# HengWeiBin/CenterFusionDetect3D

Hardware: AMD Instinct MI355X
Metric: frames/sec/GPU CenterFusion forward, 3x448x800 bs=16; 1/2/4/8-GPU scaling (higher is better)
Workload: dtype f32 storage + f32 accumulate; products as split-operand MFMA passes: f16x3 backbone/neck (3 passes), heads' first 3x3 layers fp16 main term + block-scaled FP6 e2m3 cross terms (1.5 passes), heads' 1x1 layers bf16x3; 1 GPU; Centerfusion_Middle (DLA-34 + DCNv2 neck + pc_dep frustum fusion, 7+4 heads) forward + NMS/top-100 decode + 2D->3D postProcess, bs=16/GPU, 3x448x800, 50-200 radar pts/frame, random-init weights; global_batch=16, parallelism=dp1 (batch shard, async all-gather of the final boxes)

## Files before the change

### centerfusiondetect3d_amd/_lib.py

```python
import ctypes as C
import os

_PKG = os.path.dirname(os.path.abspath(__file__))
LIB_PATH = os.path.join(_PKG, "libcfhip.so")

ABI_VERSION = 7
CF_MAX_SRC = 4
CF_MAX_GROUPS = 4
ACT_NONE, ACT_RELU, ACT_SIGMOID_CLAMP, ACT_RAW_AND_SIGDEPTH = 0, 1, 2, 3
LAYOUT_NHWC, LAYOUT_NCHW = 0, 1

_f = C.c_void_p


class ConvArgs(C.Structure):
    _fields_ = [("src", _f * CF_MAX_SRC), ("src_c", C.c_int32 * CF_MAX_SRC), ("n_src", C.c_int32),
                ("B", C.c_int32), ("H", C.c_int32), ("W", C.c_int32), ("Ho", C.c_int32),
                ("Wo", C.c_int32), ("stride", C.c_int32), ("weight", _f), ("slots", _f),
                ("bias", _f), ("K_pad", C.c_int32), ("N", C.c_int32), ("N_pad", C.c_int32),
                ("residual", _f), ("res_stride", C.c_int32), ("out", _f), ("out2", _f),
                ("out_stride", C.c_int32), ("out_layout", C.c_int32), ("act", C.c_int32),
                ("precise", C.c_int32), ("out_scale", C.c_float), ("in_scale", C.c_float)]


class DcnArgs(C.Structure):
    _fields_ = [("x", _f), ("offmask", _f), ("om_stride", C.c_int32), ("B", C.c_int32),
                ("H", C.c_int32), ("W", C.c_int32), ("C", C.c_int32), ("weight", _f), ("bias", _f),
                ("N", C.c_int32), ("N_pad", C.c_int32), ("out", _f), ("out_stride", C.c_int32),
                ("act", C.c_int32), ("precise", C.c_int32), ("out_scale", C.c_float),
                ("out_split_bf16", _f), ("split_stride", C.c_int32), ("workspace", _f),
                ("workspace_bytes", C.c_size_t), ("mask_activated", C.c_int32), ("out_mx", _f), ("in_scale", C.c_float),
                ("mx_scale", C.c_float)]


class DcnBwdArgs(C.Structure):
    _fields_ = [("gout", _f), ("weight", _f), ("x", _f), ("offmask", _f), ("B", C.c_int32), ("H", C.c_int32),
                ("W", C.c_int32), ("C", C.c_int32), ("N", C.c_int32), ("gx", _f), ("gom", _f), ("gw", _f), ("gbias", _f),
                ("workspace", _f), ("workspace_bytes", C.c_size_t)]


CF_MAX_HEADS = 12
CF_DEPTH_MAPS_MAX = 8


class HeadTailArgs(C.Structure):
    _fields_ = [("x", _f), ("x_stride", C.c_int32), ("B", C.c_int32), ("H", C.c_int32),
                ("W", C.c_int32), ("n_heads", C.c_int32), ("n_hidden", C.c_int32),
                ("w_hidden", (_f * 2) * CF_MAX_HEADS), ("b_hidden", (_f * 2) * CF_MAX_HEADS),
                ("w_out", _f * CF_MAX_HEADS), ("b_out", _f * CF_MAX_HEADS),
                ("out", _f * CF_MAX_HEADS), ("out2", _f * CF_MAX_HEADS),
                ("c_base", C.c_int32 * CF_MAX_HEADS), ("n_out", C.c_int32 * CF_MAX_HEADS),
                ("act", C.c_int32 * CF_MAX_HEADS)]


class HeadFusedArgs(C.Structure):
    _fields_ = [("tail", HeadTailArgs), ("src", _f * 2), ("src_c", C.c_int32 * 2), ("n_src", C.c_int32),
                ("slots", _f), ("K_pad", C.c_int32), ("w_first", _f * CF_MAX_HEADS),
                ("b_first", _f * CF_MAX_HEADS), ("layout3x3", C.c_int32), ("w_out_perm", _f * CF_MAX_HEADS),
                ("mfma16", C.c_int32), ("mx", C.c_int32), ("first_scale", C.c_float * CF_MAX_HEADS)]


class StemArgs(C.Structure):
    _fields_ = [("x", _f), ("B", C.c_int32), ("C", C.c_int32), ("H", C.c_int32), ("W", C.c_int32),
                ("w_base", _f), ("b_base", _f), ("scale_base", C.c_float),
                ("w_level0", _f), ("b_level0", _f), ("scale_level0", C.c_float),
                ("w_level1", _f), ("b_level1", _f), ("scale_level1", C.c_float),
                ("out", _f), ("out_pool", _f), ("in_scale", C.c_float * 3)]


class StemEarlyArgs(C.Structure):
    _fields_ = [("stem", StemArgs), ("pc", _f), ("pc_h", C.c_int32), ("pc_w", C.c_int32), ("w_base_radar", _f)]


class PackSrc(C.Structure):
    _fields_ = [("channels", C.c_int32), ("stride", C.c_int32), ("c_base", C.c_int32)]


class PackBn(C.Structure):
    _fields_ = [("gamma", _f), ("beta", _f), ("mean", _f), ("var", _f), ("eps", C.c_float)]


class PackConvDesc(C.Structure):
    _fields_ = [("weight", _f), ("bias", _f), ("bn", PackBn),
                ("cout", C.c_int32), ("kh", C.c_int32), ("kw", C.c_int32), ("stride", C.c_int32),
                ("pad", C.c_int32), ("dilation", C.c_int32),
                ("src", C.POINTER(PackSrc)), ("n_src", C.c_int32),
                ("proj_weight", _f), ("proj_bias", _f), ("proj_bn", PackBn), ("proj", PackSrc)]


class PackInfo(C.Structure):
    _fields_ = [("n_pad", C.c_int32), ("k_pad", C.c_int32), ("n_slots", C.c_int32), ("patch", C.c_int32),
                ("out_scale", C.c_float), ("weight_bytes", C.c_size_t)]


class DecodeArgs(C.Structure):
    _fields_ = [("scores", _f), ("inds", _f), ("classes", _f), ("reg", _f), ("wh", _f),
                ("depth", _f), ("rot", _f), ("dim", _f), ("amodal", _f), ("att", _f), ("vel", _f),
                ("B", C.c_int32), ("K", C.c_int32), ("H", C.c_int32), ("W", C.c_int32),
                ("out_h", C.c_int32), ("out_w", C.c_int32), ("norm2d", C.c_int32), ("det", _f)]


class SerializeArgs(C.Structure):
    _fields_ = [("post", _f), ("B", C.c_int32), ("K", C.c_int32), ("trans_matrix", _f),
                ("velocity_matrix", _f), ("cs_rot", _f), ("pose_rot", _f), ("rows", _f), ("rotation", _f),
                ("n_samples", C.c_int32), ("sample_ptr", _f), ("sample_frames", _f),
                ("max_per_sample", C.c_int32), ("order", _f), ("counts", _f)]


CF_LOSS_MAX_HEADS = 16
CF_LOSS_STATS = 4 + 4 * CF_LOSS_MAX_HEADS
LOSS_L1, LOSS_L1_UNC, LOSS_BINROT, LOSS_BCE = 0, 1, 2, 3


class LossHead(C.Structure):
    _fields_ = [("kind", C.c_int32), ("channels", C.c_int32), ("map", _f), ("target", _f), ("mask", _f), ("rotbin", _f),
                ("unc", _f), ("weight", C.c_float), ("gmap", _f), ("gunc", _f)]


class LossArgs(C.Structure):
    _fields_ = [("heat", _f), ("heat_gt", _f), ("centers", _f), ("wh", _f), ("mask", _f), ("cls", _f),
                ("B", C.c_int32), ("C", C.c_int32), ("h", C.c_int32), ("w", C.c_int32), ("M", C.c_int32),
                ("n_heads", C.c_int32), ("out_area", C.c_float), ("heat_weight", C.c_float),
                ("head", LossHead * CF_LOSS_MAX_HEADS), ("losses", _f), ("total", _f), ("layer_mask", _f), ("stats", _f),
                ("workspace", _f), ("workspace_bytes", C.c_size_t), ("grad_out", _f), ("gheat", _f)]


CF_HEAD_TRAIN_MAX_HIDDEN = 2
_HT_LAYERS = CF_HEAD_TRAIN_MAX_HIDDEN + 2


class HeadTrainArgs(C.Structure):
    _fields_ = [("x", _f), ("x2", _f), ("x_stride", C.c_int32), ("c_x", C.c_int32), ("x2_stride", C.c_int32),
                ("c_x2", C.c_int32), ("B", C.c_int32), ("h", C.c_int32), ("w", C.c_int32), ("n_hidden", C.c_int32),
                ("hidden", C.c_int32), ("n_out", C.c_int32), ("chunk_px", C.c_int32),
                ("weight", _f * _HT_LAYERS), ("bias", _f * _HT_LAYERS), ("y", _f), ("gy", _f),
                ("gw", _f * _HT_LAYERS), ("gb", _f * _HT_LAYERS), ("workspace", _f), ("workspace_bytes", C.c_size_t)]


CF_TARGETS_MAX_OBJS = 128
CF_TARGETS_F = 20
TGT_HAS_AMODAL, TGT_HAS_ATTRIBUTES, TGT_HAS_VELOCITY, TGT_HAS_ALPHA = 1, 2, 4, 8
TGT_HAS_DEPTH, TGT_HAS_DIMENSION, TGT_HAS_LOCATION, TGT_HAS_YAW = 16, 32, 64, 128
TGT_REP3D, TGT_NORM2D, TGT_WRITE_DEPTH, TGT_WRITE_ROT, TGT_FRUSTUM = 1, 2, 4, 8, 16


class TargetsArgs(C.Structure):
    _fields_ = [("ann", _f), ("iann", _f), ("counts", _f), ("trans", _f), ("calib", _f), ("scale", _f), ("pc_dep", _f),
                ("B", C.c_int32), ("M", C.c_int32), ("C", C.c_int32), ("h", C.c_int32), ("w", C.c_int32),
                ("flags", C.c_int32), ("max_pc_dist", C.c_float),
                ("heat", _f), ("cls", _f), ("mask", _f), ("trunc_mask", _f), ("wh", _f), ("reg", _f), ("amodal_offset", _f),
                ("dimension", _f), ("depth", _f), ("rotbin", _f), ("rotres", _f), ("att", _f), ("att_mask", _f),
                ("velocity", _f), ("pc_hm", _f), ("t_bboxes", _f), ("t_scores", _f), ("t_centers", _f),
                ("t_heat_centers", _f), ("t_bboxes3d", _f), ("t_rotation", _f), ("t_att", _f), ("t_velocity", _f),
                ("workspace", _f), ("workspace_bytes", C.c_size_t)]


_i, _d = C.c_int, C.c_double
SYMBOLS = {
    "cf_conv2d_fused": (_i, [C.POINTER(ConvArgs), _f]),
    "cf_conv2d_f16x3": (_i, [C.POINTER(ConvArgs), _f]),
    "cf_conv3x3_f16x3": (_i, [C.POINTER(ConvArgs), _f]),
    "cf_conv3x3_root_f16x3": (_i, [C.POINTER(ConvArgs), C.POINTER(ConvArgs), C.POINTER(C.c_int32), _f]),
    "cf_conv3x3_proj_f16x3": (_i, [C.POINTER(ConvArgs), C.POINTER(C.c_int32), _f]),
    "cf_conv3x3_f16x3_grouped": (_i, [C.POINTER(C.POINTER(ConvArgs)), C.c_int32, _f]),
    "cf_conv3x3_grouped_form": (_i, [C.POINTER(C.POINTER(ConvArgs)), C.c_int32, C.POINTER(C.c_int32)]),
    "cf_stem_fused": (_i, [C.POINTER(StemArgs), _f]),
    "cf_stem_fused_early": (_i, [C.POINTER(StemEarlyArgs), _f]),
    "cf_split_bf16": (_i, [_f, _f, C.c_long, _i, _i, _i, _f]),
    "cf_head_fused": (_i, [C.POINTER(HeadFusedArgs), _f]),
    "cf_head_fused_with": (_i, [C.POINTER(HeadFusedArgs), _i, _i, _f]),
    "cf_head_fused_at": (_i, [C.POINTER(HeadFusedArgs), _f, _i, _f]),
    "cf_head_slot_tables": (_i, [_f, _f, _i, _i, _i, _f, _f, _f]),
    "cf_pack_feat_mx": (_i, [_f, _i, _f, C.c_long, _f]),
    "cf_pack_feat_mx_scaled": (_i, [_f, _i, _f, C.c_long, C.c_float, _f]),
    "cf_absmax_f32": (_i, [_f, C.c_long, _i, _i, _f, _f]),
    "cf_dcn_v2_fused": (_i, [C.POINTER(DcnArgs), _f]),
    "cf_dcn_v2_f16x3": (_i, [C.POINTER(DcnArgs), _f]),
    "cf_dcn_v2_workspace_bytes": (C.c_size_t, [_i, _i, _i, _i, _i]),
    "cf_dcn_v2_f16x3_grouped": (_i, [C.POINTER(C.POINTER(DcnArgs)), C.c_int32, _f]),
    "cf_gemm_tile_form": (_i, [C.c_long, _i, _i, _i, _i, _i, _i, C.POINTER(C.c_int32), C.POINTER(C.c_int32), C.POINTER(C.c_int32)]),
    "cf_dcn_v2_bwd_data": (_i, [C.POINTER(DcnBwdArgs), _f]),
    "cf_dcn_v2_bwd_weight": (_i, [C.POINTER(DcnBwdArgs), _f]),
    "cf_dcn_v2_bwd_workspace_bytes": (C.c_size_t, [_i, _i, _i, _i, _i]),
    "cf_loss_forward": (_i, [C.POINTER(LossArgs), _f]),
    "cf_loss_backward": (_i, [C.POINTER(LossArgs), _f]),
    "cf_loss_workspace_bytes": (C.c_size_t, [_i, _i, _i, _i]),
    "cf_targets_build": (_i, [C.POINTER(TargetsArgs), _f]),
    "cf_targets_workspace_bytes": (C.c_size_t, [_i, _i]),
    "cf_head_train_forward": (_i, [C.POINTER(HeadTrainArgs), _f]),
    "cf_head_backward": (_i, [C.POINTER(HeadTrainArgs), _f]),
    "cf_head_train_workspace_bytes": (C.c_size_t, [_i, _i, _i, _i, _i, _i]),
    "cf_head_bwd_workspace_bytes": (C.c_size_t, [_i, _i, _i, _i, _i, _i]),
    "cf_head_bwd_chunk_px": (_i, [_i, _i, _i, _i]),
    "cf_head_backward_dx": (_i, [C.POINTER(HeadTrainArgs), _f, _i, _f, _i, _f]),
    "cf_head_bwd_dx_workspace_bytes": (C.c_size_t, [_i, _i, _i, _i, _i, _i]),
    "cf_upsample_dw": (_i, [_f, _f, _f, _f, _i, _i, _i, _i, _i, _f]),
    "cf_maxpool2x2": (_i, [_f, _f, _i, _i, _i, _i, _f]),
    "cf_nchw_to_nhwc4": (_i, [_f, _f, _i, _i, _i, _i, _f]),
    "cf_nhwc_to_nchw": (_i, [_f, _f, _i, _i, _i, _i, _i, _f]),
    "cf_nchw_to_nhwc": (_i, [_f, _f, _i, _i, _i, _i, _i, _i, _f]),
    "cf_radar_ingest": (_i, [_f, _f, _i, _i, _i, _f, _i, _i, _d, _d, _i, _f, _f, _f, _f]),
    "cf_preprocess_images": (_i, [_f, _i, _i, _i, C.POINTER(C.c_double), C.POINTER(C.c_float),
                                 C.POINTER(C.c_float), _i, _i, _f, _f]),
    "cf_augment_workspace_bytes": (C.c_size_t, [_i, _i, _i]),
    "cf_augment_images": (_i, [_f, _i, _i, _i, _f, _f, _f, _f, _f, C.POINTER(C.c_float), C.POINTER(C.c_float), _i, _i, _i, _f,
                              _f, C.c_size_t, _f]),
    "cf_topk_workspace_bytes": (C.c_size_t, [_i, _i]),
    "cf_topk_workspace_bytes_nms": (C.c_size_t, [_i, _i, _i, _i, _i]),
    "cf_topk_peaks": (_i, [_f, _i, _i, _i, _i, _i, _i, _f, _f, _f, _f, _f]),
    "cf_topk_peaks_if_changed": (_i, [_f, _i, _i, _i, _i, _i, _i, _f, _f, _f, _f, _f, _f]),
    "cf_checksum64": (_i, [_f, C.c_long, _f, _f]),
    "cf_frustum_assoc": (_i, [_f, _i, _f, _f, _f, _f, _f, _f, _i, _i, _i, C.c_float, _f, _f, _f, _f]),
    "cf_topk_frustum": (_i, [_f, _i, _i, _f, _f, _f, _f, _f, _f, _i, _i, _i, C.c_float, _f, _f, _f, _f, _f, _f, _f, _f]),
    "cf_pc_hm_direct": (_i, [_f, _i, _i, _i, C.c_float, _f, _f, _f]),
    "cf_radar_roi_expand": (_i, [_f, _f, _f, _i, _i, _i, _f, _f, _i, _i, _i, _f, _f, _f, _f]),
    "cf_pillar_expand": (_i, [_f, _f, _f, _i, _i, _i, _f, _f, _i, _i, _d, _d, _d, _f, _f, _f, _f]),
    "cf_decode_gather": (_i, [C.POINTER(DecodeArgs), _f]),
    "cf_post_process": (_i, [_f, _f, _f, _i, _i, _i, _i, _f, _f]),
    "cf_decode_post": (_i, [C.POINTER(DecodeArgs), _f, _f, _f, _f]),
    "cf_decode_gather_unc": (_i, [C.POINTER(DecodeArgs), _f, _f]),
    "cf_decode_post_unc": (_i, [C.POINTER(DecodeArgs), _f, _f, _f, _f, _f]),
    "cf_depth_maps": (_i, [C.POINTER(_f), C.POINTER(C.c_long), _i, _i, _i, _i, _f, _f]),
    "cf_serialize_nuscenes": (_i, [C.POINTER(SerializeArgs), _f]),
    "cf_serialize_max_candidates": (_i, []),
    "cf_spin_us": (_i, [_i, _f]),
    "cf_last_error": (C.c_char_p, []),
    "cf_pack_conv_f16x3_info": (_i, [C.POINTER(PackConvDesc), C.POINTER(PackInfo)]),
    "cf_pack_conv_f16x3": (_i, [C.POINTER(PackConvDesc), _f, _f, _f, C.POINTER(PackInfo)]),
    "cf_pack_dcn_f16_info": (_i, [_i, _i, C.POINTER(PackInfo)]),
    "cf_pack_dcn_f16": (_i, [_f, _f, C.POINTER(PackBn), _i, _i, _f, _f, C.POINTER(PackInfo)]),
    "cf_abi_version": (_i, []),
}

_lib = None


class CfHipError(RuntimeError):
    pass


def load():
    global _lib
    if _lib is None:
        if not os.path.exists(LIB_PATH):
            raise CfHipError(
                f"{LIB_PATH} is missing: build it with `python -m centerfusiondetect3d_amd.build` "
                "(hipcc, gfx950). The CenterFusion forward has no CPU fallback.")
        lib = C.CDLL(LIB_PATH)
        for name, (res, args) in SYMBOLS.items():
            fn = getattr(lib, name)
            fn.restype, fn.argtypes = res, args
        if lib.cf_abi_version() != ABI_VERSION:
            raise CfHipError(f"{LIB_PATH} has ABI version {lib.cf_abi_version()}, this package needs {ABI_VERSION}: "
                             "rebuild it with `python -m centerfusiondetect3d_amd.build`")
        _lib = lib
    return _lib


def check(status, what=""):
    if status != 0:
        msg = load().cf_last_error().decode()
        raise CfHipError(f"{what} failed with status {status}: {msg}")


def ptr(t):
    return None if t is None else t.data_ptr()


def stream_ptr():
    import torch
    return torch.cuda.current_stream().cuda_stream
```

### centerfusiondetect3d_amd/csrc/cf_heads.hip

```cpp
#include <string>
#include "cf_common.h"
#include "cf_mx.h"

namespace {

typedef __bf16 bf16x8 __attribute__((ext_vector_type(8)));
typedef unsigned int u32x4 __attribute__((ext_vector_type(4)));
typedef unsigned int u32x2 __attribute__((ext_vector_type(2)));
typedef _Float16 hf16x8 __attribute__((ext_vector_type(8)));
typedef int i32x8 __attribute__((ext_vector_type(8)));

constexpr int HT_PX = 64;
constexpr int HT_C = 256;
constexpr int HT_ROWB = HT_C * 2 + 16;
constexpr int HT_PLANE = HT_PX * HT_ROWB;
constexpr int HT_LDS = 2 * HT_PLANE;

struct HeadTailK {
  const unsigned char* x;
  int x_stride;
  int M, HW;
  int n_heads;
  int n_hidden;
  const unsigned char* w_hidden[CF_MAX_HEADS][2];
  const float* b_hidden[CF_MAX_HEADS][2];
  const unsigned char* w_out[CF_MAX_HEADS];
  const float* b_out[CF_MAX_HEADS];
  float* out[CF_MAX_HEADS];
  float* out2[CF_MAX_HEADS];
  int c_base[CF_MAX_HEADS];
  int n_out[CF_MAX_HEADS];
  int act[CF_MAX_HEADS];
};

__device__ __forceinline__ float bf16_rne(float a) { return (float)(__bf16)a; }
__device__ __forceinline__ unsigned pack2(float a, float b) {
  return ((unsigned)__builtin_bit_cast(unsigned short, (__bf16)b) << 16) |
         __builtin_bit_cast(unsigned short, (__bf16)a);
}

__device__ __forceinline__ const bf16x8* wfrag(const unsigned char* w, int rt, int ks, int plane, int n_ks, int lane) {
  const unsigned char* base = w + ((size_t)rt * n_ks + ks) * 2048 + plane * 1024;
  return reinterpret_cast<const bf16x8*>(base + (unsigned)lane * 16u);
}

template <bool SCALED = false>
__device__ __forceinline__ void store_hidden_tile16(unsigned char* xt, const f32x4 (&acc)[4][4], const float* bias,
                                                    int wave, int lane, float sc = 1.0f, int pxcol = -1) {
  const int g = lane >> 4, c16 = pxcol < 0 ? (lane & 15) : pxcol;
#pragma unroll
  for (int rt = 0; rt < 4; ++rt) {
    const int ch = wave * 64 + rt * 16 + 4 * g;
    const f32x4 bb = *reinterpret_cast<const f32x4*>(bias + ch);
#pragma unroll
    for (int ct = 0; ct < 4; ++ct) {
      float v[4], hi[4];
#pragma unroll
      for (int e = 0; e < 4; ++e) {
        v[e] = fmaxf(SCALED ? __builtin_fmaf(acc[rt][ct][e], sc, bb[e]) : acc[rt][ct][e] + bb[e], 0.0f);
        hi[e] = bf16_rne(v[e]);
      }
      unsigned char* o = xt + (ct * 16 + c16) * HT_ROWB + ch * 2;
      const u32x2 ph = {pack2(hi[0], hi[1]), pack2(hi[2], hi[3])};
      const u32x2 pl = {pack2(v[0] - hi[0], v[1] - hi[1]), pack2(v[2] - hi[2], v[3] - hi[3])};
      *reinterpret_cast<u32x2*>(o) = ph;
      *reinterpret_cast<u32x2*>(o + HT_PLANE) = pl;
    }
  }
}

struct TileMap {
  int b, y0, x0, H, W, sh = 4;
  __device__ __forceinline__ bool operator()(int px, int& bb, int& pix) const {
    const int y = y0 + (px >> sh), x = x0 + (px & ((1 << sh) - 1));
    if (y >= H || x >= W) return false;
    bb = b;
    pix = y * W + x;
    return true;
  }
};

constexpr int AT_SLOTS = 18;
__device__ __forceinline__ int at_slot_of(int ty, int tx) { return (ty % 3 == 0 && tx % 3 == 0) ? (ty / 3) * 6 + tx / 3 : -1; }
struct SlotMap {
  const int* slots;
  int M, HW, half;
  __device__ __forceinline__ bool operator()(int px, int& bb, int& pix) const {
    const int t = half * 64 + px, sl = at_slot_of(t >> 4, t & 15);
    if (sl < 0) return false;
    const int s = slots[sl];
    if ((unsigned)s >= (unsigned)M) return false;
    bb = s / HW;
    pix = s - bb * HW;
    return true;
  }
};

template <class PixMap>
__device__ __forceinline__ void head_tail_from_lds16(const HeadTailK& p, unsigned char* xt, int head, const PixMap& pm) {
  const int tid = threadIdx.x, lane = tid & 63, wave = tid >> 6;
  const int g = lane >> 4, c16 = lane & 15;
  for (int l = 0; l < p.n_hidden; ++l) {
    const unsigned char* w = p.w_hidden[head][l];
    const float* bias = p.b_hidden[head][l];
    f32x4 acc[4][4];
#pragma unroll
    for (int a = 0; a < 4; ++a)
#pragma unroll
      for (int b = 0; b < 4; ++b)
#pragma unroll
        for (int r = 0; r < 4; ++r) acc[a][b][r] = 0.0f;
    bf16x8 wh[2][4], wl[2][4];
#pragma unroll
    for (int rt = 0; rt < 4; ++rt) {
      wh[0][rt] = *wfrag(w, wave * 4 + rt, 0, 0, 8, lane);
      wl[0][rt] = *wfrag(w, wave * 4 + rt, 0, 1, 8, lane);
    }
#pragma unroll
    for (int ks = 0; ks < 8; ++ks) {
      if (ks + 1 < 8) {
#pragma unroll
        for (int rt = 0; rt < 4; ++rt) {
          wh[(ks + 1) & 1][rt] = *wfrag(w, wave * 4 + rt, ks + 1, 0, 8, lane);
          wl[(ks + 1) & 1][rt] = *wfrag(w, wave * 4 + rt, ks + 1, 1, 8, lane);
        }
      }
      bf16x8 xh[4], xl[4];
#pragma unroll
      for (int ct = 0; ct < 4; ++ct) {
        const unsigned char* row = xt + (ct * 16 + c16) * HT_ROWB + (ks * 32 + g * 8) * 2;
        xh[ct] = *reinterpret_cast<const bf16x8*>(row);
        xl[ct] = *reinterpret_cast<const bf16x8*>(row + HT_PLANE);
      }
#pragma unroll
      for (int rt = 0; rt < 4; ++rt)
#pragma unroll
        for (int ct = 0; ct < 4; ++ct)
          acc[rt][ct] = __builtin_amdgcn_mfma_f32_16x16x32_bf16(wl[ks & 1][rt], xh[ct], acc[rt][ct], 0, 0, 0);
#pragma unroll
      for (int rt = 0; rt < 4; ++rt)
#pragma unroll
        for (int ct = 0; ct < 4; ++ct)
          acc[rt][ct] = __builtin_amdgcn_mfma_f32_16x16x32_bf16(wh[ks & 1][rt], xl[ct], acc[rt][ct], 0, 0, 0);
#pragma unroll
      for (int rt = 0; rt < 4; ++rt)
#pragma unroll
        for (int ct = 0; ct < 4; ++ct)
          acc[rt][ct] = __builtin_amdgcn_mfma_f32_16x16x32_bf16(wh[ks & 1][rt], xh[ct], acc[rt][ct], 0, 0, 0);
      __builtin_amdgcn_sched_barrier(0);
    }
    __syncthreads();
    store_hidden_tile16(xt, acc, bias, wave, lane);
    __syncthreads();
  }

  f32x4 oacc[4];
#pragma unroll
  for (int b = 0; b < 4; ++b)
#pragma unroll
    for (int r = 0; r < 4; ++r) oacc[b][r] = 0.0f;
  {
    const unsigned char* w = p.w_out[head];
#pragma unroll
    for (int s2 = 0; s2 < 2; ++s2) {
      const int ks = wave * 2 + s2;
      const bf16x8 ah = *wfrag(w, 0, ks, 0, 8, lane), al = *wfrag(w, 0, ks, 1, 8, lane);
#pragma unroll
      for (int ct = 0; ct < 4; ++ct) {
        const unsigned char* row = xt + (ct * 16 + c16) * HT_ROWB + (ks * 32 + g * 8) * 2;
        const bf16x8 xh = *reinterpret_cast<const bf16x8*>(row);
        const bf16x8 xl = *reinterpret_cast<const bf16x8*>(row + HT_PLANE);
        oacc[ct] = __builtin_amdgcn_mfma_f32_16x16x32_bf16(al, xh, oacc[ct], 0, 0, 0);
        oacc[ct] = __builtin_amdgcn_mfma_f32_16x16x32_bf16(ah, xl, oacc[ct], 0, 0, 0);
        oacc[ct] = __builtin_amdgcn_mfma_f32_16x16x32_bf16(ah, xh, oacc[ct], 0, 0, 0);
      }
    }
  }
  __syncthreads();
  float* red = reinterpret_cast<float*>(xt);
  const int n_out = p.n_out[head], act = p.act[head];
#pragma unroll
  for (int ct = 0; ct < 4; ++ct)
#pragma unroll
    for (int r = 0; r < 4; ++r) {
      const int n = 4 * g + r;
      if (n < n_out) red[(wave * 16 + n) * HT_PX + ct * 16 + c16] = oacc[ct][r];
    }
  __syncthreads();
  const float* bo = p.b_out[head];
  float* out = p.out[head];
  float* out2 = p.out2[head];
  const int px = tid & 63;
  int b, pix;
  if (pm(px, b, pix)) {
    for (int n = tid >> 6; n < n_out; n += 4) {
      const float raw = red[n * HT_PX + px] + red[(16 + n) * HT_PX + px] + red[(32 + n) * HT_PX + px] +
                        red[(48 + n) * HT_PX + px] + bo[n];
      const size_t o = ((size_t)b * n_out + n) * p.HW + pix;
      float v = raw;
      if (act == CF_ACT_RELU) v = fmaxf(raw, 0.0f);
      else if (act == CF_ACT_SIGMOID_CLAMP) v = fminf(fmaxf(cf_sigmoid(raw), 1e-4f), 1.0f - 1e-4f);
      out[o] = v;
      if (act == CF_ACT_RAW_AND_SIGDEPTH) out2[o] = 1.0f / (cf_sigmoid(raw) + 1e-6f) - 1.0f;
    }
  }
}

constexpr int HP_ROWS = (8 + 2) * (16 + 2);
constexpr int HP_PX = 8 * 16;
constexpr int HP16_RED = 4 * 16 * HP_PX * 4;
constexpr int hp16_patch_bytes(bool pc) { return HP_ROWS * (4 * 64 + (pc ? 32 : 0) + 16); }
constexpr int HP_PCIMG_ROWB = 32 * 2 + 16;
constexpr int HP_PCIMG = HP_PX * 2 * HP_PCIMG_ROWB;
constexpr int hp16_pc_extra(bool pc) { return pc ? 16 + HP_PCIMG : 0; }
constexpr int hp16_lds(bool pc, bool hidden) {
  return hidden ? (HT_LDS > hp16_patch_bytes(pc) + hp16_pc_extra(pc) ? HT_LDS : hp16_patch_bytes(pc) + hp16_pc_extra(pc))
                : hp16_patch_bytes(pc) + hp16_pc_extra(pc) + HP16_RED;
}

struct HeadPatchK {
  HeadTailK t;
  const unsigned char* src[2];
  int src_c[2];
  int H, W, tiles_x, tiles_y, n_ks;
  int pc_skip;
  int hloop;
  const unsigned char* w_first[CF_MAX_HEADS];
  const float* b_first[CF_MAX_HEADS];
  const unsigned char* w_out_perm[CF_MAX_HEADS];
  float first_scale[CF_MAX_HEADS];
  const int* slot_pixels;
};

template <int NS, bool PC, bool TP, bool MX = false, int HID = -1, bool AT = false>
__global__ __launch_bounds__(256, 2) void head_patch16_kernel(HeadPatchK q) {
  static_assert(NS == 4, "64 feature channels");
  static_assert(!AT || !TP, "virtual tiles are laid out on the flat 8 x 16 tile");
  constexpr int MX_SLAB = 14592, PC_OFF = MX ? 272 : NS * 64;
  constexpr int TSH = TP ? 3 : 4, TMASK = (1 << TSH) - 1;
  constexpr int T_H = TP ? 16 : 8, T_W = TP ? 8 : 16, P_W = T_W + 2;
  static_assert((T_H + 2) * P_W == HP_ROWS, "both tile shapes have the same patch size");
  constexpr int ROWB = NS * 64 + (PC ? 32 : 0) + 16;
  constexpr int NKF = 9 * NS / 2;
  constexpr int NK = NKF + (PC ? 1 : 0);
  extern __shared__ __attribute__((aligned(16))) unsigned char xt[];
  const HeadTailK& p = q.t;
  const int tid = threadIdx.x, lane = tid & 63, wave = __builtin_amdgcn_readfirstlane(tid >> 6);
  const int g = lane >> 4;
  const int c16 = (MX && !TP) ? ((lane & 12) == 4 || (lane & 12) == 8 ? (((lane & 15) - 4) & 3) * 4 + (((lane & 15) - 4) >> 2)
                                                                      : (lane & 3) * 4 + 2 + ((lane & 15) >> 3))
                              : (lane & 15);
  const int per_img = q.tiles_x * q.tiles_y;
  const int per_head = AT ? per_img : per_img * (p.M / p.HW);
  const int hg = blockIdx.x / per_head;
  int rem = cf_xcd_remap(blockIdx.x - hg * per_head, per_head);
  const int head0 = hg * q.hloop, head1 = min(head0 + q.hloop, p.n_heads);
  const int b = rem / per_img;
  rem -= b * per_img;
  const int y0 = (rem / q.tiles_x) * T_H, x0 = (rem % q.tiles_x) * T_W;
  const int* const at_slots = AT ? q.slot_pixels + (size_t)rem * AT_SLOTS : nullptr;
  auto at_src = [&](int row) -> int {
    const int pr = row / P_W, pc = row % P_W;
    if (pr >= 9) return -1;
    const int s = at_slots[(pr / 3) * 6 + pc / 3];
    if ((unsigned)s >= (unsigned)p.M) return -1;
    const int bb = s / p.HW, pix = s - bb * p.HW;
    const int y = pix / q.W + pr % 3 - 1, x = pix % q.W + pc % 3 - 1;
    if ((unsigned)y >= (unsigned)q.H || (unsigned)x >= (unsigned)q.W) return -1;
    return bb * p.HW + y * q.W + x;
  };
  if constexpr (AT) {
    int any = 0;
    for (int i = 0; i < AT_SLOTS; ++i) any |= (unsigned)at_slots[i] < (unsigned)p.M ? 1 : 0;
    if (!any) return;
  }

  if constexpr (MX) {
    constexpr int UPR = 17;
    constexpr int NIT = (HP_ROWS * UPR + 255) / 256;
    u32x4 v[NIT];
#pragma unroll
    for (int it = 0; it < NIT; ++it) {
      const int idx = tid + it * 256;
      const int row = idx / UPR, u = idx % UPR;
      const int y = y0 - 1 + row / P_W, x = x0 - 1 + row % P_W;
      v[it] = u32x4{0u, 0u, 0u, 0u};
      if constexpr (AT) {
        const int s = row < HP_ROWS ? at_src(row) : -1;
        if (s >= 0) v[it] = *reinterpret_cast<const u32x4*>(q.src[0] + (size_t)s * 272 + u * 16);
      } else
      if (row < HP_ROWS && (unsigned)y < (unsigned)q.H && (unsigned)x < (unsigned)q.W)
        v[it] = *reinterpret_cast<const u32x4*>(q.src[0] + (size_t)(b * p.HW + y * q.W + x) * 272 + u * 16);
    }
#pragma unroll
    for (int it = 0; it < NIT; ++it) {
      const int idx = tid + it * 256;
      const int row = idx / UPR, u = idx % UPR;
      if (row < HP_ROWS) *reinterpret_cast<u32x4*>(xt + row * ROWB + u * 16) = v[it];
    }
  } else {
    constexpr int UPR = NS * 4;
    constexpr int NIT = (HP_ROWS * UPR + 255) / 256;
    u32x4 v[NIT];
#pragma unroll
    for (int it = 0; it < NIT; ++it) {
      const int idx = tid + it * 256;
      const int row = idx / UPR, u = idx % UPR;
      const int y = y0 - 1 + row / P_W, x = x0 - 1 + row % P_W;
      v[it] = u32x4{0u, 0u, 0u, 0u};
      if constexpr (AT) {
        const int s = row < HP_ROWS ? at_src(row) : -1;
        if (s >= 0) v[it] = *reinterpret_cast<const u32x4*>(q.src[0] + ((size_t)s * 2 * q.src_c[0]) * 2 +
                                                             (u / (NS * 2)) * q.src_c[0] * 2 + (u % (NS * 2)) * 16);
      } else
      if (row < HP_ROWS && (unsigned)y < (unsigned)q.H && (unsigned)x < (unsigned)q.W)
        v[it] = *reinterpret_cast<const u32x4*>(q.src[0] + ((size_t)(b * p.HW + y * q.W + x) * 2 * q.src_c[0]) * 2 +
                                                (u / (NS * 2)) * q.src_c[0] * 2 + (u % (NS * 2)) * 16);
    }
#pragma unroll
    for (int it = 0; it < NIT; ++it) {
      const int idx = tid + it * 256;
      const int row = idx / UPR, u = idx % UPR;
      const int plane = u / (NS * 2), uu = u % (NS * 2);
      if (row < HP_ROWS) *reinterpret_cast<u32x4*>(xt + row * ROWB + (uu >> 1) * 64 + plane * 32 + (uu & 1) * 16) = v[it];
    }
  }
  unsigned* const pc_flags = reinterpret_cast<unsigned*>(xt + hp16_patch_bytes(PC));
  if (PC) {
    unsigned nz = 0u;
    for (int idx = tid; idx < HP_ROWS * 2; idx += 256) {
      const int row = idx >> 1, plane = idx & 1;
      const int y = y0 - 1 + row / P_W, x = x0 - 1 + row % P_W;
      u32x4 w = {0u, 0u, 0u, 0u};
      if constexpr (AT) {
        const int s = at_src(row);
        if (s >= 0) w = *reinterpret_cast<const u32x4*>(q.src[1] + ((size_t)s * 2 + plane) * q.src_c[1] * 2);
      } else
      if ((unsigned)y < (unsigned)q.H && (unsigned)x < (unsigned)q.W)
        w = *reinterpret_cast<const u32x4*>(q.src[1] + ((size_t)(b * p.HW + y * q.W + x) * 2 + plane) * q.src_c[1] * 2);
      *reinterpret_cast<u32x4*>(xt + row * ROWB + PC_OFF + plane * 16) = w;
      nz |= (w[0] | w[1] | w[2] | w[3]) & 0x7fff7fffu;
    }
    const bool wave_nz = __builtin_amdgcn_ballot_w64(nz != 0u) != 0ull;
    if (lane == 0) pc_flags[wave] = (wave_nz || !q.pc_skip) ? 1u : 0u;
  }

  int rowb[8];
#pragma unroll
  for (int ct = 0; ct < 8; ++ct)
    rowb[ct] = ((c16 >> TSH) * P_W + (c16 & TMASK)) * ROWB + ct * ((16 >> TSH) * P_W * ROWB);
  const int koff = (g >> 1) * 64 + (g & 1) * 16;
  unsigned char* const pcimg = xt + hp16_patch_bytes(PC) + 16;
  const int imgb = c16 * (2 * HP_PCIMG_ROWB) + g * 16;
  __syncthreads();
  bool pc_live = false;
  if (PC) {
    const u32x4 f = *reinterpret_cast<const u32x4*>(pc_flags);
    pc_live = __builtin_amdgcn_readfirstlane((int)(f[0] | f[1] | f[2] | f[3])) != 0;
  }
  if (PC && pc_live) {
    const int ipx = tid & (HP_PX - 1), plane = tid >> 7;
    const unsigned char* sp = xt + ((ipx >> TSH) * P_W + (ipx & TMASK)) * ROWB + PC_OFF + plane * 16;
    unsigned e[32];
#pragma unroll
    for (int t = 0; t < 9; ++t) {
      const u32x2 w = *reinterpret_cast<const u32x2*>(sp + ((t / 3) * P_W + t % 3) * ROWB);
      e[3 * t] = w[0] & 0xffffu;
      e[3 * t + 1] = w[0] >> 16;
      e[3 * t + 2] = w[1] & 0xffffu;
    }
#pragma unroll
    for (int k = 27; k < 32; ++k) e[k] = 0u;
    unsigned char* dp = pcimg + (ipx * 2 + plane) * HP_PCIMG_ROWB;
#pragma unroll
    for (int j = 0; j < 4; ++j)
      *reinterpret_cast<u32x4*>(dp + j * 16) = u32x4{e[8 * j] | (e[8 * j + 1] << 16), e[8 * j + 2] | (e[8 * j + 3] << 16),
                                                     e[8 * j + 4] | (e[8 * j + 5] << 16), e[8 * j + 6] | (e[8 * j + 7] << 16)};
    __syncthreads();
  }
  auto pc_kstep = [&](const bf16x8 (&ah)[4], const bf16x8 (&al)[4], f32x4 (&acc)[4][8]) __attribute__((always_inline)) {
#pragma unroll
    for (int hf = 0; hf < 2; ++hf) {
      bf16x8 xh[4], xl[4];
#pragma unroll
      for (int ct = 0; ct < 4; ++ct) {
        const unsigned char* r = pcimg + imgb + (4 * hf + ct) * (16 * 2 * HP_PCIMG_ROWB);
        xh[ct] = *reinterpret_cast<const bf16x8*>(r);
        xl[ct] = *reinterpret_cast<const bf16x8*>(r + HP_PCIMG_ROWB);
      }
#pragma unroll
      for (int rt = 0; rt < 4; ++rt)
#pragma unroll
        for (int ct = 0; ct < 4; ++ct)
          acc[rt][4 * hf + ct] = __builtin_amdgcn_mfma_f32_16x16x32_bf16(al[rt], xh[ct], acc[rt][4 * hf + ct], 0, 0, 0);
#pragma unroll
      for (int rt = 0; rt < 4; ++rt)
#pragma unroll
        for (int ct = 0; ct < 4; ++ct)
          acc[rt][4 * hf + ct] = __builtin_amdgcn_mfma_f32_16x16x32_bf16(ah[rt], xl[ct], acc[rt][4 * hf + ct], 0, 0, 0);
#pragma unroll
      for (int rt = 0; rt < 4; ++rt)
#pragma unroll
        for (int ct = 0; ct < 4; ++ct)
          acc[rt][4 * hf + ct] = __builtin_amdgcn_mfma_f32_16x16x32_bf16(ah[rt], xh[ct], acc[rt][4 * hf + ct], 0, 0, 0);
    }
  };
  auto first_layer = [&](int head, f32x4 (&acc)[4][8]) __attribute__((always_inline)) {
  if constexpr (MX) {
    const unsigned char* wb = q.w_first[head] + (size_t)wave * (9 * MX_SLAB);
#pragma unroll
    for (int a = 0; a < 4; ++a)
#pragma unroll
      for (int c = 0; c < 8; ++c)
#pragma unroll
        for (int r = 0; r < 4; ++r) acc[a][c][r] = 0.0f;
    hf16x8 am[2][4];
    u32x4 ax0[4];
    u32x2 ax1[4];
    int sa;
    auto slab = [&](int tap) {
      return __builtin_amdgcn_make_buffer_rsrc(const_cast<unsigned char*>(wb + tap * MX_SLAB), 0, MX_SLAB, 0x00020000);
    };
    const int l16 = lane * 16, l8 = lane * 8, l4 = lane * 4;
    bf16x8 ph[4], pl[4];
    auto ldp = [&](bf16x8 (&d)[4], int plane) {
      const __amdgpu_buffer_rsrc_t rs = __builtin_amdgcn_make_buffer_rsrc(
          const_cast<unsigned char*>(q.w_first[head] + (size_t)4 * 9 * MX_SLAB), 0, 4 * 3 * 4 * 2048, 0x00020000);
      const int lo = l16 + (g ? 2 * 4 * 2048 : 0);
#pragma unroll
      for (int rt = 0; rt < 4; ++rt)
        d[rt] = __builtin_bit_cast(bf16x8, __builtin_amdgcn_raw_buffer_load_b128(rs, lo, wave * (3 * 4 * 2048) + rt * 2048 + plane * 1024, 0));
    };
    auto ldm = [&](hf16x8 (&d)[4], int tap, int ks2) {
      const __amdgpu_buffer_rsrc_t rs = slab(tap);
#pragma unroll
      for (int rt = 0; rt < 4; ++rt)
        d[rt] = __builtin_bit_cast(hf16x8, __builtin_amdgcn_raw_buffer_load_b128(rs, l16, (rt * 2 + ks2) * 1024, 0));
    };
    auto ldx = [&](int tap) {
      const __amdgpu_buffer_rsrc_t rs = slab(tap);
#pragma unroll
      for (int rt = 0; rt < 4; ++rt) {
        ax0[rt] = __builtin_bit_cast(u32x4, __builtin_amdgcn_raw_buffer_load_b128(rs, l16, 8192 + rt * 1536, 0));
        ax1[rt] = __builtin_bit_cast(u32x2, __builtin_amdgcn_raw_buffer_load_b64(rs, l8, 8192 + rt * 1536 + 1024, 0));
      }
      sa = (int)__builtin_amdgcn_raw_buffer_load_b32(rs, l4, 14336, 0);
    };
    auto main_half = [&](const hf16x8 (&A)[4], int off, int hf) {
      hf16x8 xb[4];
#pragma unroll
      for (int ct = 0; ct < 4; ++ct) xb[ct] = *reinterpret_cast<const hf16x8*>(xt + rowb[4 * hf + ct] + off);
#pragma unroll
      for (int rt = 0; rt < 4; ++rt)
#pragma unroll
        for (int ct = 0; ct < 4; ++ct)
          acc[rt][4 * hf + ct] = __builtin_amdgcn_mfma_f32_16x16x32_f16(A[rt], xb[ct], acc[rt][4 * hf + ct], 0, 0, 0);
    };
    auto cross_pair = [&](int toff, int pr) {
      i32x8 xb[2];
      int sb[2];
#pragma unroll
      for (int c2 = 0; c2 < 2; ++c2) {
        const unsigned char* r = xt + rowb[2 * pr + c2] + toff;
        const u32x4 b0 = *reinterpret_cast<const u32x4*>(r + 64 * g + 32);
        const u32x2 b1 = *reinterpret_cast<const u32x2*>(r + 64 * g + 48);
        xb[c2] = i32x8{(int)b0[0], (int)b0[1], (int)b0[2], (int)b0[3], (int)b1[0], (int)b1[1], 0, 0};
        sb[c2] = (int)(*reinterpret_cast<const unsigned*>(r + 256) >> (8 * g));
      }
#define CF_MX_ROW(RT)                                                                                                   \
      {                                                                                                                 \
        const i32x8 a6 = {(int)ax0[RT][0], (int)ax0[RT][1], (int)ax0[RT][2], (int)ax0[RT][3], (int)ax1[RT][0],          \
                          (int)ax1[RT][1], 0, 0};                                                                       \
        _Pragma("unroll") for (int c2 = 0; c2 < 2; ++c2)                                                                \
          acc[RT][2 * pr + c2] = __builtin_amdgcn_mfma_scale_f32_16x16x128_f8f6f4(a6, xb[c2], acc[RT][2 * pr + c2],    \
                                                                                  2, 2, RT, sa, 0, sb[c2]);             \
      }
      CF_MX_ROW(0) CF_MX_ROW(1) CF_MX_ROW(2) CF_MX_ROW(3)
#undef CF_MX_ROW
    };
    ldm(am[0], 0, 0);
    ldm(am[1], 0, 1);
    ldx(0);
#pragma unroll
    for (int tap = 0; tap < 9; ++tap) {
      const int toff = ((tap / 3) * P_W + tap % 3) * ROWB;
      const int o0 = toff + g * 64, o1 = toff + g * 64 + 16;
      main_half(am[0], o0, 0);
      if (tap > 0) ldx(tap);
      __builtin_amdgcn_sched_barrier(0);
      main_half(am[0], o0, 1);
      main_half(am[1], o1, 0);
      if (tap + 1 < 9) ldm(am[0], tap + 1, 0);
      else if (PC && HID == 1) ldp(ph, 0);
      __builtin_amdgcn_sched_barrier(0);
      main_half(am[1], o1, 1);
      cross_pair(toff, 0);
      cross_pair(toff, 1);
      if (tap + 1 < 9) ldm(am[1], tap + 1, 1);
      else if (PC && HID == 1) ldp(pl, 1);
      __builtin_amdgcn_sched_barrier(0);
      cross_pair(toff, 2);
      cross_pair(toff, 3);
    }
    __builtin_amdgcn_sched_barrier(0);
    if (PC) {
      if (pc_live) {
        if constexpr (HID != 1) { ldp(ph, 0); ldp(pl, 1); }
        pc_kstep(ph, pl, acc);
      }
    }
    return;
  }
  const unsigned char* w1 = q.w_first[head];
#pragma unroll
  for (int a = 0; a < 4; ++a)
#pragma unroll
    for (int c = 0; c < 8; ++c)
#pragma unroll
      for (int r = 0; r < 4; ++r) acc[a][c][r] = 0.0f;

  bf16x8 wh[2][4], wl[2][4];
  auto load_w = [&](bf16x8 (&dh)[4], bf16x8 (&dl)[4], int ks) {
#pragma unroll
    for (int rt = 0; rt < 4; ++rt) {
      dh[rt] = *wfrag(w1, wave * 4 + rt, ks, 0, q.n_ks, lane);
      dl[rt] = *wfrag(w1, wave * 4 + rt, ks, 1, q.n_ks, lane);
    }
  };
  load_w(wh[0], wl[0], 0);

#pragma unroll
  for (int ks = 0; ks < NKF; ++ks) {
    if (ks + 1 < NK) load_w(wh[(ks + 1) & 1], wl[(ks + 1) & 1], ks + 1);
    const int tap = ks / (NS / 2), half = ks % (NS / 2);
    const int off = ((tap / 3) * P_W + tap % 3) * ROWB + half * 128 + koff, lo = 32;
#pragma unroll
    for (int hf = 0; hf < 2; ++hf) {
      bf16x8 xh[4], xl[4];
#pragma unroll
      for (int ct = 0; ct < 4; ++ct) {
        xh[ct] = *reinterpret_cast<const bf16x8*>(xt + rowb[4 * hf + ct] + off);
        xl[ct] = *reinterpret_cast<const bf16x8*>(xt + rowb[4 * hf + ct] + off + lo);
      }
#pragma unroll
      for (int rt = 0; rt < 4; ++rt)
#pragma unroll
        for (int ct = 0; ct < 4; ++ct)
          acc[rt][4 * hf + ct] = __builtin_amdgcn_mfma_f32_16x16x32_bf16(wl[ks & 1][rt], xh[ct], acc[rt][4 * hf + ct], 0, 0, 0);
#pragma unroll
      for (int rt = 0; rt < 4; ++rt)
#pragma unroll
        for (int ct = 0; ct < 4; ++ct)
          acc[rt][4 * hf + ct] = __builtin_amdgcn_mfma_f32_16x16x32_bf16(wh[ks & 1][rt], xl[ct], acc[rt][4 * hf + ct], 0, 0, 0);
#pragma unroll
      for (int rt = 0; rt < 4; ++rt)
#pragma unroll
        for (int ct = 0; ct < 4; ++ct)
          acc[rt][4 * hf + ct] = __builtin_amdgcn_mfma_f32_16x16x32_bf16(wh[ks & 1][rt], xh[ct], acc[rt][4 * hf + ct], 0, 0, 0);
    }
    __builtin_amdgcn_sched_barrier(0);
  }
  if (PC) {
    if (pc_live) pc_kstep(wh[NKF & 1], wl[NKF & 1], acc);
  }
  };

  if (HID < 0 ? p.n_hidden > 0 : HID == 1) {
    const int head = head0;
    f32x4 acc[4][8];
    first_layer(head, acc);
    __syncthreads();
#pragma unroll
    for (int half = 0; half < 2; ++half) {
      f32x4 a2[4][4];
#pragma unroll
      for (int rt = 0; rt < 4; ++rt)
#pragma unroll
        for (int ct = 0; ct < 4; ++ct) a2[rt][ct] = acc[rt][4 * half + ct];
      store_hidden_tile16<MX>(xt, a2, q.b_first[head], wave, lane, MX ? q.first_scale[head] : 1.0f, c16);
      if constexpr (MX) __builtin_amdgcn_sched_barrier(0);
      __syncthreads();
      if constexpr (AT) head_tail_from_lds16(p, xt, head, SlotMap{at_slots, p.M, p.HW, half});
      else head_tail_from_lds16(p, xt, head, TileMap{b, y0 + (64 >> TSH) * half, x0, q.H, q.W, TSH});
      __syncthreads();
    }
    return;
  }
  if constexpr (HID == 1) return;

  for (int head = head0; head < head1; ++head) {
  f32x4 acc[4][8];
  first_layer(head, acc);
  f32x4 oacc[8];
#pragma unroll
  for (int c = 0; c < 8; ++c)
#pragma unroll
    for (int r = 0; r < 4; ++r) oacc[c][r] = 0.0f;
  {
    const float* b1 = q.b_first[head] + wave * 64 + 4 * g;
    const unsigned char* wo = q.w_out_perm[head];
    const float fsc = MX ? q.first_scale[head] : 1.0f;
    (void)fsc;
#pragma unroll
    for (int s2 = 0; s2 < 2; ++s2) {
      const int ks2 = wave * 2 + s2;
      const bf16x8 ah = *wfrag(wo, 0, ks2, 0, 8, lane), al = *wfrag(wo, 0, ks2, 1, 8, lane);
      const f32x4 ba = *reinterpret_cast<const f32x4*>(b1 + 32 * s2);
      const f32x4 bb = *reinterpret_cast<const f32x4*>(b1 + 32 * s2 + 16);
#pragma unroll
      for (int ct = 0; ct < 8; ++ct) {
        float v[8], hi[8];
#pragma unroll
        for (int j = 0; j < 8; ++j) {
          const float bj = j < 4 ? ba[j] : bb[j - 4];
          v[j] = fmaxf(MX ? __builtin_fmaf(acc[2 * s2 + (j >> 2)][ct][j & 3], fsc, bj) : acc[2 * s2 + (j >> 2)][ct][j & 3] + bj, 0.0f);
          hi[j] = bf16_rne(v[j]);
        }
        const u32x4 ph = {pack2(hi[0], hi[1]), pack2(hi[2], hi[3]), pack2(hi[4], hi[5]), pack2(hi[6], hi[7])};
        const u32x4 pl = {pack2(v[0] - hi[0], v[1] - hi[1]), pack2(v[2] - hi[2], v[3] - hi[3]),
                          pack2(v[4] - hi[4], v[5] - hi[5]), pack2(v[6] - hi[6], v[7] - hi[7])};
        const bf16x8 xh = __builtin_bit_cast(bf16x8, ph), xl = __builtin_bit_cast(bf16x8, pl);
        oacc[ct] = __builtin_amdgcn_mfma_f32_16x16x32_bf16(al, xh, oacc[ct], 0, 0, 0);
        oacc[ct] = __builtin_amdgcn_mfma_f32_16x16x32_bf16(ah, xl, oacc[ct], 0, 0, 0);
        oacc[ct] = __builtin_amdgcn_mfma_f32_16x16x32_bf16(ah, xh, oacc[ct], 0, 0, 0);
      }
    }
  }
  const int n_out = p.n_out[head], act = p.act[head];
  float* red = reinterpret_cast<float*>(xt + hp16_patch_bytes(PC) + hp16_pc_extra(PC));
#pragma unroll
  for (int ct = 0; ct < 8; ++ct)
#pragma unroll
    for (int r = 0; r < 4; ++r) {
      const int n = 4 * g + r;
      if (n < n_out) red[(wave * 16 + n) * HP_PX + ct * 16 + c16] = oacc[ct][r];
    }
  __syncthreads();
  {
    const int px = tid & (HP_PX - 1);
    const int y = y0 + (px >> TSH), x = x0 + (px & TMASK);
    bool valid = y < q.H && x < q.W;
    int ob = b;
    size_t opix = (size_t)y * q.W + x;
    if constexpr (AT) {
      const int sl = at_slot_of(px >> 4, px & 15);
      const int s = sl >= 0 ? at_slots[sl] : -1;
      valid = (unsigned)s < (unsigned)p.M;
      ob = s / p.HW;
      opix = (size_t)(s - ob * p.HW);
    }
    if (valid) {
      const float* bo = p.b_out[head];
      float* out = p.out[head];
      float* out2 = p.out2[head];
      for (int n = tid >> 7; n < n_out; n += 2) {
        const float raw = red[n * HP_PX + px] + red[(16 + n) * HP_PX + px] + red[(32 + n) * HP_PX + px] +
                          red[(48 + n) * HP_PX + px] + bo[n];
        const size_t o = ((size_t)ob * n_out + n) * p.HW + opix;
        float v = raw;
        if (act == CF_ACT_RELU) v = fmaxf(raw, 0.0f);
        else if (act == CF_ACT_SIGMOID_CLAMP) v = fminf(fmaxf(cf_sigmoid(raw), 1e-4f), 1.0f - 1e-4f);
        out[o] = v;
        if (act == CF_ACT_RAW_AND_SIGDEPTH) out2[o] = 1.0f / (cf_sigmoid(raw) + 1e-6f) - 1.0f;
      }
    }
  }
  __syncthreads();
  }
}

__global__ __launch_bounds__(256) void pack_feat_mx_kernel(const float* __restrict__ x, int in_stride,
                                                           unsigned char* __restrict__ rows, long M, float scale) {
  const long t = (long)blockIdx.x * 256 + threadIdx.x;
  const long m = t >> 1;
  const int blk = (int)(t & 1);
  if (m >= M) return;
  const f32x4* src = reinterpret_cast<const f32x4*>(x + m * in_stride + 32 * blk);
  float v[32];
#pragma unroll
  for (int i = 0; i < 8; ++i) {
    const f32x4 q = src[i];
#pragma unroll
    for (int e = 0; e < 4; ++e) v[4 * i + e] = q[e];
  }
  mx_pack_block(v, rows + m * 272, blk, scale);
}

}

extern "C" int cf_pack_feat_mx_scaled(const float* x, int in_stride, void* rows, long M, float scale, void* stream) {
  CF_REQUIRE(x && rows && M > 0, "cf_pack_feat_mx: null tensor or M=%ld", M);
  const float sc = cf_resolve_in_scale(scale);
  CF_REQUIRE(sc > 0.0f, "cf_pack_feat_mx_scaled: scale must be 0 (= 16) or a power of two");
  CF_REQUIRE(in_stride >= 64 && in_stride % 4 == 0, "cf_pack_feat_mx: in_stride=%d (64 channels, 16-byte aligned rows)", in_stride);
  CF_REQUIRE(M < (1L << 30), "cf_pack_feat_mx: M=%ld too large", M);
  const long threads = 2 * M;
  hipLaunchKernelGGL(pack_feat_mx_kernel, dim3((unsigned)((threads + 255) / 256)), dim3(256), 0, (hipStream_t)stream, x,
                     in_stride, static_cast<unsigned char*>(rows), M, sc);
  return cf_check_launch("cf_pack_feat_mx");
}

extern "C" int cf_pack_feat_mx(const float* x, int in_stride, void* rows, long M, void* stream) {
  return cf_pack_feat_mx_scaled(x, in_stride, rows, M, 16.0f, stream);
}

static int fill_tail(const cf_head_tail_args* a, HeadTailK& k) {
  CF_REQUIRE(a->B > 0 && a->H > 0 && a->W > 0, "cf_head_fused: bad geometry");
  CF_REQUIRE(a->n_heads >= 1 && a->n_heads <= CF_MAX_HEADS, "cf_head_fused: n_heads=%d", a->n_heads);
  CF_REQUIRE(a->n_hidden >= 0 && a->n_hidden <= 2, "cf_head_fused: n_hidden=%d", a->n_hidden);
  const long M = (long)a->B * a->H * a->W;
  CF_REQUIRE(M < (1L << 31), "cf_head_fused: tensor too large");
  k.x = reinterpret_cast<const unsigned char*>(a->x);
  k.x_stride = a->x_stride;
  k.M = (int)M;
  k.HW = a->H * a->W;
  k.n_heads = a->n_heads;
  k.n_hidden = a->n_hidden;
  for (int i = 0; i < a->n_heads; ++i) {
    for (int l = 0; l < a->n_hidden; ++l) {
      CF_REQUIRE(a->w_hidden[i][l] && a->b_hidden[i][l], "cf_head_fused: head %d layer %d weights missing", i, l);
      k.w_hidden[i][l] = reinterpret_cast<const unsigned char*>(a->w_hidden[i][l]);
      k.b_hidden[i][l] = a->b_hidden[i][l];
    }
    CF_REQUIRE(a->w_out[i] && a->b_out[i] && a->out[i], "cf_head_fused: head %d output layer missing", i);
    CF_REQUIRE(a->n_out[i] >= 1 && a->n_out[i] <= 32, "cf_head_fused: head %d n_out=%d", i, a->n_out[i]);
    CF_REQUIRE(a->act[i] != CF_ACT_RAW_AND_SIGDEPTH || a->out2[i], "cf_head_fused: head %d needs out2", i);
    k.w_out[i] = reinterpret_cast<const unsigned char*>(a->w_out[i]);
    k.b_out[i] = a->b_out[i];
    k.out[i] = a->out[i];
    k.out2[i] = a->out2[i];
    k.c_base[i] = a->c_base[i];
    k.n_out[i] = a->n_out[i];
    k.act[i] = a->act[i];
  }
  return CF_OK;
}

constexpr int HEAD_MAX_K_PAD = 2048;
#define CF_HEAD_FORMS "cf_head_fused runs layout3x3 = 1 (64-channel first source [, 8-channel second]) with mfma16 = 1 " \
                      "(16x16x32 fragments, n_out <= 16) only"

static int head_fused_launch(const cf_head_fused_args* a, const int* slot_pixels, int n_tiles, int tile, int pc_skip, void* stream) {
  const bool at = slot_pixels != nullptr;
  HeadPatchK hp{};
  hp.slot_pixels = slot_pixels;
  const int rc = fill_tail(&a->tail, hp.t);
  if (rc != CF_OK) return rc;
  CF_REQUIRE(a->n_src >= 1 && a->n_src <= 2, "cf_head_fused: n_src=%d", a->n_src);
  for (int i = 0; i < a->n_src; ++i) {
    CF_REQUIRE(a->src[i] && a->src_c[i] > 0 && a->src_c[i] % 8 == 0, "cf_head_fused: source %d invalid", i);
    hp.src[i] = reinterpret_cast<const unsigned char*>(a->src[i]);
    hp.src_c[i] = a->src_c[i];
  }
  const bool mx = a->mx != 0;
  if (mx) {
    CF_REQUIRE(a->layout3x3 && a->mfma16 && a->src_c[0] == 64 && (a->n_src == 1 || a->src_c[1] == 8),
               "cf_head_fused: mx = 1 needs layout3x3 = 1, mfma16 = 1, a 64-channel mx source [and an 8-channel pc_hm source]");
  } else {
    CF_REQUIRE(a->slots && a->K_pad > 0 && a->K_pad % 64 == 0, "cf_head_fused: K_pad=%d must be a multiple of 64", a->K_pad);
    CF_REQUIRE(a->K_pad <= HEAD_MAX_K_PAD, "cf_head_fused: K_pad=%d exceeds %d", a->K_pad, HEAD_MAX_K_PAD);
  }
  const int n_heads = a->tail.n_heads, H = a->tail.H, W = a->tail.W;
  for (int i = 0; i < n_heads; ++i) {
    CF_REQUIRE(a->w_first[i] && a->b_first[i], "cf_head_fused: head %d first layer missing", i);
    hp.w_first[i] = reinterpret_cast<const unsigned char*>(a->w_first[i]);
    hp.b_first[i] = a->b_first[i];
  }
  if (!(a->layout3x3 && a->src_c[0] == 64 && (a->n_src == 1 || a->src_c[1] == 8))) {
    CF_REQUIRE(a->mfma16 == 0, "cf_head_fused: mfma16 fragments need the 3x3 patch layout (layout3x3 = 1, 64-channel first "
                               "source [, 8-channel second]); this launch would run on the 32x32x16 slot-table kernel");
    cf_set_error(CF_HEAD_FORMS ": there is no slot-table kernel (layout3x3 = 0)");
    return CF_EINVAL;
  }
  const bool m16 = a->mfma16 != 0;
  hp.H = H; hp.W = W;
  hp.n_ks = a->K_pad / 32;
  CF_REQUIRE(mx || a->K_pad / 16 >= (a->n_src == 2 ? 38 : 36), "cf_head_fused: K_pad=%d too small for the 3x3 layout", a->K_pad);
  for (int i = 0; i < n_heads; ++i) {
    CF_REQUIRE(!mx || (a->first_scale[i] > 0.0f && a->first_scale[i] < 1e30f), "cf_head_fused: head %d: first_scale missing (mx)", i);
    hp.first_scale[i] = a->first_scale[i];
  }
  if (m16) {
    CF_REQUIRE(mx || (a->K_pad % 32 == 0 && a->K_pad / 32 >= (a->n_src == 2 ? 19 : 18)), "cf_head_fused: K_pad=%d (16x16x32 fragments)", a->K_pad);
    for (int i = 0; i < n_heads; ++i)
      CF_REQUIRE(a->tail.n_out[i] <= 16, "cf_head_fused: head %d: n_out=%d > 16 (the 16x16x32 kernels produce ONE 16-row output tile, with or without hidden layers)", i, a->tail.n_out[i]);
  }
  for (int i = 0; i < n_heads; ++i) {
    CF_REQUIRE(a->tail.n_hidden > 0 || a->w_out_perm[i], "cf_head_fused: head %d: w_out_perm missing", i);
    hp.w_out_perm[i] = reinterpret_cast<const unsigned char*>(a->w_out_perm[i]);
  }
  const long t_land = (long)((W + 15) / 16) * ((H + 7) / 8), t_port = (long)((W + 7) / 8) * ((H + 15) / 16);
  CF_REQUIRE(t_land * a->tail.B * n_heads < (1L << 31), "cf_head_fused: grid too large");
  CF_REQUIRE(m16, CF_HEAD_FORMS ": nothing reads 32x32x16 fragments (mfma16 = 0)");
  bool portrait = tile < 0 ? t_port < t_land : tile != 0;
  if (at) portrait = false;
  hp.pc_skip = pc_skip != 0;
  hp.tiles_x = portrait ? (W + 7) / 8 : (W + 15) / 16;
  hp.tiles_y = portrait ? (H + 15) / 16 : (H + 7) / 8;
  const int n_img = at ? 1 : a->tail.B;
  if (at) { hp.tiles_x = n_tiles; hp.tiles_y = 1; }
  int hloop = 1;
  if (a->tail.n_hidden == 0) {
    static const int slots = [] {
      int dev = 0, cus = 256;
      if (hipGetDevice(&dev) == hipSuccess) (void)hipDeviceGetAttribute(&cus, hipDeviceAttributeMultiprocessorCount, dev);
      return 2 * (cus > 0 ? cus : 256);
    }();
    const long tiles = (long)hp.tiles_x * hp.tiles_y * n_img;
    const int n = n_heads, cand[3] = {1, 2, (n + 1) / 2};
    double best = 0.0;
    for (int i = 0; i < 3; ++i) {
      const int h = cand[i] < 1 ? 1 : (cand[i] > n ? n : cand[i]);
      const double cost = (double)((tiles * ((n + h - 1) / h) + slots - 1) / slots) * (h + 0.25);
      if (i == 0 || cost < best - 1e-9) { best = cost; hloop = h; }
    }
  }
  hp.hloop = hloop;
  const long blocks = (long)hp.tiles_x * hp.tiles_y * n_img * ((n_heads + hloop - 1) / hloop);
  CF_REQUIRE(blocks < (1L << 31), "%s: grid too large", at ? "cf_head_fused_at" : "cf_head_fused");
  const bool hidden = a->tail.n_hidden > 0;
  const bool pc = a->n_src == 2;
  const int lds = hp16_lds(pc, hidden);
  auto launch = [&](auto kernel, CfLdsLimit& lim) {
    lim.ensure(kernel, lds, hp16_lds(pc, false));
    hipLaunchKernelGGL(kernel, dim3((unsigned)blocks), dim3(256), lds, (hipStream_t)stream, hp);
  };
  static CfLdsLimit lim16[4], limx[4], limxh[2], lim_at[4];
  if (at) {
    CF_REQUIRE(!mx || hidden == pc, "cf_head_fused_at: mx = 1 runs without hidden layers and pc_hm source, or with both (the forms "
                                    "the model's head groups take); pack other heads for bf16x3");
    if (mx && hidden) launch(head_patch16_kernel<4, true, false, true, 1, true>, lim_at[3]);
    else if (mx) launch(head_patch16_kernel<4, false, false, true, 0, true>, lim_at[2]);
    else if (pc) launch(head_patch16_kernel<4, true, false, false, -1, true>, lim_at[1]);
    else launch(head_patch16_kernel<4, false, false, false, -1, true>, lim_at[0]);
    return cf_check_launch("cf_head_fused_at");
  }
  if (mx && hidden) {
    CF_REQUIRE(pc, "cf_head_fused: mx = 1 with hidden layers needs the pc_hm source (n_src = 2); pack such heads for bf16x3");
    if (portrait) launch(head_patch16_kernel<4, true, true, true, 1>, limxh[1]);
    else launch(head_patch16_kernel<4, true, false, true, 1>, limxh[0]);
  } else if (mx) {
    if (pc && portrait) launch(head_patch16_kernel<4, true, true, true, 0>, limx[3]);
    else if (pc) launch(head_patch16_kernel<4, true, false, true, 0>, limx[2]);
    else if (portrait) launch(head_patch16_kernel<4, false, true, true, 0>, limx[1]);
    else launch(head_patch16_kernel<4, false, false, true, 0>, limx[0]);
  } else {
    if (pc && portrait) launch(head_patch16_kernel<4, true, true>, lim16[3]);
    else if (pc) launch(head_patch16_kernel<4, true, false>, lim16[2]);
    else if (portrait) launch(head_patch16_kernel<4, false, true>, lim16[1]);
    else launch(head_patch16_kernel<4, false, false>, lim16[0]);
  }
  return cf_check_launch("cf_head_fused");
}

extern "C" int cf_head_fused_with(const cf_head_fused_args* a, int tile, int pc_skip, void* stream) {
  CF_REQUIRE(a != nullptr, "cf_head_fused: null args (a)");
  CF_REQUIRE(tile >= -1 && tile <= 1, "cf_head_fused_with: tile=%d is not 0 (8 x 16), 1 (16 x 8) or -1 (the rule's own)", tile);
  CF_REQUIRE(pc_skip >= -1 && pc_skip <= 1, "cf_head_fused_with: pc_skip=%d is not 0, 1 or -1 (the rule's own)", pc_skip);
  return head_fused_launch(a, nullptr, 0, tile, pc_skip, stream);
}

extern "C" int cf_head_fused(const cf_head_fused_args* a, void* stream) { return cf_head_fused_with(a, -1, -1, stream); }

extern "C" int cf_head_fused_at(const cf_head_fused_args* a, const int32_t* slot_pixels, int n_tiles, void* stream) {
  CF_REQUIRE(a != nullptr, "cf_head_fused_at: null args");
  CF_REQUIRE(slot_pixels != nullptr && n_tiles > 0, "cf_head_fused_at: slot table missing or n_tiles=%d", n_tiles);
  const int rc = head_fused_launch(a, slot_pixels, n_tiles, -1, -1, stream);
  if (rc == CF_EINVAL) {
    const std::string why = cf_last_error();
    cf_set_error("cf_head_fused_at: %s", why.c_str());
  }
  return rc;
}

namespace {
__global__ __launch_bounds__(256) void head_slot_tables_kernel(const int* __restrict__ tk, const int* __restrict__ pk, int B, int K,
                                                               int HW, int* __restrict__ tp, int* __restrict__ ts) {
  const int i = blockIdx.x * 256 + threadIdx.x;
  const int per_p = (2 * K + AT_SLOTS - 1) / AT_SLOTS * AT_SLOTS, per_s = (K + AT_SLOTS - 1) / AT_SLOTS * AT_SLOTS;
  if (tp && i < B * per_p) {
    const int b = i / per_p, j = i - b * per_p;
    int v = -1;
    if (j < K) v = tk ? tk[b * K + j] : -1;
    else if (j < 2 * K) v = pk ? pk[b * K + j - K] : -1;
    tp[i] = (unsigned)v < (unsigned)HW ? b * HW + v : -1;
  }
  if (ts && i < B * per_s) {
    const int b = i / per_s, j = i - b * per_s;
    const int v = (j < K && pk) ? pk[b * K + j] : -1;
    ts[i] = (unsigned)v < (unsigned)HW ? b * HW + v : -1;
  }
}
}

extern "C" int cf_head_slot_tables(const int32_t* list_a, const int32_t* list_b, int B, int K, int HW, int32_t* table_ab,
                                   int32_t* table_b, void* stream) {
  CF_REQUIRE(B > 0 && K > 0 && HW > 0, "cf_head_slot_tables: B=%d K=%d HW=%d", B, K, HW);
  CF_REQUIRE((long)B * HW < (1L << 31), "cf_head_slot_tables: B * HW must stay below 2^31 (flat pixels are int32)");
  CF_REQUIRE((long)B * (2L * K + AT_SLOTS) < (1L << 31), "cf_head_slot_tables: B * K too large");
  CF_REQUIRE(list_a || list_b, "cf_head_slot_tables: no list");
  CF_REQUIRE(table_ab || table_b, "cf_head_slot_tables: no table");
  CF_REQUIRE(!table_b || list_b, "cf_head_slot_tables: table_b is built from list_b");
  const long n = (long)B * ((2 * K + AT_SLOTS - 1) / AT_SLOTS * AT_SLOTS);
  hipLaunchKernelGGL(head_slot_tables_kernel, dim3((unsigned)((n + 255) / 256)), dim3(256), 0, (hipStream_t)stream, list_a,
                     list_b, B, K, HW, table_ab, table_b);
  return cf_check_launch("cf_head_slot_tables");
}
```

### centerfusiondetect3d_amd/csrc/cf_topk.hip

```cpp
#include "cf_topk.h"

namespace {
template <bool NMS>
__device__ __forceinline__ float peak_value(const float* __restrict__ img, int i, int H, int W) {
  const float v = img[i];
  if (!NMS) return v;
  const int HW = H * W;
  const int c = i / HW, pix = i - c * HW;
  const int y = pix / W, x = pix - y * W;
  const float* pl = img + (size_t)c * HW;
  float m = v;
  const int y0 = y > 0 ? y - 1 : y, y1 = y < H - 1 ? y + 1 : y;
  const int x0 = x > 0 ? x - 1 : x, x1 = x < W - 1 ? x + 1 : x;
  for (int yy = y0; yy <= y1; ++yy)
    for (int xx = x0; xx <= x1; ++xx) m = fmaxf(m, pl[yy * W + xx]);
  return (m == v) ? v : v * 0.0f;
}

__global__ __launch_bounds__(256) void nms_kernel(const float* __restrict__ heat, float* __restrict__ out, int H,
                                                  int W, long total) {
  const long N = (long)H * W;
  for (long i = (long)blockIdx.x * 256 + threadIdx.x; i < total; i += (long)gridDim.x * 256) {
    const long plane = i / N;
    out[i] = peak_value<true>(heat + plane * N, (int)(i - plane * N), H, W);
  }
}

template <bool NMS>
__device__ __forceinline__ void topk_slice_body(const float* __restrict__ heat, int C, int H, int W, int K,
                                                uint64_t* __restrict__ out_keys, int img_i, int slice) {
  __shared__ __attribute__((aligned(16))) uint64_t keys[TOPK_CAP];
  __shared__ uint32_t hist[256];
  __shared__ uint32_t wave_cnt[TOPK_THREADS / 64];
  __shared__ uint32_t s_gt, s_sel[2];
  const int tid = threadIdx.x;
  const int HW = H * W, N = C * HW;
  const float* img = heat + (size_t)img_i * N;
  const int len = (N + TOPK_SLICES - 1) / TOPK_SLICES;
  const int lo = min(slice * len, N), hi = min(lo + len, N);
  uint64_t* out = out_keys + ((size_t)img_i * TOPK_SLICES + slice) * K;
  const int n = hi - lo;
  if (n <= K) {
    topk_tiny_slice<TOPK_THREADS>(keys, lo, n, K, out, [&](int i) { return f2u(peak_value<NMS>(img, i, H, W)); });
    return;
  }

  uint32_t lmax = 0;
  {
    int i = lo + tid;
    for (; i + 3 * TOPK_THREADS < hi; i += 4 * TOPK_THREADS) {
      float v[4];
#pragma unroll
      for (int u = 0; u < 4; ++u) v[u] = img[i + u * TOPK_THREADS];
#pragma unroll
      for (int u = 0; u < 4; ++u)
        if (!NMS || f2u(v[u]) > lmax || v[u] < 0.0f)
          lmax = max(lmax, NMS ? f2u(peak_value<NMS>(img, i + u * TOPK_THREADS, H, W)) : f2u(v[u]));
    }
    for (; i < hi; i += TOPK_THREADS) {
      const float v = img[i];
      if (!NMS || f2u(v) > lmax || v < 0.0f) lmax = max(lmax, f2u(peak_value<NMS>(img, i, H, W)));
    }
  }
  uint32_t* lm = reinterpret_cast<uint32_t*>(keys);
  lm[tid] = lmax;
  __syncthreads();
  {
    const u32x4p* l4 = reinterpret_cast<const u32x4p*>(lm);
    int rank = 0;
#pragma unroll 8
    for (int j4 = 0; j4 < TOPK_THREADS / 4; ++j4) {
      const u32x4p o = l4[j4];
#pragma unroll
      for (int e = 0; e < 4; ++e) rank += (o[e] > lmax || (o[e] == lmax && 4 * j4 + e < tid)) ? 1 : 0;
    }
    if (rank == K - 1) s_sel[0] = lmax;
  }
  __syncthreads();
  uint32_t L = s_sel[0];
  __syncthreads();

  for (int attempt = 0; attempt < 2; ++attempt) {
    if (tid == 0) s_gt = 0;
    __syncthreads();
    {
      auto take = [&](int i, float v) {
        uint32_t u = f2u(v);
        if (NMS && (u > L || v < 0.0f)) u = f2u(peak_value<NMS>(img, i, H, W));
        if (u > L) {
          const uint32_t pos = atomicAdd(&s_gt, 1u);
          if (pos < TOPK_CAP) keys[pos] = pack_key(u, i);
        }
      };
      int i = lo + tid;
      for (; i + 3 * TOPK_THREADS < hi; i += 4 * TOPK_THREADS) {
        float v[4];
#pragma unroll
        for (int u = 0; u < 4; ++u) v[u] = img[i + u * TOPK_THREADS];
#pragma unroll
        for (int u = 0; u < 4; ++u) take(i + u * TOPK_THREADS, v[u]);
      }
      for (; i < hi; i += TOPK_THREADS) take(i, img[i]);
    }
    __syncthreads();
    if (s_gt <= TOPK_CAP) break;
    L = topk_radix_select<TOPK_THREADS>(hist, s_sel, K, [&](auto count) {
      for (int i = lo + tid; i < hi; i += TOPK_THREADS) count(f2u(peak_value<NMS>(img, i, H, W)));
    });
  }
  const int g = (int)s_gt;
  int total = g;
  if (g < K) {
    const int r = K - g;
    int found = 0;
    for (int base = lo; base < hi && found < r; base += TOPK_THREADS) {
      const int i = base + tid;
      const bool eq = (i < hi) && (!NMS || f2u(img[i]) >= L || img[i] < 0.0f) && (f2u(peak_value<NMS>(img, i, H, W)) == L);
      int all;
      const int rank = found + topk_tie_round<TOPK_THREADS>(eq, wave_cnt, all);
      if (eq && rank < r) keys[g + rank] = pack_key(L, i);
      found += all;
      __syncthreads();
    }
    total = K;
  }
  if (total <= 4 * TOPK_THREADS) {
    __syncthreads();
    rank_select_desc(keys, total, K, out);
    return;
  }
  int P = 1;
  while (P < total) P <<= 1;
  for (int i = total + tid; i < P; i += TOPK_THREADS) keys[i] = 0;
  __syncthreads();
  bitonic_sort_desc(keys, P);
  for (int j = tid; j < K; j += TOPK_THREADS) out[j] = keys[j];
}

template <bool NMS>
__global__ __launch_bounds__(TOPK_THREADS) void topk_slice_kernel(const float* __restrict__ heat, int C, int H,
                                                                  int W, int K, uint64_t* __restrict__ out_keys) {
  topk_slice_body<NMS>(heat, C, H, W, K, out_keys, blockIdx.x / TOPK_SLICES, blockIdx.x % TOPK_SLICES);
}

__global__ __launch_bounds__(TOPK_RT) void topk_slice_reg_kernel(const float* __restrict__ heat, int C, int H, int W, int K,
                                                                 uint64_t* __restrict__ out_keys) {
  __shared__ uint64_t keys[TOPK_CAP];
  __shared__ __attribute__((aligned(16))) uint32_t gmax[256];
  __shared__ uint32_t hist[256];
  __shared__ uint32_t wave_cnt[TOPK_RT / 64];
  __shared__ uint32_t s_gt, s_sel[2];
  const int tid = threadIdx.x;
  const int N = C * H * W;
  const int img_i = blockIdx.x / TOPK_SLICES, slice = blockIdx.x % TOPK_SLICES;
  const float* img = heat + (size_t)img_i * N;
  const int len = (N + TOPK_SLICES - 1) / TOPK_SLICES;
  const int lo = min(slice * len, N), hi = min(lo + len, N);
  uint64_t* out = out_keys + (size_t)blockIdx.x * K;
  const int n = hi - lo;
  if (n <= K) {
    topk_tiny_slice<TOPK_RT>(keys, lo, n, K, out, [&](int i) { return f2u(img[i]); });
    return;
  }
  uint32_t u[TOPK_RE];
  uint32_t lmax = 0;
#pragma unroll
  for (int e = 0; e < TOPK_RE; ++e) {
    const int i = lo + tid + e * TOPK_RT;
    u[e] = i < hi ? f2u(img[i]) : 0u;
  }
#pragma unroll
  for (int e = 0; e < TOPK_RE; ++e) lmax = max(lmax, u[e]);
  const int P = K <= 128 ? 8 : 4, G = TOPK_RT / P;
  {
    uint32_t m = lmax;
    m = max(m, (uint32_t)__shfl_xor((int)m, 1));
    m = max(m, (uint32_t)__shfl_xor((int)m, 2));
    if (P == 8) m = max(m, (uint32_t)__shfl_xor((int)m, 4));
    if ((tid & (P - 1)) == 0) gmax[tid / P] = m;
  }
  if (tid == 0) s_sel[0] = 0u;
  __syncthreads();
  {
    const int c = tid / P, part = tid & (P - 1), per = G / P;
    const uint32_t mine = gmax[c];
    const u32x4p* g4 = reinterpret_cast<const u32x4p*>(gmax + part * per);
    int rank = 0;
#pragma unroll 4
    for (int j4 = 0; j4 < per / 4; ++j4) {
      const u32x4p o = g4[j4];
#pragma unroll
      for (int e = 0; e < 4; ++e) rank += (o[e] > mine || (o[e] == mine && part * per + 4 * j4 + e < c)) ? 1 : 0;
    }
    rank += __shfl_xor(rank, 1);
    rank += __shfl_xor(rank, 2);
    if (P == 8) rank += __shfl_xor(rank, 4);
    if (part == 0 && rank == K - 1) s_sel[0] = mine;
  }
  __syncthreads();
  uint32_t L = s_sel[0];
  __syncthreads();

  if (tid == 0) s_gt = 0;
  __syncthreads();
#pragma unroll
  for (int e = 0; e < TOPK_RE; ++e) {
    const int i = lo + tid + e * TOPK_RT;
    if (i < hi && u[e] >= L) {
      const uint32_t pos = atomicAdd(&s_gt, 1u);
      if (pos < TOPK_CAP) keys[pos] = pack_key(u[e], i);
    }
  }
  __syncthreads();
  if (s_gt <= TOPK_CAP) {
    rank_select_desc(keys, (int)s_gt, K, out);
    return;
  }
  __syncthreads();

  for (int attempt = 0; attempt < 2; ++attempt) {
    if (tid == 0) s_gt = 0;
    __syncthreads();
#pragma unroll
    for (int e = 0; e < TOPK_RE; ++e) {
      const int i = lo + tid + e * TOPK_RT;
      if (i < hi && u[e] > L) {
        const uint32_t pos = atomicAdd(&s_gt, 1u);
        if (pos < TOPK_CAP) keys[pos] = pack_key(u[e], i);
      }
    }
    __syncthreads();
    if (s_gt <= TOPK_CAP) break;
    L = topk_radix_select<TOPK_RT>(hist, s_sel, K, [&](auto count) {
#pragma unroll
      for (int e = 0; e < TOPK_RE; ++e)
        if (lo + tid + e * TOPK_RT < hi) count(u[e]);
    });
  }
  const int g = (int)s_gt;
  int total = g;
  if (g < K) {
    const int r = K - g;
    int found = 0;
#pragma unroll 1
    for (int e = 0; e < TOPK_RE && found < r; ++e) {
      const int i = lo + tid + e * TOPK_RT;
      uint32_t ue = 0;
#pragma unroll
      for (int q = 0; q < TOPK_RE; ++q) ue = q == e ? u[q] : ue;
      const bool eq = i < hi && ue == L;
      int all;
      const int rank = found + topk_tie_round<TOPK_RT>(eq, wave_cnt, all);
      if (eq && rank < r) keys[g + rank] = pack_key(L, i);
      found += all;
      __syncthreads();
    }
    total = K;
  }
  __syncthreads();
  rank_select_desc(keys, total, K, out);
}

template <int THREADS>
__device__ __forceinline__ void emit_peaks(const uint64_t* best, int K, int HW, int b, float* __restrict__ scores,
                                           int32_t* __restrict__ inds, int32_t* __restrict__ classes) {
  for (int j = threadIdx.x; j < K; j += THREADS) {
    float score;
    int pix, cls;
    unpack_key(best[j], HW, score, pix, cls);
    scores[(size_t)b * K + j] = score;
    inds[(size_t)b * K + j] = pix;
    classes[(size_t)b * K + j] = cls;
  }
}

__global__ __launch_bounds__(TOPK_MERGE_THREADS) void topk_merge_kernel(const uint64_t* __restrict__ in_keys,
                                                                        int K, int HW, float* __restrict__ scores,
                                                                        int32_t* __restrict__ inds,
                                                                        int32_t* __restrict__ classes) {
  extern __shared__ __attribute__((aligned(16))) uint64_t keys[];
  const int tid = threadIdx.x, total = TOPK_SLICES * K;
  const uint64_t* src = in_keys + (size_t)blockIdx.x * total;
  for (int i = tid; i < total; i += TOPK_MERGE_THREADS) keys[i] = src[i];
  __syncthreads();
  emit_peaks<TOPK_MERGE_THREADS>(merge_sorted_lists(keys, keys + total, K), K, HW, blockIdx.x, scores, inds, classes);
}
}

static int topk_check_geometry(const char* who, int B, int C, int H, int W, int K) {
  CF_REQUIRE(B > 0 && C > 0 && H > 0 && W > 0, "%s: bad geometry", who);
  CF_REQUIRE(K >= 1 && K <= TOPK_MAXK, "%s: K=%d outside [1,%d]", who, K, TOPK_MAXK);
  CF_REQUIRE((long)C * H * W >= K, "%s: fewer than K elements per image", who);
  CF_REQUIRE((long)C * H * W < (1L << 31), "%s: image too large", who);
  return CF_OK;
}

int topk_launch_slices(const char* who, const float* heat, int B, int C, int H, int W, int K, int nms, void* workspace,
                       hipStream_t st) {
  if (const int e = topk_check_geometry(who, B, C, H, W, K)) return e;
  CF_REQUIRE(nms >= 0 && nms <= 2, "%s: nms=%d", who, nms);
  uint64_t* keys = static_cast<uint64_t*>(workspace);
  if (nms == 2) {
    float* sup = reinterpret_cast<float*>(static_cast<unsigned char*>(workspace) + ((cf_topk_workspace_bytes(B, K) + 255) / 256) * 256);
    const long total = (long)B * C * H * W;
    const long blocks = (total + 255) / 256;
    hipLaunchKernelGGL(nms_kernel, dim3((unsigned)(blocks < 65536 ? blocks : 65536)), dim3(256), 0, st, heat, sup, H, W, total);
    heat = sup;
  }
  const long slice_len = ((long)C * H * W + TOPK_SLICES - 1) / TOPK_SLICES;
  const bool reg = nms == 0 && slice_len <= (long)TOPK_RT * TOPK_RE;
  const auto kernel = reg ? topk_slice_reg_kernel : nms == 1 ? topk_slice_kernel<true> : topk_slice_kernel<false>;
  hipLaunchKernelGGL(kernel, dim3(B * TOPK_SLICES), dim3(reg ? TOPK_RT : TOPK_THREADS), 0, st, heat, C, H, W, K, keys);
  return CF_OK;
}

extern "C" size_t cf_topk_workspace_bytes(int B, int K) {
  return (size_t)(B > 0 ? B : 0) * TOPK_SLICES * (size_t)(K > 0 ? K : 0) * sizeof(uint64_t);
}

extern "C" size_t cf_topk_workspace_bytes_nms(int B, int C, int H, int W, int K) {
  const size_t map = (size_t)(B > 0 ? B : 0) * (size_t)(C > 0 ? C : 0) * (size_t)(H > 0 ? H : 0) * (size_t)(W > 0 ? W : 0);
  return ((cf_topk_workspace_bytes(B, K) + 255) / 256) * 256 + map * sizeof(float);
}

extern "C" int cf_topk_peaks(const float* heat, int B, int C, int H, int W, int K, int nms, float* scores,
                             int32_t* inds, int32_t* classes, void* workspace, void* stream) {
  CF_REQUIRE(heat && scores && inds && classes && workspace, "cf_topk_peaks: null buffer");
  hipStream_t st = (hipStream_t)stream;
  if (const int e = topk_launch_slices("cf_topk_peaks", heat, B, C, H, W, K, nms, workspace, st)) return e;
  static CfLdsLimit merge_limit;
  merge_limit.ensure(topk_merge_kernel, topk_merge_lds_bytes(K), 65536);
  hipLaunchKernelGGL(topk_merge_kernel, dim3(B), dim3(TOPK_MERGE_THREADS), topk_merge_lds_bytes(K), st,
                     static_cast<const uint64_t*>(workspace), K, H * W, scores, inds, classes);
  return cf_check_launch("cf_topk_peaks");
}

namespace {
__global__ __launch_bounds__(TOPK_THREADS) void topk_fallback_kernel(const float* __restrict__ heat, int C, int H, int W, int K,
                                                                     uint64_t* __restrict__ keys_ws, float* __restrict__ scores,
                                                                     int32_t* __restrict__ inds, int32_t* __restrict__ classes,
                                                                     const unsigned long long* __restrict__ sums) {
  {
    int diff = 0;
    for (int i = threadIdx.x; i < CK_PARTS; i += TOPK_THREADS) diff |= sums[i] != sums[CK_PARTS + i] ? 1 : 0;
    if (!__syncthreads_or(diff)) return;
  }
  extern __shared__ __attribute__((aligned(16))) uint64_t mkeys[];
  const int b = blockIdx.x, tid = threadIdx.x, total = TOPK_SLICES * K;
  for (int sl = 0; sl < TOPK_SLICES; ++sl) {
    topk_slice_body<true>(heat, C, H, W, K, keys_ws, b, sl);
    __syncthreads();
  }
  __threadfence_block();
  __syncthreads();
  const uint64_t* src = keys_ws + (size_t)b * total;
  for (int i = tid; i < total; i += TOPK_THREADS) mkeys[i] = src[i];
  __syncthreads();
  emit_peaks<TOPK_THREADS>(merge_sorted_lists(mkeys, mkeys + total, K), K, H * W, b, scores, inds, classes);
}
}

extern "C" int cf_topk_peaks_if_changed(const float* heat, int B, int C, int H, int W, int K, int nms, float* scores,
                                        int32_t* inds, int32_t* classes, void* workspace,
                                        const unsigned long long* sums, void* stream) {
  CF_REQUIRE(heat && scores && inds && classes && workspace && sums, "cf_topk_peaks_if_changed: null buffer");
  if (const int e = topk_check_geometry("cf_topk_peaks_if_changed", B, C, H, W, K)) return e;
  CF_REQUIRE(nms == 1 || nms == 2, "cf_topk_peaks_if_changed: nms=%d (the guard of the decoder's NMS'd peaks: 1 or 2, same result)", nms);
  static CfLdsLimit limit;
  limit.ensure(topk_fallback_kernel, topk_merge_lds_bytes(K), 65536);
  hipLaunchKernelGGL(topk_fallback_kernel, dim3(B), dim3(TOPK_THREADS), topk_merge_lds_bytes(K), (hipStream_t)stream, heat, C,
                     H, W, K, static_cast<uint64_t*>(workspace), scores, inds, classes, sums);
  return cf_check_launch("cf_topk_peaks_if_changed");
}

namespace {
__global__ __launch_bounds__(1024) void checksum64_kernel(const uint32_t* __restrict__ x, long n, unsigned long long* __restrict__ parts) {
  unsigned long long acc = 0ull;
  const long step = (long)CK_PARTS * 1024;
  const long n4 = (reinterpret_cast<uintptr_t>(x) & 15) == 0 ? n / 4 : 0;
  const u32x4p* x4 = reinterpret_cast<const u32x4p*>(x);
  for (long i = (long)blockIdx.x * 1024 + threadIdx.x; i < n4; i += step) {
    const u32x4p v = x4[i];
#pragma unroll
    for (int e = 0; e < 4; ++e)
      acc += (unsigned long long)v[e] * (unsigned long long)(((uint32_t)(4 * i + e) * 2654435761u) | 1u);
  }
  for (long i = 4 * n4 + (long)blockIdx.x * 1024 + threadIdx.x; i < n; i += step)
    acc += (unsigned long long)x[i] * (unsigned long long)(((uint32_t)i * 2654435761u) | 1u);
#pragma unroll
  for (int o = 32; o > 0; o >>= 1) acc += (unsigned long long)__shfl_xor((long long)acc, o, 64);
  __shared__ unsigned long long part[16];
  if ((threadIdx.x & 63) == 0) part[threadIdx.x >> 6] = acc;
  __syncthreads();
  if (threadIdx.x == 0) {
    unsigned long long t = 0ull;
    for (int w = 0; w < 16; ++w) t += part[w];
    parts[blockIdx.x] = t;
  }
}
}

extern "C" int cf_checksum64(const void* x, long n_words, unsigned long long* parts, void* stream) {
  CF_REQUIRE(x && parts && n_words >= 0, "cf_checksum64: null buffer or n_words=%ld", n_words);
  hipLaunchKernelGGL(checksum64_kernel, dim3(CK_PARTS), dim3(1024), 0, (hipStream_t)stream, static_cast<const uint32_t*>(x), n_words, parts);
  return cf_check_launch("cf_checksum64");
}
```

### centerfusiondetect3d_amd/ops.py

```python
import ctypes as C
from typing import Optional, Sequence

import torch

from . import _lib
from ._lib import (ACT_NONE, ACT_RELU, ACT_SIGMOID_CLAMP, ACT_RAW_AND_SIGDEPTH, LAYOUT_NHWC, LAYOUT_NCHW)
from .packing import PackedConv, PackedDcn, MX_ROW as packing_MX_ROW


def _need_cuda(*ts):
    for t in ts:
        if t is not None and not t.is_cuda:
            raise _lib.CfHipError("libcfhip operators need device tensors (no CPU path)")


DEFAULT_IN_SCALE = 16.0
F16_MAX = 65504.0


IN_SCALE_KEEP_MIN = 2.0 ** -6
IN_SCALE_MAX = 2.0 ** 32
F32_MIN_NORMAL = 2.0 ** -126


# ... 585 lines not shown
    return total, vec, lm, stats


class _GenericLossFn(torch.autograd.Function):

    @staticmethod
    def forward(ctx, spec, *tensors):
        total, vec, lm, stats = _loss_run_forward(spec, tensors)
        ctx.spec = spec
        ctx.save_for_backward(stats, *tensors)
        ctx.mark_non_differentiable(vec, lm)
        return total, vec, lm

    @staticmethod
    @torch.autograd.function.once_differentiable
    def backward(ctx, gtotal, _gvec, _glm):
        stats, *tensors = ctx.saved_tensors
        spec = ctx.spec
        n = len(spec["kinds"])
        need = ctx.needs_input_grad[1:2 + n + 1]
        a, keep = _loss_forward(spec, tensors)
        dev = stats.device
        go = gtotal.detach().to(torch.float32).contiguous()
        a.stats, a.grad_out = stats.data_ptr(), go.data_ptr()
        grads = [None] * len(tensors)
        if need[0]:
            grads[0] = torch.empty(tensors[0].shape, device=dev, dtype=torch.float32)
            a.gheat = grads[0].data_ptr()
        sparse = [i for i in range(1, n + 2) if need[i] and tensors[i] is not None]
        if sparse:
            sizes = [(tensors[i].numel() + 3) // 4 * 4 for i in sparse]
            flat = torch.zeros(sum(sizes), device=dev, dtype=torch.float32)
            at = 0
            for i, sz in zip(sparse, sizes):
                grads[i] = flat[at:at + tensors[i].numel()].view(tensors[i].shape)
                at += sz
            for i in range(n):
                if grads[1 + i] is not None:
                    a.head[i].gmap = grads[1 + i].data_ptr()
                if grads[1 + n] is not None and spec["kinds"][i] == LOSS_L1_UNC:
                    a.head[i].gunc = grads[1 + n].data_ptr()
        _lib.check(_lib.load().cf_loss_backward(C.byref(a), _lib.stream_ptr()), "cf_loss_backward")
        return (None, *grads)


def generic_loss(heat, heat_gt, centers, wh, mask, cls, heads, heat_weight=1.0, out_area=None, uncertainty=None):
    kinds, weights = [int(hd[0]) for hd in heads], [float(hd[4]) for hd in heads]
    maps = [hd[1] for hd in heads]
    spec = {"kinds": kinds, "weights": weights, "heat_weight": float(heat_weight),
            "out_area": float(out_area if out_area is not None else heat.shape[-2] * heat.shape[-1])}
    tensors = [heat, *maps, uncertainty, heat_gt, centers, wh, mask, cls]
    for hd in heads:
        tensors += [hd[2], hd[3]]
    for t in [heat, *maps, uncertainty]:
        if t is not None and (not torch.is_tensor(t) or t.dtype != torch.float32):
            raise NotImplementedError("generic_loss: float32 maps only (no autocast, no fp16 / bf16 / float64)")
    _need_cuda(*[t for t in tensors if torch.is_tensor(t)])
    if torch.is_grad_enabled() and any(t is not None and t.requires_grad for t in [heat, *maps, uncertainty]):
        return _GenericLossFn.apply(spec, *tensors)
    with torch.no_grad():
        return _loss_run_forward(spec, tensors)[:3]


HEAD_HIDDEN = 256
HEAD_MAX_OUT = 16
HEAD_MAX_HIDDEN = _lib.CF_HEAD_TRAIN_MAX_HIDDEN
HEAD_FINALS = (None, "heatmap", "depth")


def _head_check(x, x2, weights, biases, final):
    if final not in HEAD_FINALS:
        raise ValueError(f"head_stack: final must be one of {HEAD_FINALS}, got {final!r}")
    weights, biases = list(weights), list(biases)
    if len(weights) != len(biases) or not 2 <= len(weights) <= HEAD_MAX_HIDDEN + 2:
        raise NotImplementedError(f"head_stack: a 3x3 layer, 0..{HEAD_MAX_HIDDEN} hidden 1x1 layers and an output layer "
                                  f"(2..{HEAD_MAX_HIDDEN + 2} weights with their biases), got {len(weights)} / {len(biases)}")
    for t in (x, x2, *weights, *biases):
        if t is not None and (not torch.is_tensor(t) or t.dtype != torch.float32):
            raise NotImplementedError("head_stack: float32 tensors only (no autocast, no fp16 / bf16 / float64)")
    if x.dim() != 4 or (x2 is not None and (x2.dim() != 4 or x2.shape[0] != x.shape[0] or x2.shape[2:] != x.shape[2:])):
        raise ValueError("head_stack: x must be (B,Cin,h,w) and the second source (B,C2,h,w) on the same map")
    c_x, c_x2 = x.shape[1], (0 if x2 is None else x2.shape[1])
    cin = c_x + c_x2
    if cin > 512:
        raise NotImplementedError(f"head_stack: Cin={cin} above the limit of 512")
    if tuple(weights[0].shape) != (HEAD_HIDDEN, cin, 3, 3):
        raise NotImplementedError(f"head_stack: the first layer must be a 3x3 convolution ({HEAD_HIDDEN},{cin},3,3) - hidden width "
                                  f"{HEAD_HIDDEN} only - got {tuple(weights[0].shape)}")
    for w in weights[1:-1]:
        if tuple(w.shape) != (HEAD_HIDDEN, HEAD_HIDDEN, 1, 1):
            raise NotImplementedError(f"head_stack: hidden layers must be 1x1 convolutions ({HEAD_HIDDEN},{HEAD_HIDDEN},1,1), "
                                      f"got {tuple(w.shape)}")
    n_out = weights[-1].shape[0]
    if weights[-1].dim() != 4 or tuple(weights[-1].shape[1:]) != (HEAD_HIDDEN, 1, 1) or not 1 <= n_out <= HEAD_MAX_OUT:
        raise NotImplementedError(f"head_stack: the output layer must be a 1x1 convolution (Cout,{HEAD_HIDDEN},1,1) with "
                                  f"1 <= Cout <= {HEAD_MAX_OUT}, got {tuple(weights[-1].shape)}")
    for w, b in zip(weights, biases):
        if tuple(b.shape) != (w.shape[0],):
            raise ValueError(f"head_stack: bias {tuple(b.shape)} does not fit weight {tuple(w.shape)}")
    return c_x, c_x2, len(weights) - 2, n_out


def head_train_args(xn, c_x, x2n, c_x2, weights, biases, chunk_px=0) -> _lib.HeadTrainArgs:
    a = _lib.HeadTrainArgs()
    a.B, a.h, a.w = xn.shape[:3]
    a.x, a.x_stride, a.c_x = xn.data_ptr(), xn.shape[-1], c_x
    if x2n is not None:
        a.x2, a.x2_stride, a.c_x2 = x2n.data_ptr(), x2n.shape[-1], c_x2
    a.n_hidden, a.hidden, a.n_out, a.chunk_px = len(weights) - 2, HEAD_HIDDEN, weights[-1].shape[0], int(chunk_px)
    for l, (w, b) in enumerate(zip(weights, biases)):
        a.weight[l], a.bias[l] = w.data_ptr(), b.data_ptr()
    return a


def _workspace(a, nbytes):
    ws = torch.empty(nbytes, device=torch.device("cuda", torch.cuda.current_device()), dtype=torch.uint8)
    a.workspace, a.workspace_bytes = ws.data_ptr(), nbytes
    return ws


class _HeadStackFn(torch.autograd.Function):

    @staticmethod
    def forward(ctx, xn, x2n, c_x, c_x2, chunk_px, n_layers, input_grad, *params):
        weights = [p.detach().contiguous() for p in params[:n_layers]]
        biases = [p.detach().contiguous() for p in params[n_layers:]]
        B, h, w = xn.shape[:3]
        with torch.cuda.device(xn.device):
            a = head_train_args(xn, c_x, x2n, c_x2, weights, biases, chunk_px)
            y = torch.empty((B, a.n_out, h, w), device=xn.device, dtype=torch.float32)
            a.y = y.data_ptr()
            ws = _workspace(a, _lib.load().cf_head_train_workspace_bytes(B, h, w, c_x + c_x2, a.n_hidden, int(chunk_px)))
            _lib.check(_lib.load().cf_head_train_forward(C.byref(a), _lib.stream_ptr()), "cf_head_train_forward")
        ctx.meta = (c_x, c_x2, int(chunk_px), n_layers, x2n is not None, bool(input_grad))
        ctx.save_for_backward(xn, *([x2n] if x2n is not None else []), *weights, *biases)
        return y

    @staticmethod
    @torch.autograd.function.once_differentiable
    def backward(ctx, gy):
        c_x, c_x2, chunk_px, n, has2, input_grad = ctx.meta
        saved = list(ctx.saved_tensors)
        xn = saved.pop(0)
        x2n = saved.pop(0) if has2 else None
        weights, biases = saved[:n], saved[n:]
        B, h, w = xn.shape[:3]
        gy = gy.detach().to(torch.float32).contiguous()
        with torch.cuda.device(xn.device):
            a = head_train_args(xn, c_x, x2n, c_x2, weights, biases, chunk_px)
            gws = [torch.empty_like(t) for t in weights]
            gbs = [torch.empty_like(t) for t in biases]
            for l in range(n):
                a.gw[l], a.gb[l] = gws[l].data_ptr(), gbs[l].data_ptr()
            a.gy = gy.data_ptr()
            want = input_grad and ctx.needs_input_grad[0], input_grad and has2 and ctx.needs_input_grad[1]
            gx = torch.empty_like(xn) if want[0] else None
            gx2 = torch.empty_like(x2n) if want[1] else None
            if gx is None and gx2 is None:
                ws = _workspace(a, _lib.load().cf_head_bwd_workspace_bytes(B, h, w, c_x + c_x2, a.n_hidden, chunk_px))
                _lib.check(_lib.load().cf_head_backward(C.byref(a), _lib.stream_ptr()), "cf_head_backward")
            else:
                ws = _workspace(a, _lib.load().cf_head_bwd_dx_workspace_bytes(B, h, w, c_x + c_x2, a.n_hidden, chunk_px))
                _lib.check(_lib.load().cf_head_backward_dx(C.byref(a), _lib.ptr(gx), xn.shape[-1], _lib.ptr(gx2),
                                                           0 if x2n is None else x2n.shape[-1], _lib.stream_ptr()),
                           "cf_head_backward_dx")
        need = ctx.needs_input_grad[7:]
        grads = [g if nd else None for g, nd in zip(gws + gbs, need)]
        return (gx, gx2, None, None, None, None, None, *grads)


class _NchwToNhwcFn(torch.autograd.Function):

    @staticmethod
    def forward(ctx, x):
        with torch.cuda.device(x.device):
            return nchw_to_nhwc(x.detach().contiguous())

    @staticmethod
    @torch.autograd.function.once_differentiable
    def backward(ctx, g):
        with torch.cuda.device(g.device):
            return nhwc_to_nchw(g.detach().contiguous())


def head_final(y, final):
    if final == "heatmap":
        return torch.clamp(torch.sigmoid(y), min=1e-4, max=1 - 1e-4)
    if final == "depth":
        return 1.0 / (torch.sigmoid(y) + 1e-6) - 1.0
    return y


def head_stack_nhwc(xn, c_x, x2n, c_x2, weights, biases, final=None, chunk_px=0, input_grad=False):
    weights, biases = list(weights), list(biases)
    y = _HeadStackFn.apply(xn, x2n, int(c_x), int(c_x2), int(chunk_px), len(weights), bool(input_grad), *weights, *biases)
    return y if final is None else (head_final(y, final), y)


def head_stack(x, weights, biases, final=None, x2=None, chunk_px=0, input_grad=False):
    weights, biases = list(weights), list(biases)
    c_x, c_x2, _, _ = _head_check(x, x2, weights, biases, final)
    _need_cuda(x, x2, *weights, *biases)
    if not input_grad and torch.is_grad_enabled() and (x.requires_grad or (x2 is not None and x2.requires_grad)):
        raise NotImplementedError("head_stack: the gradient with respect to x is off by default (frozen trunk only): detach it, "
                                  "or pass input_grad=True")
    if int(chunk_px) < 0 or int(chunk_px) % 64:
        raise ValueError("head_stack: chunk_px must be a multiple of 64 (0: the default)")

    def to_nhwc(t):
        if input_grad and torch.is_grad_enabled() and t.requires_grad:
            return _NchwToNhwcFn.apply(t)
        with torch.no_grad(), torch.cuda.device(t.device):
            return nchw_to_nhwc(t.contiguous())

    xn = to_nhwc(x)
    x2n = None if x2 is None else to_nhwc(x2)
    return head_stack_nhwc(xn, c_x, x2n, c_x2, weights, biases, final, chunk_px, input_grad)


def upsample_dw(x, weight_kkc, f, skip=None, out=None):
    _need_cuda(x, weight_kkc, skip)
    B, H, W, Cc = x.shape
    if out is None:
        out = torch.empty((B, H * f, W * f, Cc), device=x.device, dtype=torch.float32)
    _lib.check(_lib.load().cf_upsample_dw(x.data_ptr(), weight_kkc.data_ptr(), _lib.ptr(skip),
                                          out.data_ptr(), B, H, W, Cc, f, _lib.stream_ptr()),
               "cf_upsample_dw")
    return out


def maxpool2x2(x, out=None):
    _need_cuda(x)
    B, H, W, Cc = x.shape
    if out is None:
        out = torch.empty((B, H // 2, W // 2, Cc), device=x.device, dtype=torch.float32)
    _lib.check(_lib.load().cf_maxpool2x2(x.data_ptr(), out.data_ptr(), B, H, W, Cc,
                                         _lib.stream_ptr()), "cf_maxpool2x2")
    return out


def nchw_to_nhwc4(x, out=None):
    _need_cuda(x)
    B, Cc, H, W = x.shape
    if out is None:
        out = torch.empty((B, H, W, 4), device=x.device, dtype=torch.float32)
    _lib.check(_lib.load().cf_nchw_to_nhwc4(x.data_ptr(), out.data_ptr(), B, Cc, H, W,
                                            _lib.stream_ptr()), "cf_nchw_to_nhwc4")
    return out


def nhwc_to_nchw(x, channels=None, out=None):
    _need_cuda(x)
    B, H, W, S = x.shape
    Cc = channels or S
    if out is None:
        out = torch.empty((B, Cc, H, W), device=x.device, dtype=torch.float32)
    _lib.check(_lib.load().cf_nhwc_to_nchw(x.data_ptr(), out.data_ptr(), B, H, W, Cc, S,
                                           _lib.stream_ptr()), "cf_nhwc_to_nchw")
    return out


CHECKSUM_PARTS = 256


def checksum64(t, out=None):
    _need_cuda(t)
    nbytes = t.numel() * t.element_size()
    if not t.is_contiguous() or nbytes % 4:
        raise _lib.CfHipError("checksum64: contiguous tensor of a multiple of 4 bytes")
    if out is None:
        out = torch.empty(CHECKSUM_PARTS, device=t.device, dtype=torch.int64)
    assert out.numel() == CHECKSUM_PARTS and out.dtype == torch.int64 and out.is_contiguous()
    _lib.check(_lib.load().cf_checksum64(t.data_ptr(), nbytes // 4, out.data_ptr(), _lib.stream_ptr()), "cf_checksum64")
    return out


def topk_peaks(heat, K=100, nms=False, out=None, only_if_changed=None):
    _need_cuda(heat)
    if not heat.is_contiguous():
        heat = heat.contiguous()
    B, Cc, H, W = heat.shape
    dev = heat.device
    if out is not None:
        scores, inds, classes = out
    else:
        scores = torch.empty((B, K), device=dev, dtype=torch.float32)
        inds = torch.empty((B, K), device=dev, dtype=torch.int32)
        classes = torch.empty((B, K), device=dev, dtype=torch.int32)
    lib = _lib.load()
    mode = int(nms) if nms in (0, 1, 2) and not isinstance(nms, bool) else (2 if nms else 0)
    size = lib.cf_topk_workspace_bytes_nms(B, Cc, H, W, K) if mode == 2 else lib.cf_topk_workspace_bytes(B, K)
    ws = torch.empty(max(1, size), device=dev, dtype=torch.uint8)
    if only_if_changed is not None:
        _lib.check(lib.cf_topk_peaks_if_changed(heat.data_ptr(), B, Cc, H, W, K, mode, scores.data_ptr(), inds.data_ptr(),
                                                classes.data_ptr(), ws.data_ptr(), only_if_changed.data_ptr(),
                                                _lib.stream_ptr()), "cf_topk_peaks_if_changed")
        return scores, inds, classes
    _lib.check(lib.cf_topk_peaks(heat.data_ptr(), B, Cc, H, W, K, mode,
                                 scores.data_ptr(), inds.data_ptr(), classes.data_ptr(),
                                 ws.data_ptr(), _lib.stream_ptr()), "cf_topk_peaks")
    return scores, inds, classes


def frustum_assoc(inds, depth, wh, dim, rot, calib, pc_dep, max_pc_dist=60.0, want_nhwc4=False,
                  pc_hm=None, pc_hm_nhwc4=None, pc_hm_split8=None):
    _need_cuda(inds, depth, wh, dim, rot, calib, pc_dep)
    B, _, H, W = pc_dep.shape
    K = inds.shape[1]
    dev = pc_dep.device
    if pc_hm is None:
        pc_hm = torch.empty((B, 3, H, W), device=dev, dtype=torch.float32)
    if want_nhwc4 and pc_hm_nhwc4 is None:
        pc_hm_nhwc4 = torch.empty((B, H, W, 4), device=dev, dtype=torch.float32)
    ts = [t if t.is_contiguous() else t.contiguous() for t in (depth, wh, dim, rot, calib, pc_dep)]
    _lib.check(_lib.load().cf_frustum_assoc(inds.data_ptr(), K, *(t.data_ptr() for t in ts), B, H,
                                            W, float(max_pc_dist), pc_hm.data_ptr(),
                                            _lib.ptr(pc_hm_nhwc4), _lib.ptr(pc_hm_split8),
                                            _lib.stream_ptr()),
               "cf_frustum_assoc")
    return (pc_hm, pc_hm_nhwc4) if want_nhwc4 else pc_hm


def topk_frustum(heat, depth, wh, dim, rot, calib, pc_dep, K=100, max_pc_dist=60.0, want_nhwc4=False, want_split8=False,
                 want_peaks=False):
    _need_cuda(heat, depth, wh, dim, rot, calib, pc_dep)
    B, Cc, H, W = heat.shape
    dev = heat.device
    ts = [t if t.is_contiguous() else t.contiguous() for t in (heat, depth, wh, dim, rot, calib, pc_dep)]
    pc_hm = torch.empty((B, 3, H, W), device=dev, dtype=torch.float32)
    hm4 = torch.empty((B, H, W, 4), device=dev, dtype=torch.float32) if want_nhwc4 else None
    hm8 = torch.empty((B, H, W, 2, 8), device=dev, dtype=torch.bfloat16) if want_split8 else None
    peaks = (torch.empty((B, K), device=dev, dtype=torch.float32), torch.empty((B, K), device=dev, dtype=torch.int32),
             torch.empty((B, K), device=dev, dtype=torch.int32)) if want_peaks else (None, None, None)
    lib = _lib.load()
    ws = torch.empty(max(1, lib.cf_topk_workspace_bytes(B, K)), device=dev, dtype=torch.uint8)
    _lib.check(lib.cf_topk_frustum(ts[0].data_ptr(), Cc, K, *(t.data_ptr() for t in ts[1:]), B, H, W, float(max_pc_dist),
                                   pc_hm.data_ptr(), _lib.ptr(hm4), _lib.ptr(hm8), *(_lib.ptr(t) for t in peaks),
                                   ws.data_ptr(), _lib.stream_ptr()), "cf_topk_frustum")
    out = [pc_hm] + ([hm4] if want_nhwc4 else []) + ([hm8] if want_split8 else []) + ([peaks] if want_peaks else [])
    return out[0] if len(out) == 1 else tuple(out)


def _decode_args(scores, inds, classes, maps: dict, H, W, out_hw, norm2d, det):
    _need_cuda(scores, inds, classes)
    B, K = scores.shape
    a = _lib.DecodeArgs()
    a.scores, a.inds, a.classes = scores.data_ptr(), inds.data_ptr(), classes.data_ptr()
    keep = []
    for name in ("reg", "wh", "depth", "rot", "dim", "amodal", "att", "vel"):
        t = maps.get(name)
        if t is not None and not t.is_contiguous():
            t = t.contiguous()
        keep.append(t)
        setattr(a, name, _lib.ptr(t))
    a.B, a.K, a.H, a.W = B, K, H, W
    a.out_h, a.out_w, a.norm2d = int(out_hw[0]), int(out_hw[1]), int(bool(norm2d))
    a.det = _lib.ptr(det)
    return a, keep


def _uncertainty_map(uncertainty, B, H, W):
    if uncertainty is None:
        return None
    _need_cuda(uncertainty)
    if uncertainty.dtype != torch.float32 or tuple(uncertainty.shape) != (B, 1, H, W):
        raise _lib.CfHipError(f"uncertainty must be a float32 ({B},1,{H},{W}) map, got {uncertainty.dtype} "
                              f"{tuple(uncertainty.shape)}")
    return uncertainty if uncertainty.is_contiguous() else uncertainty.contiguous()


def decode_gather(scores, inds, classes, maps: dict, H, W, out_hw, norm2d=False, uncertainty=None):
    B, K = scores.shape
    det = torch.empty((B, K, 33), device=scores.device, dtype=torch.float32)
    a, _keep = _decode_args(scores, inds, classes, maps, H, W, out_hw, norm2d, det)
    unc = _uncertainty_map(uncertainty, B, H, W)
    if unc is None:
        _lib.check(_lib.load().cf_decode_gather(C.byref(a), _lib.stream_ptr()), "cf_decode_gather")
    else:
        _lib.check(_lib.load().cf_decode_gather_unc(C.byref(a), unc.data_ptr(), _lib.stream_ptr()), "cf_decode_gather_unc")
    return det


def decode_post(scores, inds, classes, maps: dict, H, W, out_hw, calib, trans_inv, norm2d=False, want_det=False,
                uncertainty=None):
    _need_cuda(calib, trans_inv)
    B, K = scores.shape
    dev = scores.device
    det = torch.empty((B, K, 33), device=dev, dtype=torch.float32) if want_det else None
    post = torch.empty((B, K, 54), device=dev, dtype=torch.float32)
    a, _keep = _decode_args(scores, inds, classes, maps, H, W, out_hw, norm2d, det)
    if calib.dtype != torch.float32 or not calib.is_contiguous() or calib.numel() != B * 12:
        raise _lib.CfHipError("cf_decode_post: calib must be contiguous float32 (B,3,4)")
    if trans_inv.dtype != torch.float32 or not trans_inv.is_contiguous() or trans_inv.numel() != 6:
        raise _lib.CfHipError("cf_decode_post: trans_inv must be contiguous float32 (2,3)")
    unc = _uncertainty_map(uncertainty, B, H, W)
    if unc is None:
        _lib.check(_lib.load().cf_decode_post(C.byref(a), calib.data_ptr(), trans_inv.data_ptr(), post.data_ptr(),
                                              _lib.stream_ptr()), "cf_decode_post")
    else:
        _lib.check(_lib.load().cf_decode_post_unc(C.byref(a), unc.data_ptr(), calib.data_ptr(), trans_inv.data_ptr(),
                                                  post.data_ptr(), _lib.stream_ptr()), "cf_decode_post_unc")
    return (post, det) if want_det else post


def depth_maps(maps, out=None):
    maps = list(maps)
    if not 1 <= len(maps) <= _lib.CF_DEPTH_MAPS_MAX:
        raise _lib.CfHipError(f"depth_maps: 1..{_lib.CF_DEPTH_MAPS_MAX} maps, got {len(maps)}")
    _need_cuda(*maps)
    B, one, H, W = maps[0].shape
    for t in maps:
        if t.dtype != torch.float32 or tuple(t.shape) != (B, 1, H, W):
            raise _lib.CfHipError(f"depth_maps: every map must be float32 ({B},1,{H},{W}), got {t.dtype} {tuple(t.shape)}")
    keep = [t if (B == 1 or t.stride(0) >= H * W) and t.stride(2) == W and t.stride(3) == 1 else t.contiguous() for t in maps]
    if out is None:
        out = torch.empty((len(keep), B, H, W), device=keep[0].device, dtype=torch.uint8)
    assert out.dtype == torch.uint8 and out.is_contiguous() and tuple(out.shape) == (len(keep), B, H, W)
    ptrs = (_lib._f * len(keep))(*(t.data_ptr() for t in keep))
    strides = (C.c_long * len(keep))(*(max(t.stride(0), H * W) for t in keep))
    _lib.check(_lib.load().cf_depth_maps(ptrs, strides, len(keep), B, H, W, out.data_ptr(), _lib.stream_ptr()), "cf_depth_maps")
    return out


def serialize_nuscenes(post, trans_matrix, velocity_matrix, cs_rot=None, pose_rot=None, sample_ptr=None,
                       sample_frames=None, max_per_sample=500):
    _need_cuda(post, trans_matrix, velocity_matrix)
    B, K, w = post.shape
    dev = post.device
    for t, dt, n in ((post, torch.float32, B * K * 54), (trans_matrix, torch.float32, B * 16),
                     (velocity_matrix, torch.float32, B * 16)):
        if t.dtype != dt or not t.is_contiguous() or t.numel() != n:
            raise _lib.CfHipError("cf_serialize_nuscenes: wrong dtype / shape / non-contiguous input")
    a = _lib.SerializeArgs()
    a.post, a.B, a.K = post.data_ptr(), B, K
    a.trans_matrix, a.velocity_matrix = trans_matrix.data_ptr(), velocity_matrix.data_ptr()
    if (cs_rot is None) != (pose_rot is None):
        raise _lib.CfHipError("cf_serialize_nuscenes: cs_rot and pose_rot go together")
    for q in (cs_rot, pose_rot):
        if q is not None and (q.dtype != torch.float64 or not q.is_contiguous() or q.numel() != B * 4 or not q.is_cuda):
            raise _lib.CfHipError("cf_serialize_nuscenes: quaternions must be contiguous float64 (B,4) on the device")
    a.cs_rot, a.pose_rot = _lib.ptr(cs_rot), _lib.ptr(pose_rot)
    rows = torch.empty((B * K, 12), device=dev, dtype=torch.float32)
    rotation = torch.empty((B * K, 4), device=dev, dtype=torch.float64)
    a.rows, a.rotation = rows.data_ptr(), rotation.data_ptr()
    order = counts = None
    if sample_ptr is not None:
        _need_cuda(sample_ptr, sample_frames)
        if sample_ptr.dtype != torch.int32 or sample_frames.dtype != torch.int32:
            raise _lib.CfHipError("cf_serialize_nuscenes: sample tables must be int32")
        S = sample_ptr.numel() - 1
        order = torch.empty((S, max_per_sample), device=dev, dtype=torch.int32)
        counts = torch.empty((S,), device=dev, dtype=torch.int32)
        a.n_samples, a.sample_ptr, a.sample_frames = S, sample_ptr.data_ptr(), sample_frames.data_ptr()
        a.max_per_sample, a.order, a.counts = int(max_per_sample), order.data_ptr(), counts.data_ptr()
    _lib.check(_lib.load().cf_serialize_nuscenes(C.byref(a), _lib.stream_ptr()), "cf_serialize_nuscenes")
    return rows, rotation, order, counts


def _radar_expand(entry, extra, pc_2d, pc_3d, counts, calib, trans, out_hw, want_aux):
    _need_cuda(pc_2d, pc_3d, counts, calib, trans)
    B, _, max_n = pc_2d.shape
    H, W = out_hw
    dev = pc_2d.device
    pc_dep = torch.empty((B, 3, H, W), device=dev, dtype=torch.float32)
    keep = torch.empty((B, max_n), device=dev, dtype=torch.uint8) if want_aux else None
    xy = torch.empty((B, 2, max_n), device=dev, dtype=torch.float64) if want_aux else None
    for t, dt in ((pc_2d, torch.float64), (pc_3d, torch.float64), (counts, torch.int32),
                  (calib, torch.float64), (trans, torch.float64)):
        if t.dtype != dt or not t.is_contiguous():
            raise _lib.CfHipError(f"{entry}: wrong dtype / non-contiguous input")
    _lib.check(getattr(_lib.load(), entry)(pc_2d.data_ptr(), pc_3d.data_ptr(), counts.data_ptr(), B, max_n, pc_3d.shape[1],
                                           calib.data_ptr(), trans.data_ptr(), H, W, *extra, pc_dep.data_ptr(),
                                           _lib.ptr(keep), _lib.ptr(xy), _lib.stream_ptr()), entry)
    return (pc_dep, keep, xy) if want_aux else pc_dep


def pillar_expand(pc_2d, pc_3d, counts, calib, trans, out_hw, pillar_dims=(1.5, 0.2, 0.2),
                  want_aux=False):
    return _radar_expand("cf_pillar_expand", [float(v) for v in pillar_dims], pc_2d, pc_3d, counts, calib, trans, out_hw,
                         want_aux)


ROI_METHODS = {"pillars": 0, "points": 1, "heatmap": 2}


def roi_method_id(roi_method):
    if roi_method not in ROI_METHODS:
        raise ValueError(f"Invalid PC_ROI_METHOD: {roi_method}")
    return ROI_METHODS[roi_method]


def radar_roi_expand(pc_2d, pc_3d, counts, calib, trans, out_hw, roi_method, want_aux=False):
    method = roi_method_id(roi_method)
    if method == 0:
        raise ValueError("radar_roi_expand: 'pillars' is pillar_expand (it needs the pillar dimensions)")
    return _radar_expand("cf_radar_roi_expand", [method], pc_2d, pc_3d, counts, calib, trans, out_hw, want_aux)


def stem_args(ps, x, out, shape=None, out_pool=None, in_scales=None, into=None) -> _lib.StemArgs:
    a = _lib.StemArgs() if into is None else into
    B, Cc, H, W = shape if x is None else x.shape
    a.x, a.B, a.C, a.H, a.W = (_lib.ptr(x), B, Cc, H, W)
    a.w_base, a.b_base, a.scale_base = ps.w_base.data_ptr(), ps.b_base.data_ptr(), ps.scale_base
    a.w_level0, a.b_level0, a.scale_level0 = ps.w_level0.data_ptr(), ps.b_level0.data_ptr(), ps.scale_level0
    a.w_level1, a.b_level1, a.scale_level1 = ps.w_level1.data_ptr(), ps.b_level1.data_ptr(), ps.scale_level1
    a.out = out.data_ptr()
    a.out_pool = _lib.ptr(out_pool)
    if in_scales is not None:
        for i, (s, name) in enumerate(zip(in_scales, ("scale_base", "scale_level0", "scale_level1"))):
            if s is not None and float(s) != DEFAULT_IN_SCALE:
                a.in_scale[i] = float(s)
                setattr(a, name, _scaled_out_scale(getattr(a, name), s, "stem_args"))
    return a


def stem_fused(ps, x, out=None, out_pool=None, in_scales=None):
    _need_cuda(x, out_pool)
    B, Cc, H, W = x.shape
    if out is None:
        out = torch.empty((B, H // 2, W // 2, 32), device=x.device, dtype=torch.float32)
    a = stem_args(ps, x.contiguous(), out, out_pool=out_pool, in_scales=in_scales)
    _lib.check(_lib.load().cf_stem_fused(C.byref(a), _lib.stream_ptr()), "cf_stem_fused")
    return out


def stem_early_args(ps, x, pc, out, shape=None, out_pool=None, in_scales=None) -> _lib.StemEarlyArgs:
    assert ps.w_base_radar is not None, "weights packed without the radar part (packing.pack_stem_early)"
    e = _lib.StemEarlyArgs()
    stem_args(ps, x, out, shape=shape, out_pool=out_pool, in_scales=in_scales, into=e.stem)
    e.pc = _lib.ptr(pc)
    e.pc_h, e.pc_w = (e.stem.H // 4, e.stem.W // 4) if pc is None else pc.shape[2:]
    e.w_base_radar = ps.w_base_radar.data_ptr()
    return e


def stem_fused_early(ps, x, pc, out=None, out_pool=None, in_scales=None):
    _need_cuda(x, pc, out_pool)
    B, Cc, H, W = x.shape
    if pc.dim() != 4 or pc.shape[0] != B or pc.shape[1] != 3 or pc.dtype != torch.float32:
        raise _lib.CfHipError(f"stem_fused_early: the radar map must be float32 (B, 3, H/4, W/4), got {tuple(pc.shape)}")
    if out is None:
        out = torch.empty((B, H // 2, W // 2, 32), device=x.device, dtype=torch.float32)
    a = stem_early_args(ps, x.contiguous(), pc.contiguous(), out, out_pool=out_pool, in_scales=in_scales)
    _lib.check(_lib.load().cf_stem_fused_early(C.byref(a), _lib.stream_ptr()), "cf_stem_fused_early")
    return out


def radar_ingest(pc, counts, intrinsics, img_wh, max_dist=60.0, z_offset=0.0, descending=False):
    _need_cuda(pc, counts, intrinsics)
    for t, dt in ((pc, torch.float64), (counts, torch.int32), (intrinsics, torch.float64)):
        if t.dtype != dt or not t.is_contiguous():
            raise _lib.CfHipError("cf_radar_ingest: wrong dtype / non-contiguous input")
    B, R, max_n = pc.shape
    pc_2d = torch.empty((B, 3, max_n), device=pc.device, dtype=torch.float64)
    pc_3d = torch.empty((B, R, max_n), device=pc.device, dtype=torch.float64)
    cnt = torch.empty((B,), device=pc.device, dtype=torch.int32)
    _lib.check(_lib.load().cf_radar_ingest(pc.data_ptr(), counts.data_ptr(), B, R, max_n, intrinsics.data_ptr(),
                                           int(img_wh[0]), int(img_wh[1]), float(max_dist), float(z_offset),
                                           int(bool(descending)), pc_2d.data_ptr(), pc_3d.data_ptr(), cnt.data_ptr(),
                                           _lib.stream_ptr()), "cf_radar_ingest")
    return pc_2d, pc_3d, cnt
```

### centerfusiondetect3d_amd/plan.py

```python
import ctypes as C
import weakref
from typing import Dict, List

import torch

from . import _lib, ops, packing
from .pending import PendingOutputs
from ._lib import (ACT_NONE, ACT_RELU, ACT_SIGMOID_CLAMP, ACT_RAW_AND_SIGDEPTH, LAYOUT_NHWC, LAYOUT_NCHW)
from .streams import _side_streams

SECONDARY_HEADS = ["velocity", "nuscenes_att", "depth2", "rotation2"]
AT_SLOTS = 18
AT_TIMED = ("at.topk", "at.peaks", "at.tables", "at.primary")


def feat_operand(model):
    if not model._heads_bf():
        return None
    return ((packing.MX_ROW,), torch.uint8) if model._mx_active else ((2, 64), torch.bfloat16)


def act_of(h):
    return ACT_SIGMOID_CLAMP if h == "heatmap" else (ACT_RAW_AND_SIGDEPTH if h in ("depth", "depth2") else ACT_NONE)

# ... 32 lines not shown
        self.tk_scores = self.tk_inds = self.tk_cls = self.tk_ws = None
        self.pk_ws = self.ev_peaks = None
        self.at, self.at_tails, self.group_flops, self.group_srcs, self._last = None, {}, {}, {}, None
        self.feat, self.feat_in = feat, feat_in
        self._m, self._pk = model, model._packed
        try:
            if part != "heads":
                self._build_trunk()
            if part != "trunk":
                self._build_heads()
        finally:
            self._m = self._pk = None

    def _buf(self, *shape, dtype=torch.float32):
        t = torch.empty(shape, device=self.device, dtype=dtype)
        self.bytes += t.numel() * t.element_size()
        self.keep.append(t)
        return t

    def _add(self, name, flops, step, *keep):
        self.keep += keep
        self.step_index[name] = len(self.steps)
        if flops is not None:
            self.step_flops[name] = flops
        self.add_step(step)
        return len(self.steps) - 1

    def _slot(self):
        self.add_step(None)
        return len(self.steps) - 1

    def _conv(self, name, srcs, h, w, act=ACT_RELU, residual=None, out=None, out_stride=None):
        m, B, pc = self._m, self.B, self._pk[name]
        ho = (h + 2 * pc.pad - pc.kh) // pc.stride + 1
        wo = (w + 2 * pc.pad - pc.kh) // pc.stride + 1
        if out is None:
            out = self._buf(B, ho, wo, pc.n)
        a = ops.conv_args(pc, srcs, [s.shape[-1] for s in srcs], B, h, w, out, out_stride or pc.n, act, residual,
                          residual.shape[-1] if residual is not None else 0, LAYOUT_NHWC, None, 0, m.precise,
                          in_scale=m._scale(name) if pc.out_scale > 0 else None)
        self.inputs[name] = list(srcs)
        fn = self.lib.cf_conv2d_fused
        if pc.out_scale > 0:
            fn = self.lib.cf_conv3x3_f16x3 if (pc.patch and m.conv_patch) else self.lib.cf_conv2d_f16x3
        self._add(name, 2.0 * B * ho * wo * pc.n * (pc.kh * pc.kh * sum(int(c) for c in pc.real_cin)), (fn, C.byref(a)), a)
        return out

    def _pool(self, x):
        if x.data_ptr() in self._pooled:
            return self._pooled[x.data_ptr()]
        _, h, w, c = x.shape
        o = self._buf(self.B, h // 2, w // 2, c)
        self.add_step((self.lib.cf_maxpool2x2, x.data_ptr(), o.data_ptr(), self.B, h, w, c))
        self._pooled[x.data_ptr()] = o
        return o

    def _block(self, p, x, residual, pooled=None):
        m, B = self._m, self.B
        _, h, w, _ = x.shape
        t = self._conv(p + ".conv1", [x], h, w)
        _, ho, wo, _ = t.shape
        if pooled is None:
            return self._conv(p + ".conv2", [t], ho, wo, residual=residual if residual is not None else x)
        pc = self._pk[p + ".conv2"]
        o = self._buf(B, ho, wo, pc.n)
        a = ops.conv_args(pc, [t, pooled], [t.shape[-1], pooled.shape[-1]], B, ho, wo, o, pc.n, ACT_RELU, None, 0,
                          LAYOUT_NHWC, None, 0, False, in_scale=m._scale(p + ".conv2"))
        self.inputs[p + ".conv2"], self.inputs[p[:-len(".tree1")] + ".project"] = [t], [pooled]
        ch = (C.c_int32 * 2)(*[int(c) for c in pc.real_cin])
        step = (self.lib.cf_conv3x3_proj_f16x3, C.byref(a), ch) if m.conv_patch else (self.lib.cf_conv2d_f16x3, C.byref(a))
        self._add(p + ".conv2+project", 2.0 * B * ho * wo * pc.n * (9 * pc.real_cin[0] + pc.real_cin[1]), step, a, ch)
        return o

    def _tree(self, p, levels, x, stride, level_root, children=None):
        m, B, pk = self._m, self.B, self._pk
        children = [] if children is None else children
        bottom = self._pool(x) if stride > 1 else x
        proj_fused = levels == 1 and getattr(pk[p + ".tree1.conv2"], "proj_k", 0) > 0
        if proj_fused:
            residual = None
        elif (p + ".project") in pk:
            _, h, w, _ = bottom.shape
            residual = self._conv(p + ".project", [bottom], h, w, act=ACT_NONE)
        else:
            residual = bottom
        if level_root:
            children.append(bottom)
        if levels > 1:
            x1 = self._tree(p + ".tree1", levels - 1, x, stride, False)
            children.append(x1)
            return self._tree(p + ".tree2", levels - 1, x1, 1, False, children)
        x1 = self._block(p + ".tree1", x, residual, pooled=bottom if proj_fused else None)
        _, h, w, _ = x1.shape
        pc2, pcr = pk[p + ".tree2.conv2"], pk[p + ".root"]
        if not (m.root_fuse and m.conv_patch and pc2.out_scale > 0 and pcr.out_scale > 0
                and getattr(pc2, "patch", False) and pc2.stride == 1 and (not children or m.root_fuse_children)):
            x2 = self._block(p + ".tree2", x1, None)
            return self._conv(p + ".root", [x2, x1, *children], h, w)
        t = self._conv(p + ".tree2.conv1", [x1], h, w)
        x2, o = self._buf(B, h, w, pc2.n), self._buf(B, h, w, pcr.n)
        a2 = ops.conv_args(pc2, [t], [t.shape[-1]], B, h, w, x2, pc2.n, ACT_RELU, x1, x1.shape[-1],
                           LAYOUT_NHWC, None, 0, False, in_scale=m._scale(p + ".tree2.conv2"))
        rsrcs = [x2, x1, *children]
        ar = ops.conv_args(pcr, rsrcs, [s_.shape[-1] for s_ in rsrcs], B, h, w, o, pcr.n, ACT_RELU, None, 0,
                           LAYOUT_NHWC, None, 0, False, in_scale=m._scale(p + ".root"))
        self.inputs[p + ".tree2.conv2"], self.inputs[p + ".root"] = [t], [x1, *children]
        self.hidden.add(p + ".root")
        rch = (C.c_int32 * len(rsrcs))(*[int(c) for c in pcr.real_cin])
        flops = 2.0 * B * h * w * (pc2.n * 9 * sum(int(c) for c in pc2.real_cin) + pcr.n * sum(int(c) for c in pcr.real_cin))
        self._add(p + ".tree2.conv2+root", flops, (self.lib.cf_conv3x3_root_f16x3, C.byref(a2), C.byref(ar), rch), a2, ar, rch)
        return o

    def _dcn_node(self, p, x, out=None, feat_producer=False):
        m, B = self._m, self.B
        _, h, w, c = x.shape
        om = self._buf(B, h, w, 32)
        self._conv(p + ".conv_offset_mask", [x], h, w, act=ACT_NONE, out=om, out_stride=32)
        pd = self._pk[p]
        o = self._buf(B, h, w, pd.n) if out is None else out
        ws = None
        if pd.out_scale > 0:
            nbytes = self.lib.cf_dcn_v2_workspace_bytes(B, h, w, pd.c, pd.n_pad)
            ws = self._buf(nbytes, dtype=torch.uint8) if nbytes else None
        a = ops.dcn_args(pd, x, om, 32, B, h, w, o, pd.n, ACT_RELU, precise=m.precise, workspace=ws,
                         in_scale=m._scale(p) if pd.out_scale > 0 else None)
        if feat_producer:
            self.feat_producer = a
        self.inputs[p] = [x]
        fn = self.lib.cf_dcn_v2_f16x3 if pd.out_scale > 0 else self.lib.cf_dcn_v2_fused
        self._add(p, 2.0 * B * h * w * pd.n * 9 * pd.c, (fn, C.byref(a)), a)
        return o

    def _dcn_group(self, members):
        m, B, G = self._m, self.B, len(members)
        _, h, w, c = members[0][1].shape
        pd0 = self._pk[members[0][0]]
        om = self._buf(G, B, h, w, 32)
        out = self._buf(G, B, h, w, pd0.n)
        nbytes = self.lib.cf_dcn_v2_workspace_bytes(B, h, w, pd0.c, pd0.n_pad)
        ws = self._buf(G * nbytes, dtype=torch.uint8) if nbytes else None
        ca, da, flops_c, flops_d = [], [], 0.0, 0.0
        for g, (name, x) in enumerate(members):
            pc, pd = self._pk[name + ".conv_offset_mask"], self._pk[name]
            ca.append(ops.conv_args(pc, [x], [c], B, h, w, om[g], 32, ACT_NONE, None, 0, LAYOUT_NHWC, None, 0, m.precise,
                                    in_scale=m._scale(name + ".conv_offset_mask")))
            da.append(ops.dcn_args(pd, x, om[g], 32, B, h, w, out[g], pd.n, ACT_RELU, precise=m.precise, workspace=ws,
                                   in_scale=m._scale(name)))
            self.inputs[name + ".conv_offset_mask"], self.inputs[name] = [x], [x]
            flops_c += 2.0 * B * h * w * pc.n * 9 * sum(int(v) for v in pc.real_cin)
            flops_d += 2.0 * B * h * w * pd.n * 9 * pd.c
        cp, dp = ops.group_ptrs(ca), ops.group_ptrs(da)
        for name, _ in members[1:]:
            self.step_index[name + ".conv_offset_mask"], self.step_index[name] = len(self.steps), len(self.steps) + 1
            self.step_flops[name + ".conv_offset_mask"] = self.step_flops[name] = 0.0
        first = members[0][0]
        self._add(first + ".conv_offset_mask", flops_c, (self.lib.cf_conv3x3_f16x3_grouped, cp, G), cp, ca)
        self._add(first, flops_d, (self.lib.cf_dcn_v2_f16x3_grouped, dp, G), dp, da)
        return [out[g] for g in range(G)]

    def _groupable(self, name, x):
        m, pc, pd = self._m, self._pk[name + ".conv_offset_mask"], self._pk[name]
        ok = pc.out_scale > 0 and getattr(pc, "patch", False) and m.conv_patch and pc.n_pad == 32 and \
            pd.out_scale > 0 and pd.n % 4 == 0 and pd.n_pad <= 128
        return (tuple(x.shape), pc.k_pad, pd.c, pd.n, pd.n_pad) if ok else None

    def _ida(self, p, layers, startp, endp, final_out=None, feat=False, also=()):
        projs = {}
        if self._m.neck_groups and not self.use_lanes:
            sets = {}
            for name, x in [(f"{p}.proj_{i - startp}", layers[i]) for i in range(startp + 1, endp)] + list(also):
                key = self._groupable(name, x) if name not in self._pre else None
                if key is not None:
                    sets.setdefault(key, []).append((name, x))
            for members in sets.values():
                for k in range(0, len(members), _lib.CF_MAX_GROUPS):
                    part = members[k:k + _lib.CF_MAX_GROUPS]
                    if len(part) > 1:
                        self._pre.update(zip([n for n, _ in part], self._dcn_group(part)))
        if self.use_lanes:
            self.ctl("rec", 0, ev0 := self.new_event())
            self.ctl("wait", 1, ev0)
            self.lane = 1
            for i in range(startp + 1, endp):
                projs[i] = self._dcn_node(f"{p}.proj_{i - startp}", layers[i])
                self.ctl("rec", 1, ev := self.new_event())
                projs[i] = (projs[i], ev)
            self.lane = 0
        for i in range(startp + 1, endp):
            j = i - startp
            if self.use_lanes:
                proj, ev = projs[i]
                self.ctl("wait", 0, ev)
            elif f"{p}.proj_{j}" in self._pre:
                proj = self._pre.pop(f"{p}.proj_{j}")
            else:
                proj = self._dcn_node(f"{p}.proj_{j}", layers[i])
            wk, f = self._pk[f"{p}.up_{j}"]
            _, h, w, c = proj.shape
            summed = self._buf(self.B, h * f, w * f, c)
            self.add_step((self.lib.cf_upsample_dw, proj.data_ptr(), wk.data_ptr(),
                           layers[i - 1].data_ptr(), summed.data_ptr(), self.B, h, w, c, f))
            layers[i] = self._dcn_node(f"{p}.node_{j}", summed, out=final_out if i == endp - 1 else None,
                                       feat_producer=feat and i == endp - 1)

    def _build_trunk(self):
        m, B, H, W, pk = self._m, self.B, self.H, self.W, self._pk
        if self.early and self.part == "all":
            self.direct_step = self._add("pc_hm_direct", 0.0, None)
        if "base.stem" in pk:
            y0, y1 = None, self._buf(B, H // 2, W // 2, 32)
            y1p = self._buf(B, H // 4, W // 4, 32) if m.stem_pool else None
            if y1p is not None:
                self._pooled[y1.data_ptr()] = y1p
            stem_layers = ("base.base_layer", "base.level0", "base.level1")
            kw = dict(shape=(B, 3, H, W), out_pool=y1p, in_scales=[m._scale(n) for n in stem_layers])
            self.stem = ops.stem_early_args(pk["base.stem"], None, None, y1, **kw) if self.early else \
                ops.stem_args(pk["base.stem"], None, y1, **kw)
            self.hidden.update(stem_layers)
            k_base = 16 * 49 * (6 if self.early else 3)
            self.in_step = self._add("base.stem", 2.0 * B * H * W * (k_base + 16 * 144 + 32 * 144 / 4), None, self.stem)
        else:
            self.in_step = self._slot()
            self.x4 = self._buf(B, H, W, 8 if self.early else 4)
            if self.early:
                self.x4.zero_()
            t = self._conv("base.base_layer", [self.x4], H, W)
            y0 = self._conv("base.level0", [t], H, W)
            y1 = self._conv("base.level1", [y0], H, W)
        layers = [y0, y1]
        for lvl, levels, root in ((2, 1, False), (3, 2, True), (4, 2, True), (5, 1, True)):
            layers.append(self._tree(f"base.level{lvl}", levels, layers[-1], 2, root))
        self.debug = {f"y{i}": t for i, t in enumerate(layers) if t is not None}
        out = [layers[-1]]
        n_ida = len(layers) - 2 - 1
        for i in range(n_ida):
            also = [("ida_up.proj_1", layers[-1])] if i == n_ida - 1 and i > 0 else []
            self._ida(f"dla_up.ida_{i}", layers, len(layers) - i - 2, len(layers), also=also)
            out.insert(0, layers[-1])
        for i, t in enumerate(out):
            self.debug[f"up{i}"] = t
        y = out[:3]
        self._ida("ida_up", y, 0, 3, final_out=self.feat, feat=True)
        feat = self.feat = y[-1]
        spec, pr, M4 = feat_operand(m), self.feat_producer, B * self.h4 * self.w4
        if spec is None:
            self.feat_in = feat
            return
        if self.feat_in is None:
            self.feat_in = self._buf(B, self.h4, self.w4, *spec[0], dtype=spec[1])
        if m._mx_active:
            if pr.out_scale > 0 and pr.N == 64 and pr.N_pad == 64 and bool(m.pack_mx_fused):
                pr.out_mx = self.feat_in.data_ptr()
                pr.mx_scale = m._feat_scale
                pr.workspace = None
            else:
                self._add("feat.pack_mx", None, (self.lib.cf_pack_feat_mx_scaled, feat.data_ptr(), 64, self.feat_in.data_ptr(),
                                                 C.c_long(M4), C.c_float(m._feat_scale)))
        elif pr.out_scale > 0 and pr.N == 64:
            pr.out_split_bf16, pr.split_stride = self.feat_in.data_ptr(), 64
            pr.workspace = None
        else:
            self.add_step((self.lib.cf_split_bf16, feat.data_ptr(), self.feat_in.data_ptr(), M4, 64, 64, 64))

    def _hconv(self, name, srcs, strides, out_c=None, out=None, out_offset=0):
        B, h4, w4, pc = self.B, self.h4, self.w4, self._pk[name]
        if out is None:
            out = self._buf(B, h4, w4, out_c)
        a = ops.conv_args(pc, srcs, strides, B, h4, w4, out, out.shape[-1], ACT_RELU, None, 0, LAYOUT_NHWC, None, out_offset, False, 4)
        flops = 2.0 * B * h4 * w4 * pc.n * (pc.kh * pc.kh * sum(int(c) for c in pc.real_cin))
        self._add(name, flops, (self.lib.cf_conv2d_fused, C.byref(a)), a)
        return out

    def _head_out(self, h, src, src_stride):
        B, h4, w4, act, pc = self.B, self.h4, self.w4, act_of(h), self._pk[f"heads.{h}.out"]
        a = ops.conv_args(pc, [src], [src_stride], B, h4, w4, src, 0, act, None, 0,
                          LAYOUT_NCHW, src if act == ACT_RAW_AND_SIGDEPTH else None, 0, False)
        self._add(f"heads.{h}.out", 2.0 * B * h4 * w4 * pc.n * 256, (self.lib.cf_conv2d_fused, C.byref(a)), a)
        self.outs[h] = a

    def _head_block(self, name, names, srcs, strides):
        B, h4, w4, heads = self.B, self.h4, self.w4, self._m.config.heads
        hd = [dict(self._pk[name][h], act=act_of(h)) for h in names]
        f = ops.head_fused_args(srcs, strides, hd[0].get("slots"), hd[0].get("k_pad", 0), B, h4, w4, hd)
        self.keep.append(f)
        return f, sum(2.0 * 256 * (9 * sum(d["real_cin"]) + 256 * len(d["w_hidden"]) + heads[h]) for h, d in zip(names, hd))

    def _fused_heads(self, name, names, srcs, strides):
        f, px_flops = self._head_block(name, names, srcs, strides)
        for n, h in enumerate(names):
            self.tails[h] = (f.tail, n)
        flops = self.B * self.h4 * self.w4 * px_flops
        self.group_flops[name] = (flops, px_flops, f)
        self.group_srcs[name] = list(srcs)
        self._add(name, flops, (self.lib.cf_head_fused, C.byref(f)), f)

    def _build_at(self, feat_in):
        B, K, primary = self.B, self.K, self.primary
        f_hm, px_hm = self._head_block("tails.primary", primary[:1], [feat_in], [64])
        f_rest, px_rest = self._head_block("tails.primary", primary[1:], [feat_in], [64])
        self.at_tails = {primary[0]: (f_hm.tail, 0), **{h: (f_rest.tail, n) for n, h in enumerate(primary[1:])}}
        tiles_b, tiles_ab = -(-K // AT_SLOTS), -(-2 * K // AT_SLOTS)
        self.at = dict(f_hm=f_hm, flops_hm=B * self.h4 * self.w4 * px_hm, f_rest=f_rest, px_rest=px_rest,
                       tab_b=self._buf(B * tiles_b * AT_SLOTS, dtype=torch.int32), n_b=B * tiles_b,
                       tab_ab=self._buf(B * tiles_ab * AT_SLOTS, dtype=torch.int32) if self.frustum else None, n_ab=B * tiles_ab)

    def _peaks_lane(self):
        ev_a = self.new_event()
        self.ctl("rec", 0, ev_a)
        self.lane = 1
        self.ctl("wait", 1, ev_a)
        n_cls = self._m.config.heads["heatmap"]
        self.pk_ws = self._buf(max(1, self.lib.cf_topk_workspace_bytes_nms(self.B, n_cls, self.h4, self.w4, self.K)), dtype=torch.uint8)
        self.peaks_step = self._slot()
        self.ev_peaks = self.new_event()
        self.ctl("rec", 1, self.ev_peaks)
        self.lane = 0

    def _chained_heads(self, bf, feat, feat_in):
        B, h4, w4, chained = self.B, self.h4, self.w4, self.chained
        if bf:
            src = feat_in
            if self._m._mx_active:
                src = self.feat_bf = self._buf(B, h4, w4, 2, 64, dtype=torch.bfloat16)
                self._add("feat.split_bf16", None, (self.lib.cf_split_bf16, feat.data_ptr(), src.data_ptr(), C.c_long(B * h4 * w4), 64, 64, 64))
            self._fused_heads("tails.chained", chained, [src], [64])
            return
        ss = 256 * len(chained)
        s1 = self._hconv("heads.secondary.0", [feat_in], [64], out_c=ss)
        s2 = self._buf(B, h4, w4, ss)
        for n, h in enumerate(chained):
            self._hconv(f"heads.{h}.2", [s1], [ss], out=s2, out_offset=256 * n)
            self._hconv(f"heads.{h}.4", [s2], [ss], out=s1, out_offset=256 * n)
            self._head_out(h, s1, ss)

    def _build_heads(self):
        m, B, h4, w4, K = self._m, self.B, self.h4, self.w4, self.K
        feat, feat_in = self.feat, self.feat_in
        radar = m.isRadarEnabled and m.fusionStrategy == "middle"
        frustum = radar and m.isFrustumEnabled
        bf = m._heads_bf()
        chained = [h for h in m.config.heads if len(m.config.head_conv[h]) == 3] if self.early else []
        primary = [h for h in m.config.heads if not (radar and h in SECONDARY_HEADS) and h not in chained]
        self.primary, self.radar, self.frustum, self.chained = primary, radar, frustum, chained
        if feat is not None:
            self.inputs["heads.primary.0"] = [feat]
            if radar:
                self.inputs["heads.secondary.0"] = [feat]
        split = bf and bool(m.heads_lanes) and primary[0] == "heatmap"
        if split:
            self.use_lanes = True
        if bf:
            self._fused_heads("tails.primary", primary, [feat_in], [64])
            if split and not (frustum and m.peaks_behind_frustum):
                self._peaks_lane()
        else:
            hs = 256 * len(primary)
            hid = self._hconv("heads.primary.0", [feat_in], [64], out_c=hs)
            for h in primary:
                self._head_out(h, hid, hs)
        if chained:
            self._chained_heads(bf, feat, feat_in)
        if radar:
            self.pc_hm4 = None if bf else self._buf(B, h4, w4, 4)
            self.pc_hm8 = self._buf(B, h4, w4, 2, 8, dtype=torch.bfloat16) if bf else None
            if frustum:
                self.tk_scores = self._buf(B, K)
                self.tk_inds = self._buf(B, K, dtype=torch.int32)
                self.tk_cls = self._buf(B, K, dtype=torch.int32)
                self.tk_ws = self._buf(max(1, self.lib.cf_topk_workspace_bytes(B, K)), dtype=torch.uint8)
                if not m.frustum_fused:
                    self.topk_step = self._slot()
                self.frustum_step = self._slot()
            else:
                self.frustum_step = self._add("pc_hm_direct", 0.0, None)
            if split and self.peaks_step is None:
                self._peaks_lane()
            if bf:
                self._fused_heads("tails.secondary", SECONDARY_HEADS, [feat_in, self.pc_hm8], [64, 8])
            else:
                ss = 256 * len(SECONDARY_HEADS)
                s1 = self._hconv("heads.secondary.0", [feat_in, self.pc_hm4], [64, 4], out_c=ss)
                s2 = self._buf(B, h4, w4, ss)
                for n, h in enumerate(SECONDARY_HEADS):
                    self._hconv(f"heads.{h}.2", [s1], [ss], out=s2, out_offset=256 * n)
                    self._hconv(f"heads.{h}.4", [s2], [ss], out=s1, out_offset=256 * n)
                    self._head_out(h, s1, ss)
        if split:
            self.ctl("wait", 0, self.ev_peaks)
        if split and len(primary) > 1:
            self._build_at(feat_in)

    def add_step(self, step):
        self.steps.append(step)
        self.lanes.append(self.lane)

    def ctl(self, op, lane, ev):
        self.steps.append((op, ev))
        self.lanes.append(lane)

    def new_event(self):
        self.n_events += 1
        return self.n_events - 1

    @staticmethod
    def _timed_call(ev, step, st, stream):
        e0, e1 = torch.cuda.Event(enable_timing=True), torch.cuda.Event(enable_timing=True)
        e0.record(stream)
        rc = step[0](*step[1:], st)
        e1.record(stream)
        ev.append((e0, e1))
        return rc

    def _launch(self, st, seq=None):
        lanes_on = self.use_lanes and not torch.cuda.is_current_stream_capturing()
        timed = self.timed
        if seq is None:
            seq = zip(range(len(self.steps)), self.steps, self.lanes)
        if not lanes_on:
            for i, step, _ in seq:
                if isinstance(step[0], str):
                    continue
                ev = timed.get(i) if timed else None
                rc = step[0](*step[1:], st) if ev is None else self._timed_call(ev, step, st, None)
                if rc != 0:
                    _lib.check(rc, step[0].__name__)
            return
        cur = torch.cuda.current_stream(self.device)
        if self._side is None:
            self._side = _side_streams(self.device, cur.cuda_stream, 1)[0]
            self._events = [torch.cuda.Event() for _ in range(self.n_events)]
        streams = (cur, self._side)
        ptrs = (st, self._side.cuda_stream)
        for i, step, lane in seq:
            op = step[0]
            if op == "rec":
                self._events[step[1]].record(streams[lane])
            elif op == "wait":
                streams[lane].wait_event(self._events[step[1]])
            else:
                ev = timed.get(i) if timed else None
                rc = op(*step[1:], ptrs[lane]) if ev is None else self._timed_call(ev, step, ptrs[lane], streams[lane])
                if rc != 0:
                    _lib.check(rc, op.__name__)

    def _patch_input(self, x, pc=None):
        if self.early and self.stem is not None:
            self.stem.stem.x, self.stem.pc = x.data_ptr(), pc.data_ptr()
            self.steps[self.in_step] = (self.lib.cf_stem_fused_early, C.byref(self.stem))
        elif self.early:
            self.steps[self.in_step] = (_early_input, x, pc, self.x4)
        elif self.stem is not None:
            self.stem.x = x.data_ptr()
            self.steps[self.in_step] = (self.lib.cf_stem_fused, C.byref(self.stem))
        else:
            self.steps[self.in_step] = (self.lib.cf_nchw_to_nhwc4, x.data_ptr(), self.x4.data_ptr(), self.B, 3, self.H, self.W)

    def run_trunk(self, x, pc=None):
        self._patch_input(x, pc)
        self._launch(_lib.stream_ptr())

    def _radar_outputs(self, y, out, heads, pc_dep, pc_hm):
        y["pc_hm_in"] = pc_dep[:, :1]
        y["pc_hm"] = pc_hm[:, 0, :, :].unsqueeze(1)
        for h in SECONDARY_HEADS:
            y[h] = out(h, heads[h])
        y["pc_hm_out"] = pc_hm[:, :1]
        y["depthMap"] = y["depth2"]
        y["depth2"] = out("depth2", 1, second=True)

    def run(self, model, x, pc_dep, calib, alloc=None):
        B, dev, lib, K = self.B, self.device, self.lib, self.K
        st = _lib.stream_ptr()
        h4, w4 = self.h4, self.w4
        heads = model.config.heads
        self.flush_pending()
        at = self.at if (self.at is not None and getattr(model, "heads_at_peaks", True)
                         and not torch.cuda.is_current_stream_capturing()) else None
        y, written = {}, []
        new = alloc or (lambda c: torch.empty((B, c, h4, w4), device=dev, dtype=torch.float32))

        def out(h, c, second=False):
            t = new(c)
            written.append(t)
            if h in self.tails:
                a, n = self.tails[h]
                (a.out2 if second else a.out)[n] = t.data_ptr()
                if h in self.at_tails:
                    a, n = self.at_tails[h]
                    (a.out2 if second else a.out)[n] = t.data_ptr()
            elif second:
                self.outs[h].out2 = t.data_ptr()
            else:
                self.outs[h].out = t.data_ptr()
            return t

        for h in self.primary + self.chained:
            y[h] = out(h, heads[h])
        depth_raw = y["depth"]
        y["depthMap"] = depth_raw
        y["depth"] = out("depth", 1, second=True)
        y["calib"] = calib
        hm = y["heatmap"]
        if self.peaks_step is not None:
            peaks_on = not torch.cuda.is_current_stream_capturing()
            if peaks_on:
                pk_s = torch.empty((B, K), device=dev, dtype=torch.float32)
                pk_i = torch.empty((B, K), device=dev, dtype=torch.int32)
                pk_c = torch.empty((B, K), device=dev, dtype=torch.int32)
                pk_sum = torch.empty(2 * ops.CHECKSUM_PARTS, device=dev, dtype=torch.int64)
                n_words = B * heads["heatmap"] * h4 * w4
                peaks = (_peaks_and_checksum, lib, (hm.data_ptr(), B, heads["heatmap"], h4, w4, K, 2,
                         pk_s.data_ptr(), pk_i.data_ptr(), pk_c.data_ptr(), self.pk_ws.data_ptr()),
                         (hm.data_ptr(), C.c_long(n_words), pk_sum.data_ptr()))
                self.steps[self.peaks_step] = peaks if at is None else (_no_launch,)
            else:
                self.steps[self.peaks_step] = (_no_launch,)
        if self.direct_step is not None:
            self.steps[self.direct_step] = (lib.cf_pc_hm_direct, pc_dep.data_ptr(), B, h4, w4,
                                            C.c_float(float(model.config.DATASET.MAX_PC_DIST)), None, None)
        if self.in_step is not None:
            self._patch_input(x, pc_dep)
        if self.radar:
            max_dist = C.c_float(float(model.config.DATASET.MAX_PC_DIST))
            maps = (_lib.ptr(self.pc_hm4), _lib.ptr(self.pc_hm8))
            if not self.frustum:
                pc_hm = pc_dep
                self.steps[self.frustum_step] = (lib.cf_pc_hm_direct, pc_dep.data_ptr(), B, h4, w4, max_dist, *maps)
            else:
                pc_hm = new(3)
                geom = (y["depth"].data_ptr(), y["widthHeight"].data_ptr(), y["dimension"].data_ptr(), y["rotation"].data_ptr(),
                        calib.data_ptr(), pc_dep.data_ptr(), B, h4, w4, max_dist, pc_hm.data_ptr(), *maps)
                tk = (self.tk_scores.data_ptr(), self.tk_inds.data_ptr(), self.tk_cls.data_ptr(), self.tk_ws.data_ptr())
                if at is not None:
                    if self.topk_step is not None:
                        self.steps[self.topk_step] = (_no_launch,)
                    self.steps[self.frustum_step] = (lib.cf_frustum_assoc, self.tk_inds.data_ptr(), K, *geom)
                elif self.topk_step is None:
                    self.steps[self.frustum_step] = (lib.cf_topk_frustum, hm.data_ptr(), heads["heatmap"], K, *geom, *tk)
                else:
                    self.steps[self.topk_step] = (lib.cf_topk_peaks, hm.data_ptr(), B, heads["heatmap"], h4, w4, K, 0, *tk)
                    self.steps[self.frustum_step] = (lib.cf_frustum_assoc, self.tk_inds.data_ptr(), K, *geom)
            self._radar_outputs(y, out, heads, pc_dep, pc_hm)
        for name, (flops, px_flops, _) in self.group_flops.items():
            self.step_flops[name] = flops
        if at is None:
            self._launch(st)
        else:
            topk = (lib.cf_topk_peaks, hm.data_ptr(), B, heads["heatmap"], h4, w4, K, 0, *tk) if self.frustum else None
            self._launch(st, self._at_seq(at, peaks, topk, pk_i))
            y = self._pending(y, model, written)
        if self.peaks_step is not None and peaks_on:
            hm._cf_peaks = (K, hm.data_ptr(), pk_s, pk_i, pk_c, pk_sum)
            if self._side is not None:
                for t in (hm, pk_s, pk_i, pk_c, pk_sum):
                    t.record_stream(self._side)
        return [y]

    def _at_seq(self, at, peaks, topk, pk_i):
        lib, idx = self.lib, self.step_index
        tab_b, n_b = at["tab_b"].data_ptr(), at["n_b"]
        tab_p, n_p = (at["tab_ab"].data_ptr(), at["n_ab"]) if self.frustum else (tab_b, n_b)
        HP_PX = 128
        extra = ([("at.topk", topk, 0)] if topk is not None else []) + [("at.peaks", peaks, 0)]
        extra += [
                  ("at.tables", (lib.cf_head_slot_tables, self.tk_inds.data_ptr() if self.frustum else None, pk_i.data_ptr(),
                                 self.B, self.K, self.h4 * self.w4, at["tab_ab"].data_ptr() if self.frustum else None, tab_b), 0),
                  ("at.primary", (lib.cf_head_fused_at, C.byref(at["f_rest"]), tab_p, n_p), 0)]
        repl = {idx["tails.primary"]: (lib.cf_head_fused, C.byref(at["f_hm"]))}
        self.step_flops["tails.primary"] = at["flops_hm"]
        self.step_flops["at.primary"] = n_p * HP_PX * at["px_rest"]
        for name in ("tails.chained", "tails.secondary"):
            if name in idx:
                _, px_flops, f = self.group_flops[name]
                repl[idx[name]] = (lib.cf_head_fused_at, C.byref(f), tab_b, n_b)
                self.step_flops[name] = n_b * HP_PX * px_flops
        seq = []
        for i, (step, lane) in enumerate(zip(self.steps, self.lanes)):
            seq.append((i, repl.get(i, step), lane))
            if i == idx["tails.primary"]:
                seq += extra
        return seq

    def _pending(self, y, model, written):
        fwd = torch.cuda.current_stream(self.device)
        lib, dev = self.lib, self.device
        names = [n for n in ("tails.primary", "tails.chained", "tails.secondary") if n in self.step_index]
        blocks = []
        for n in names:
            f = self.group_flops[n][2]
            c = _lib.HeadFusedArgs()
            C.memmove(C.byref(c), C.byref(f), C.sizeof(f))
            blocks.append(c)
        bufs = {t.data_ptr(): t for n in names for t in self.group_srcs[n]}
        keep = [written, list(y.values()), self, model._packed, bufs]

        def materialise():
            with torch.cuda.device(dev):
                for c in blocks:
                    rc = lib.cf_head_fused(C.byref(c), fwd.cuda_stream)
                    if rc != 0:
                        _lib.check(rc, "cf_head_fused")
                rd = torch.cuda.current_stream(dev)
                if rd != fwd:
                    rd.wait_stream(fwd)
            keep.clear()

        def release():
            with torch.cuda.device(dev), torch.cuda.stream(fwd):
                for ptr, t in list(bufs.items()):
                    snap = t.clone()
                    for c in blocks:
                        for i in range(c.n_src):
                            if c.src[i] == ptr:
                                c.src[i] = snap.data_ptr()
                    bufs[ptr] = snap
            keep[2] = None

        p = PendingOutputs(y, materialise, model._lock, release)
        self._last = weakref.ref(p)
        return p

    def flush_pending(self):
        last, self._last = (self._last() if self._last is not None else None), None
        if last is not None:
            last.release()


def _early_input(x, pc, x8, stream):
    x8[..., :3].copy_(x.permute(0, 2, 3, 1))
    x8[..., 3:6].copy_(pc.permute(0, 2, 3, 1).repeat_interleave(4, dim=1).repeat_interleave(4, dim=2))
    return 0


def _no_launch(stream):
    return 0


def _peaks_and_checksum(lib, topk_args, sum_args, stream):
    rc = lib.cf_topk_peaks(*topk_args, stream)
    return rc if rc != 0 else lib.cf_checksum64(*sum_args, stream)
```

### include/cf_hip.h

```cpp
#ifndef CF_HIP_H
#define CF_HIP_H

#include <stddef.h>
#include <stdint.h>

#ifdef __cplusplus
extern "C" {
#endif

#define CF_ABI_VERSION 7

#define CF_OK 0
#define CF_EINVAL (-22)
#define CF_ELAUNCH (-5)

#define CF_MAX_SRC 4
#define CF_MAX_GROUPS 4

#define CF_ACT_NONE 0
#define CF_ACT_RELU 1
#define CF_ACT_SIGMOID_CLAMP 2
#define CF_ACT_RAW_AND_SIGDEPTH 3

#define CF_LAYOUT_NHWC 0
#define CF_LAYOUT_NCHW 1

typedef struct cf_slot {
  int32_t src;
  int32_t dy;
  int32_t dx;
  int32_t c_off;
} cf_slot;

typedef struct cf_conv_args {
  const float* src[CF_MAX_SRC];
  int32_t src_c[CF_MAX_SRC];
  int32_t n_src;
  int32_t B, H, W;
  int32_t Ho, Wo;
  int32_t stride;
  const float* weight;
  const cf_slot* slots;
  const float* bias;
  int32_t K_pad;
  int32_t N;
  int32_t N_pad;
  const float* residual;
  int32_t res_stride;
  float* out;
  float* out2;
  int32_t out_stride;
  int32_t out_layout;
  int32_t act;
  int32_t precise;
  float out_scale;
  float in_scale;
} cf_conv_args;
int cf_conv2d_fused(const cf_conv_args* a, void* stream);

typedef struct cf_stem_args {
  const float* x;
  int32_t B, C, H, W;
  const void* w_base;   const float* b_base;   float scale_base;
  const void* w_level0; const float* b_level0; float scale_level0;
  const void* w_level1; const float* b_level1; float scale_level1;
  float* out;
  float* out_pool;
  float in_scale[3];
} cf_stem_args;
int cf_stem_fused(const cf_stem_args* a, void* stream);

typedef struct cf_stem_early_args {
  cf_stem_args stem;
  const float* pc;
  int32_t pc_h, pc_w;
  const void* w_base_radar;
} cf_stem_early_args;
int cf_stem_fused_early(const cf_stem_early_args* a, void* stream);

int cf_conv2d_f16x3(const cf_conv_args* a, void* stream);

int cf_conv3x3_f16x3(const cf_conv_args* a, void* stream);

int cf_conv3x3_root_f16x3(const cf_conv_args* conv, const cf_conv_args* root, const int32_t* root_channels, void* stream);

int cf_conv3x3_proj_f16x3(const cf_conv_args* a, const int32_t* src_channels, void* stream);

int cf_conv3x3_f16x3_grouped(const cf_conv_args* const* groups, int32_t n_groups, void* stream);
int cf_conv3x3_grouped_form(const cf_conv_args* const* groups, int32_t n_groups, int32_t* form);

typedef struct cf_pack_src {
  int32_t channels;
  int32_t stride;
  int32_t c_base;
} cf_pack_src;
typedef struct cf_pack_bn {
  const float* gamma; const float* beta; const float* mean; const float* var;
  float eps;
} cf_pack_bn;
typedef struct cf_pack_conv_desc {
  const float* weight;
  const float* bias;
  cf_pack_bn bn;
  int32_t cout, kh, kw, stride;
  int32_t pad;
  int32_t dilation;
  const cf_pack_src* src; int32_t n_src;
  const float* proj_weight;
  const float* proj_bias;
  cf_pack_bn proj_bn;
  cf_pack_src proj;
} cf_pack_conv_desc;
typedef struct cf_pack_info {
  int32_t n_pad, k_pad;
  int32_t n_slots;
  int32_t patch;
  float out_scale;
  size_t weight_bytes;
} cf_pack_info;
int cf_pack_conv_f16x3_info(const cf_pack_conv_desc* d, cf_pack_info* info);
int cf_pack_conv_f16x3(const cf_pack_conv_desc* d, void* weight_out, cf_slot* slots_out, float* bias_out, cf_pack_info* info);
int cf_pack_dcn_f16_info(int32_t cout, int32_t cin, cf_pack_info* info);
int cf_pack_dcn_f16(const float* weight, const float* bias, const cf_pack_bn* bn, int32_t cout, int32_t cin,
                    void* weight_out, float* bias_out, cf_pack_info* info);

int cf_split_bf16(const float* x, void* out, long M, int C, int in_stride, int Cs, void* stream);

#define CF_MAX_HEADS 12
typedef struct cf_head_tail_args {
  const void* x;
  int32_t x_stride;
  int32_t B, H, W;
  int32_t n_heads;
  int32_t n_hidden;
  const void* w_hidden[CF_MAX_HEADS][2];
  const float* b_hidden[CF_MAX_HEADS][2];
  const void* w_out[CF_MAX_HEADS];
  const float* b_out[CF_MAX_HEADS];
  float* out[CF_MAX_HEADS];
  float* out2[CF_MAX_HEADS];
  int32_t c_base[CF_MAX_HEADS];
  int32_t n_out[CF_MAX_HEADS];
  int32_t act[CF_MAX_HEADS];
} cf_head_tail_args;

typedef struct cf_head_fused_args {
  cf_head_tail_args tail;
  const void* src[2];
  int32_t src_c[2];
  int32_t n_src;
  const cf_slot* slots;
  int32_t K_pad;
  const void* w_first[CF_MAX_HEADS];
  const float* b_first[CF_MAX_HEADS];
  int32_t layout3x3;
  const void* w_out_perm[CF_MAX_HEADS];
  int32_t mfma16;
  int32_t mx;
  float first_scale[CF_MAX_HEADS];
} cf_head_fused_args;
int cf_head_fused(const cf_head_fused_args* a, void* stream);
int cf_head_fused_with(const cf_head_fused_args* a, int tile, int pc_skip, void* stream);

int cf_head_fused_at(const cf_head_fused_args* a, const int32_t* slot_pixels, int n_tiles, void* stream);
int cf_head_slot_tables(const int32_t* list_a, const int32_t* list_b, int B, int K, int HW, int32_t* table_ab,
                        int32_t* table_b, void* stream);

int cf_pack_feat_mx(const float* x, int in_stride, void* rows, long M, void* stream);
int cf_pack_feat_mx_scaled(const float* x, int in_stride, void* rows, long M, float scale, void* stream);

typedef struct cf_dcn_args {
  const float* x;
  const float* offmask;
  int32_t om_stride;
  int32_t B, H, W, C;
  const float* weight;
  const float* bias;
  int32_t N, N_pad;
  float* out;
  int32_t out_stride;
  int32_t act;
  int32_t precise;
  float out_scale;
  void* out_split_bf16;
  int32_t split_stride;
  void* workspace;
  size_t workspace_bytes;
  int32_t mask_activated;
  void* out_mx;
  float in_scale;
  float mx_scale;
} cf_dcn_args;
int cf_dcn_v2_fused(const cf_dcn_args* a, void* stream);

int cf_dcn_v2_f16x3(const cf_dcn_args* a, void* stream);
size_t cf_dcn_v2_workspace_bytes(int B, int H, int W, int C, int N_pad);

int cf_dcn_v2_f16x3_grouped(const cf_dcn_args* const* groups, int32_t n_groups, void* stream);

int cf_gemm_tile_form(long M, int N, int N_pad, int out_layout, int act, int precise, int dcn,
                      int32_t* kind, int32_t* bm, int32_t* bn);

typedef struct cf_dcn_bwd_args {
  const float* gout;
  const float* weight;
  const float* x;
  const float* offmask;
  int32_t B, H, W, C, N;
  float* gx;
  float* gom;
  float* gw;
  float* gbias;
  void* workspace;
  size_t workspace_bytes;
} cf_dcn_bwd_args;
int cf_dcn_v2_bwd_data(const cf_dcn_bwd_args* a, void* stream);
int cf_dcn_v2_bwd_weight(const cf_dcn_bwd_args* a, void* stream);
size_t cf_dcn_v2_bwd_workspace_bytes(int B, int H, int W, int C, int N);

int cf_upsample_dw(const float* x, const float* weight, const float* skip, float* out, int B,
                   int H, int W, int C, int f, void* stream);

int cf_maxpool2x2(const float* x, float* out, int B, int H, int W, int C, void* stream);

int cf_nchw_to_nhwc4(const float* x, float* out, int B, int C, int H, int W, void* stream);

int cf_nhwc_to_nchw(const float* x, float* out, int B, int H, int W, int C, int c_stride,
                    void* stream);

int cf_nchw_to_nhwc(const float* x, float* out, int B, int C, int H, int W, int out_stride, int out_offset,
                    void* stream);

int cf_radar_ingest(const double* pc, const int32_t* counts_in, int B, int n_rows, int max_n,
                    const double* intrinsics, int img_w, int img_h, double max_dist, double z_offset,
                    int descending, double* pc_2d, double* pc_3d, int32_t* counts_out, void* stream);

int cf_preprocess_images(const uint8_t* src, int B, int Hs, int Ws, const double* map_dst_to_src,
                         const float* mean, const float* stdv, int Hd, int Wd, float* out, void* stream);

size_t cf_augment_workspace_bytes(int B, int Hd, int Wd);
int cf_augment_images(const uint8_t* src, int B, int Hs, int Ws, const double* map_dst_to_src, const uint8_t* flip,
                      const int32_t* order, const float* factor, const float* lighting, const float* mean, const float* stdv,
                      int colour, int Hd, int Wd, float* out, void* workspace, size_t workspace_bytes, void* stream);

size_t cf_topk_workspace_bytes(int B, int K);
size_t cf_topk_workspace_bytes_nms(int B, int C, int H, int W, int K);
#define CF_CHECKSUM_PARTS 256
int cf_checksum64(const void* x, long n_words, unsigned long long* parts, void* stream);
int cf_topk_peaks_if_changed(const float* heat, int B, int C, int H, int W, int K, int nms, float* scores, int32_t* inds,
                             int32_t* classes, void* workspace, const unsigned long long* sums, void* stream);
int cf_topk_peaks(const float* heat, int B, int C, int H, int W, int K, int nms, float* scores,
                  int32_t* inds, int32_t* classes, void* workspace, void* stream);

int cf_frustum_assoc(const int32_t* inds, int K, const float* depth, const float* wh,
                     const float* dim, const float* rot, const float* calib, const float* pc_dep,
                     int B, int H, int W, float max_pc_dist, float* pc_hm, float* pc_hm_nhwc4,
                     void* pc_hm_split8, void* stream);

int cf_topk_frustum(const float* heat, int C, int K, const float* depth, const float* wh, const float* dim,
                    const float* rot, const float* calib, const float* pc_dep, int B, int H, int W, float max_pc_dist,
                    float* pc_hm, float* pc_hm_nhwc4, void* pc_hm_split8, float* scores, int32_t* inds, int32_t* classes,
                    void* workspace, void* stream);

int cf_pc_hm_direct(float* pc_dep, int B, int H, int W, float max_pc_dist, float* pc_hm_nhwc4, void* pc_hm_split8,
                    void* stream);

int cf_pillar_expand(const double* pc_2d, const double* pc_3d, const int32_t* counts, int B,
                     int max_n, int n_rows, const double* calib, const double* trans, int H, int W,
                     double pillar_h, double pillar_w, double pillar_l, float* pc_dep,
                     uint8_t* keep_mask, double* xy_out, void* stream);

int cf_radar_roi_expand(const double* pc_2d, const double* pc_3d, const int32_t* counts, int B, int max_n,
                        int n_rows, const double* calib, const double* trans, int H, int W, int method,
                        float* pc_dep, uint8_t* keep_mask, double* xy_out, void* stream);

typedef struct cf_decode_args {
  const float* scores;
  const int32_t* inds;
  const int32_t* classes;
  const float *reg, *wh, *depth, *rot, *dim, *amodal, *att, *vel;
  int32_t B, K, H, W;
  int32_t out_h, out_w;
  int32_t norm2d;
  float* det;
} cf_decode_args;
int cf_decode_gather(const cf_decode_args* a, void* stream);

int cf_post_process(const float* det, const float* calib, const float* trans_inv, int B, int K,
                    int out_h, int out_w, float* out, void* stream);

int cf_decode_post(const cf_decode_args* a, const float* calib, const float* trans_inv, float* post,
                   void* stream);

int cf_decode_gather_unc(const cf_decode_args* a, const float* uncertainty, void* stream);
int cf_decode_post_unc(const cf_decode_args* a, const float* uncertainty, const float* calib, const float* trans_inv,
                       float* post, void* stream);

#define CF_DEPTH_MAPS_MAX 8
int cf_depth_maps(const float* const* maps, const long* batch_strides, int n_maps, int B, int H, int W, uint8_t* out,
                  void* stream);

typedef struct cf_serialize_args {
  const float* post;
  int32_t B, K;
  const float* trans_matrix;
  const float* velocity_matrix;
  const double* cs_rot;
  const double* pose_rot;
  float* rows;
  double* rotation;
  int32_t n_samples;
  const int32_t* sample_ptr;
  const int32_t* sample_frames;
  int32_t max_per_sample;
  int32_t* order;
  int32_t* counts;
} cf_serialize_args;
int cf_serialize_nuscenes(const cf_serialize_args* a, void* stream);
int cf_serialize_max_candidates(void);

#define CF_LOSS_MAX_HEADS 16
#define CF_LOSS_L1 0
#define CF_LOSS_L1_UNC 1
#define CF_LOSS_BINROT 2
#define CF_LOSS_BCE 3
#define CF_LOSS_STATS (4 + 4 * CF_LOSS_MAX_HEADS)

typedef struct cf_loss_head {
  int32_t kind;
  int32_t channels;
  const float* map;
  const float* target;
  const float* mask;
  const int64_t* rotbin;
  const float* unc;
  float weight;
  float* gmap;
  float* gunc;
} cf_loss_head;

typedef struct cf_loss_args {
  const float* heat;
  const float* heat_gt;
  const float* centers;
  const float* wh;
  const float* mask;
  const int64_t* cls;
  int32_t B, C, h, w, M;
  int32_t n_heads;
  float out_area;
  float heat_weight;
  cf_loss_head head[CF_LOSS_MAX_HEADS];
  float* losses;
  float* total;
  uint8_t* layer_mask;
  float* stats;
  void* workspace;
  size_t workspace_bytes;
  const float* grad_out;
  float* gheat;
} cf_loss_args;
int cf_loss_forward(const cf_loss_args* a, void* stream);
int cf_loss_backward(const cf_loss_args* a, void* stream);
size_t cf_loss_workspace_bytes(int B, int C, int h, int w);

#define CF_HEAD_TRAIN_MAX_HIDDEN 2
typedef struct cf_head_train_args {
  const float* x;
  const float* x2;
  int32_t x_stride, c_x, x2_stride, c_x2;
  int32_t B, h, w;
  int32_t n_hidden;
  int32_t hidden;
  int32_t n_out;
  int32_t chunk_px;
  const float* weight[CF_HEAD_TRAIN_MAX_HIDDEN + 2];
  const float* bias[CF_HEAD_TRAIN_MAX_HIDDEN + 2];
  float* y;
  const float* gy;
  float* gw[CF_HEAD_TRAIN_MAX_HIDDEN + 2];
  float* gb[CF_HEAD_TRAIN_MAX_HIDDEN + 2];
  void* workspace;
  size_t workspace_bytes;
} cf_head_train_args;
int cf_head_train_forward(const cf_head_train_args* a, void* stream);
int cf_head_backward(const cf_head_train_args* a, void* stream);
size_t cf_head_train_workspace_bytes(int B, int h, int w, int Cin, int n_hidden, int chunk_px);
size_t cf_head_bwd_workspace_bytes(int B, int h, int w, int Cin, int n_hidden, int chunk_px);
int cf_head_bwd_chunk_px(int B, int h, int w, int chunk_px);
int cf_head_backward_dx(const cf_head_train_args* a, float* gx, int gx_stride, float* gx2, int gx2_stride, void* stream);
size_t cf_head_bwd_dx_workspace_bytes(int B, int h, int w, int Cin, int n_hidden, int chunk_px);

#define CF_TARGETS_MAX_OBJS 128
#define CF_TARGETS_F 20
#define CF_TARGETS_DESC_BYTES 112
#define CF_TARGETS_HAS_AMODAL 1
#define CF_TARGETS_HAS_ATTRIBUTES 2
#define CF_TARGETS_HAS_VELOCITY 4
#define CF_TARGETS_HAS_ALPHA 8
#define CF_TARGETS_HAS_DEPTH 16
#define CF_TARGETS_HAS_DIMENSION 32
#define CF_TARGETS_HAS_LOCATION 64
#define CF_TARGETS_HAS_YAW 128
#define CF_TARGETS_REP3D 1
#define CF_TARGETS_NORM2D 2
#define CF_TARGETS_WRITE_DEPTH 4
#define CF_TARGETS_WRITE_ROT 8
#define CF_TARGETS_FRUSTUM 16

typedef struct cf_targets_args {
  const double* ann;
  const int32_t* iann;
  const int32_t* counts;
  const double* trans;
  const float* calib;
  const double* scale;
  const float* pc_dep;
  int32_t B, M, C, h, w;
  int32_t flags;
  float max_pc_dist;
  float* heat;
  int64_t* cls;
  float* mask;
  float* trunc_mask;
  float* wh;
  float* reg;
  float* amodal_offset;
  float* dimension;
  float* depth;
  int64_t* rotbin;
  float* rotres;
  float* att;
  float* att_mask;
  float* velocity;
  float* pc_hm;
  float* t_bboxes;
  float* t_scores;
  float* t_centers;
  float* t_heat_centers;
  float* t_bboxes3d;
  float* t_rotation;
  float* t_att;
  float* t_velocity;
  void* workspace;
  size_t workspace_bytes;
} cf_targets_args;
int cf_targets_build(const cf_targets_args* a, void* stream);
size_t cf_targets_workspace_bytes(int B, int M);


int cf_absmax_f32(const float* x, long M, int C, int stride, float* out, void* stream);

int cf_spin_us(int microseconds, void* stream);

const char* cf_last_error(void);
int cf_abi_version(void);

#ifdef __cplusplus
}
#endif
#endif
```

Before: 3017 frames/s.

## Fuse raw/NMS top-k peaks with slot-table build; skip dead columns in AT heads

Adds a fused top-k kernel that computes the raw and NMS peak sets in one pass over the heatmap, holding values in registers. A merge kernel then writes the scores, indices and head slot tables directly. This replaces three separate launches (topk, peaks, slot tables). Separately, the slot-table head path now issues MFMAs, LDS loads and stores only for the column tiles that hold live slot pixels (every third tile), skipping work on dead columns. The HP_PX accounting constant also changes from 128 to 48.

```diff
diff --git a/centerfusiondetect3d_amd/_lib.py b/centerfusiondetect3d_amd/_lib.py
--- a/centerfusiondetect3d_amd/_lib.py
+++ b/centerfusiondetect3d_amd/_lib.py
@@ -208,6 +208,8 @@
     "cf_topk_workspace_bytes": (C.c_size_t, [_i, _i]),
     "cf_topk_workspace_bytes_nms": (C.c_size_t, [_i, _i, _i, _i, _i]),
     "cf_topk_peaks": (_i, [_f, _i, _i, _i, _i, _i, _i, _f, _f, _f, _f, _f]),
+    "cf_topk_peaks_fused_workspace_bytes": (C.c_size_t, [_i, _i, _i, _i, _i]),
+    "cf_topk_peaks_fused": (_i, [_f, _i, _i, _i, _i, _i, _f, _f, _f, _f, _f, _f, _f, _f, _f, _f]),
     "cf_topk_peaks_if_changed": (_i, [_f, _i, _i, _i, _i, _i, _i, _f, _f, _f, _f, _f, _f]),
     "cf_checksum64": (_i, [_f, C.c_long, _f, _f]),
     "cf_frustum_assoc": (_i, [_f, _i, _f, _f, _f, _f, _f, _f, _i, _i, _i, C.c_float, _f, _f, _f, _f]),
diff --git a/centerfusiondetect3d_amd/csrc/cf_heads.hip b/centerfusiondetect3d_amd/csrc/cf_heads.hip
--- a/centerfusiondetect3d_amd/csrc/cf_heads.hip
+++ b/centerfusiondetect3d_amd/csrc/cf_heads.hip
@@ -44,7 +44,7 @@
   return reinterpret_cast<const bf16x8*>(base + (unsigned)lane * 16u);
 }
 
-template <bool SCALED = false>
+template <bool SCALED = false, int CTS = 0xF>
 __device__ __forceinline__ void store_hidden_tile16(unsigned char* xt, const f32x4 (&acc)[4][4], const float* bias,
                                                     int wave, int lane, float sc = 1.0f, int pxcol = -1) {
   const int g = lane >> 4, c16 = pxcol < 0 ? (lane & 15) : pxcol;
@@ -54,6 +54,7 @@
     const f32x4 bb = *reinterpret_cast<const f32x4*>(bias + ch);
 #pragma unroll
     for (int ct = 0; ct < 4; ++ct) {
+      if (!((CTS >> ct) & 1)) continue;
       float v[4], hi[4];
 #pragma unroll
       for (int e = 0; e < 4; ++e) {
@@ -80,7 +81,7 @@
   }
 };
 
-constexpr int AT_SLOTS = 18;
+constexpr int AT_SLOTS = CF_HEAD_AT_SLOTS;
 __device__ __forceinline__ int at_slot_of(int ty, int tx) { return (ty % 3 == 0 && tx % 3 == 0) ? (ty / 3) * 6 + tx / 3 : -1; }
 struct SlotMap {
   const int* slots;
@@ -96,7 +97,7 @@
   }
 };
 
-template <class PixMap>
+template <class PixMap, int CTS = 0xF>
 __device__ __forceinline__ void head_tail_from_lds16(const HeadTailK& p, unsigned char* xt, int head, const PixMap& pm) {
   const int tid = threadIdx.x, lane = tid & 63, wave = tid >> 6;
   const int g = lane >> 4, c16 = lane & 15;
@@ -128,6 +129,7 @@
       bf16x8 xh[4], xl[4];
 #pragma unroll
       for (int ct = 0; ct < 4; ++ct) {
+        if (!((CTS >> ct) & 1)) continue;
         const unsigned char* row = xt + (ct * 16 + c16) * HT_ROWB + (ks * 32 + g * 8) * 2;
         xh[ct] = *reinterpret_cast<const bf16x8*>(row);
         xl[ct] = *reinterpret_cast<const bf16x8*>(row + HT_PLANE);
@@ -136,21 +138,21 @@
       for (int rt = 0; rt < 4; ++rt)
 #pragma unroll
         for (int ct = 0; ct < 4; ++ct)
-          acc[rt][ct] = __builtin_amdgcn_mfma_f32_16x16x32_bf16(wl[ks & 1][rt], xh[ct], acc[rt][ct], 0, 0, 0);
+          if ((CTS >> ct) & 1) acc[rt][ct] = __builtin_amdgcn_mfma_f32_16x16x32_bf16(wl[ks & 1][rt], xh[ct], acc[rt][ct], 0, 0, 0);
 #pragma unroll
       for (int rt = 0; rt < 4; ++rt)
 #pragma unroll
         for (int ct = 0; ct < 4; ++ct)
-          acc[rt][ct] = __builtin_amdgcn_mfma_f32_16x16x32_bf16(wh[ks & 1][rt], xl[ct], acc[rt][ct], 0, 0, 0);
+          if ((CTS >> ct) & 1) acc[rt][ct] = __builtin_amdgcn_mfma_f32_16x16x32_bf16(wh[ks & 1][rt], xl[ct], acc[rt][ct], 0, 0, 0);
 #pragma unroll
       for (int rt = 0; rt < 4; ++rt)
 #pragma unroll
         for (int ct = 0; ct < 4; ++ct)
-          acc[rt][ct] = __builtin_amdgcn_mfma_f32_16x16x32_bf16(wh[ks & 1][rt], xh[ct], acc[rt][ct], 0, 0, 0);
+          if ((CTS >> ct) & 1) acc[rt][ct] = __builtin_amdgcn_mfma_f32_16x16x32_bf16(wh[ks & 1][rt], xh[ct], acc[rt][ct], 0, 0, 0);
       __builtin_amdgcn_sched_barrier(0);
     }
     __syncthreads();
-    store_hidden_tile16(xt, acc, bias, wave, lane);
+    store_hidden_tile16<false, CTS>(xt, acc, bias, wave, lane);
     __syncthreads();
   }
 
@@ -167,6 +169,7 @@
       const bf16x8 ah = *wfrag(w, 0, ks, 0, 8, lane), al = *wfrag(w, 0, ks, 1, 8, lane);
 #pragma unroll
       for (int ct = 0; ct < 4; ++ct) {
+        if (!((CTS >> ct) & 1)) continue;
         const unsigned char* row = xt + (ct * 16 + c16) * HT_ROWB + (ks * 32 + g * 8) * 2;
         const bf16x8 xh = *reinterpret_cast<const bf16x8*>(row);
         const bf16x8 xl = *reinterpret_cast<const bf16x8*>(row + HT_PLANE);
@@ -184,7 +187,7 @@
 #pragma unroll
     for (int r = 0; r < 4; ++r) {
       const int n = 4 * g + r;
-      if (n < n_out) red[(wave * 16 + n) * HT_PX + ct * 16 + c16] = oacc[ct][r];
+      if (((CTS >> ct) & 1) && n < n_out) red[(wave * 16 + n) * HT_PX + ct * 16 + c16] = oacc[ct][r];
     }
   __syncthreads();
   const float* bo = p.b_out[head];
@@ -259,6 +262,7 @@
   rem -= b * per_img;
   const int y0 = (rem / q.tiles_x) * T_H, x0 = (rem % q.tiles_x) * T_W;
   const int* const at_slots = AT ? q.slot_pixels + (size_t)rem * AT_SLOTS : nullptr;
+  constexpr auto live = [](int ct) { return !AT || ct % 3 == 0; };
   auto at_src = [&](int row) -> int {
     const int pr = row / P_W, pc = row % P_W;
     if (pr >= 9) return -1;
@@ -384,6 +388,7 @@
       bf16x8 xh[4], xl[4];
 #pragma unroll
       for (int ct = 0; ct < 4; ++ct) {
+        if (!live(4 * hf + ct)) continue;
         const unsigned char* r = pcimg + imgb + (4 * hf + ct) * (16 * 2 * HP_PCIMG_ROWB);
         xh[ct] = *reinterpret_cast<const bf16x8*>(r);
         xl[ct] = *reinterpret_cast<const bf16x8*>(r + HP_PCIMG_ROWB);
@@ -392,17 +397,20 @@
       for (int rt = 0; rt < 4; ++rt)
 #pragma unroll
         for (int ct = 0; ct < 4; ++ct)
-          acc[rt][4 * hf + ct] = __builtin_amdgcn_mfma_f32_16x16x32_bf16(al[rt], xh[ct], acc[rt][4 * hf + ct], 0, 0, 0);
+          if (live(4 * hf + ct))
+            acc[rt][4 * hf + ct] = __builtin_amdgcn_mfma_f32_16x16x32_bf16(al[rt], xh[ct], acc[rt][4 * hf + ct], 0, 0, 0);
 #pragma unroll
       for (int rt = 0; rt < 4; ++rt)
 #pragma unroll
         for (int ct = 0; ct < 4; ++ct)
-          acc[rt][4 * hf + ct] = __builtin_amdgcn_mfma_f32_16x16x32_bf16(ah[rt], xl[ct], acc[rt][4 * hf + ct], 0, 0, 0);
+          if (live(4 * hf + ct))
+            acc[rt][4 * hf + ct] = __builtin_amdgcn_mfma_f32_16x16x32_bf16(ah[rt], xl[ct], acc[rt][4 * hf + ct], 0, 0, 0);
 #pragma unroll
       for (int rt = 0; rt < 4; ++rt)
 #pragma unroll
         for (int ct = 0; ct < 4; ++ct)
-          acc[rt][4 * hf + ct] = __builtin_amdgcn_mfma_f32_16x16x32_bf16(ah[rt], xh[ct], acc[rt][4 * hf + ct], 0, 0, 0);
+          if (live(4 * hf + ct))
+            acc[rt][4 * hf + ct] = __builtin_amdgcn_mfma_f32_16x16x32_bf16(ah[rt], xh[ct], acc[rt][4 * hf + ct], 0, 0, 0);
     }
   };
   auto first_layer = [&](int head, f32x4 (&acc)[4][8]) __attribute__((always_inline)) {
@@ -449,18 +457,21 @@
     auto main_half = [&](const hf16x8 (&A)[4], int off, int hf) {
       hf16x8 xb[4];
 #pragma unroll
-      for (int ct = 0; ct < 4; ++ct) xb[ct] = *reinterpret_cast<const hf16x8*>(xt + rowb[4 * hf + ct] + off);
+      for (int ct = 0; ct < 4; ++ct)
+        if (live(4 * hf + ct)) xb[ct] = *reinterpret_cast<const hf16x8*>(xt + rowb[4 * hf + ct] + off);
 #pragma unroll
       for (int rt = 0; rt < 4; ++rt)
 #pragma unroll
         for (int ct = 0; ct < 4; ++ct)
-          acc[rt][4 * hf + ct] = __builtin_amdgcn_mfma_f32_16x16x32_f16(A[rt], xb[ct], acc[rt][4 * hf + ct], 0, 0, 0);
+          if (live(4 * hf + ct))
+            acc[rt][4 * hf + ct] = __builtin_amdgcn_mfma_f32_16x16x32_f16(A[rt], xb[ct], acc[rt][4 * hf + ct], 0, 0, 0);
     };
     auto cross_pair = [&](int toff, int pr) {
       i32x8 xb[2];
       int sb[2];
 #pragma unroll
       for (int c2 = 0; c2 < 2; ++c2) {
+        if (!live(2 * pr + c2)) continue;
         const unsigned char* r = xt + rowb[2 * pr + c2] + toff;
         const u32x4 b0 = *reinterpret_cast<const u32x4*>(r + 64 * g + 32);
         const u32x2 b1 = *reinterpret_cast<const u32x2*>(r + 64 * g + 48);
@@ -471,7 +482,7 @@
       {                                                                                                                 \
         const i32x8 a6 = {(int)ax0[RT][0], (int)ax0[RT][1], (int)ax0[RT][2], (int)ax0[RT][3], (int)ax1[RT][0],          \
                           (int)ax1[RT][1], 0, 0};                                                                       \
-        _Pragma("unroll") for (int c2 = 0; c2 < 2; ++c2)                                                                \
+        _Pragma("unroll") for (int c2 = 0; c2 < 2; ++c2) if (live(2 * pr + c2))                                         \
           acc[RT][2 * pr + c2] = __builtin_amdgcn_mfma_scale_f32_16x16x128_f8f6f4(a6, xb[c2], acc[RT][2 * pr + c2],    \
                                                                                   2, 2, RT, sa, 0, sb[c2]);             \
       }
@@ -539,6 +550,7 @@
       bf16x8 xh[4], xl[4];
 #pragma unroll
       for (int ct = 0; ct < 4; ++ct) {
+        if (!live(4 * hf + ct)) continue;
         xh[ct] = *reinterpret_cast<const bf16x8*>(xt + rowb[4 * hf + ct] + off);
         xl[ct] = *reinterpret_cast<const bf16x8*>(xt + rowb[4 * hf + ct] + off + lo);
       }
@@ -546,17 +558,20 @@
       for (int rt = 0; rt < 4; ++rt)
 #pragma unroll
         for (int ct = 0; ct < 4; ++ct)
-          acc[rt][4 * hf + ct] = __builtin_amdgcn_mfma_f32_16x16x32_bf16(wl[ks & 1][rt], xh[ct], acc[rt][4 * hf + ct], 0, 0, 0);
+          if (live(4 * hf + ct))
+            acc[rt][4 * hf + ct] = __builtin_amdgcn_mfma_f32_16x16x32_bf16(wl[ks & 1][rt], xh[ct], acc[rt][4 * hf + ct], 0, 0, 0);
 #pragma unroll
       for (int rt = 0; rt < 4; ++rt)
 #pragma unroll
         for (int ct = 0; ct < 4; ++ct)
-          acc[rt][4 * hf + ct] = __builtin_amdgcn_mfma_f32_16x16x32_bf16(wh[ks & 1][rt], xl[ct], acc[rt][4 * hf + ct], 0, 0, 0);
+          if (live(4 * hf + ct))
+            acc[rt][4 * hf + ct] = __builtin_amdgcn_mfma_f32_16x16x32_bf16(wh[ks & 1][rt], xl[ct], acc[rt][4 * hf + ct], 0, 0, 0);
 #pragma unroll
       for (int rt = 0; rt < 4; ++rt)
 #pragma unroll
         for (int ct = 0; ct < 4; ++ct)
-          acc[rt][4 * hf + ct] = __builtin_amdgcn_mfma_f32_16x16x32_bf16(wh[ks & 1][rt], xh[ct], acc[rt][4 * hf + ct], 0, 0, 0);
+          if (live(4 * hf + ct))
+            acc[rt][4 * hf + ct] = __builtin_amdgcn_mfma_f32_16x16x32_bf16(wh[ks & 1][rt], xh[ct], acc[rt][4 * hf + ct], 0, 0, 0);
     }
     __builtin_amdgcn_sched_barrier(0);
   }
@@ -577,10 +592,17 @@
       for (int rt = 0; rt < 4; ++rt)
 #pragma unroll
         for (int ct = 0; ct < 4; ++ct) a2[rt][ct] = acc[rt][4 * half + ct];
+      if constexpr (AT) {
+        if (half == 0) store_hidden_tile16<MX, 0x9>(xt, a2, q.b_first[head], wave, lane, MX ? q.first_scale[head] : 1.0f, c16);
+        else store_hidden_tile16<MX, 0x4>(xt, a2, q.b_first[head], wave, lane, MX ? q.first_scale[head] : 1.0f, c16);
+      } else
       store_hidden_tile16<MX>(xt, a2, q.b_first[head], wave, lane, MX ? q.first_scale[head] : 1.0f, c16);
       if constexpr (MX) __builtin_amdgcn_sched_barrier(0);
       __syncthreads();
-      if constexpr (AT) head_tail_from_lds16(p, xt, head, SlotMap{at_slots, p.M, p.HW, half});
+      if constexpr (AT) {
+        if (half == 0) head_tail_from_lds16<SlotMap, 0x9>(p, xt, head, SlotMap{at_slots, p.M, p.HW, half});
+        else head_tail_from_lds16<SlotMap, 0x4>(p, xt, head, SlotMap{at_slots, p.M, p.HW, half});
+      }
       else head_tail_from_lds16(p, xt, head, TileMap{b, y0 + (64 >> TSH) * half, x0, q.H, q.W, TSH});
       __syncthreads();
     }
@@ -609,6 +631,7 @@
       const f32x4 bb = *reinterpret_cast<const f32x4*>(b1 + 32 * s2 + 16);
 #pragma unroll
       for (int ct = 0; ct < 8; ++ct) {
+        if (!live(ct)) continue;
         float v[8], hi[8];
 #pragma unroll
         for (int j = 0; j < 8; ++j) {
@@ -633,7 +656,7 @@
 #pragma unroll
     for (int r = 0; r < 4; ++r) {
       const int n = 4 * g + r;
-      if (n < n_out) red[(wave * 16 + n) * HP_PX + ct * 16 + c16] = oacc[ct][r];
+      if (live(ct) && n < n_out) red[(wave * 16 + n) * HP_PX + ct * 16 + c16] = oacc[ct][r];
     }
   __syncthreads();
   {
diff --git a/centerfusiondetect3d_amd/csrc/cf_topk.hip b/centerfusiondetect3d_amd/csrc/cf_topk.hip
--- a/centerfusiondetect3d_amd/csrc/cf_topk.hip
+++ b/centerfusiondetect3d_amd/csrc/cf_topk.hip
@@ -143,13 +143,119 @@
   topk_slice_body<NMS>(heat, C, H, W, K, out_keys, blockIdx.x / TOPK_SLICES, blockIdx.x % TOPK_SLICES);
 }
 
+struct TopkRegLds {
+  uint64_t keys[TOPK_CAP];
+  __attribute__((aligned(16))) uint32_t gmax[256];
+  uint32_t hist[256];
+  uint32_t wave_cnt[TOPK_RT / 64];
+  uint32_t s_gt, s_sel[2];
+};
+
+__device__ __forceinline__ void topk_reg_select(TopkRegLds& s, const uint32_t (&u)[TOPK_RE], int lo, int hi, int K,
+                                                uint64_t* __restrict__ out) {
+  uint64_t* const keys = s.keys;
+  uint32_t* const gmax = s.gmax;
+  uint32_t* const hist = s.hist;
+  uint32_t* const wave_cnt = s.wave_cnt;
+  uint32_t& s_gt = s.s_gt;
+  uint32_t* const s_sel = s.s_sel;
+  const int tid = threadIdx.x;
+  uint32_t lmax = 0;
+#pragma unroll
+  for (int e = 0; e < TOPK_RE; ++e) lmax = max(lmax, u[e]);
+  const int P = K <= 128 ? 8 : 4, G = TOPK_RT / P;
+  {
+    uint32_t m = lmax;
+    m = max(m, (uint32_t)__shfl_xor((int)m, 1));
+    m = max(m, (uint32_t)__shfl_xor((int)m, 2));
+    if (P == 8) m = max(m, (uint32_t)__shfl_xor((int)m, 4));
+    if ((tid & (P - 1)) == 0) gmax[tid / P] = m;
+  }
+  if (tid == 0) s_sel[0] = 0u;
+  __syncthreads();
+  {
+    const int c = tid / P, part = tid & (P - 1), per = G / P;
+    const uint32_t mine = gmax[c];
+    const u32x4p* g4 = reinterpret_cast<const u32x4p*>(gmax + part * per);
+    int rank = 0;
+#pragma unroll 4
+    for (int j4 = 0; j4 < per / 4; ++j4) {
+      const u32x4p o = g4[j4];
+#pragma unroll
+      for (int e = 0; e < 4; ++e) rank += (o[e] > mine || (o[e] == mine && part * per + 4 * j4 + e < c)) ? 1 : 0;
+    }
+    rank += __shfl_xor(rank, 1);
+    rank += __shfl_xor(rank, 2);
+    if (P == 8) rank += __shfl_xor(rank, 4);
+    if (part == 0 && rank == K - 1) s_sel[0] = mine;
+  }
+  __syncthreads();
+  uint32_t L = s_sel[0];
+  __syncthreads();
+
+  if (tid == 0) s_gt = 0;
+  __syncthreads();
+#pragma unroll
+  for (int e = 0; e < TOPK_RE; ++e) {
+    const int i = lo + tid + e * TOPK_RT;
+    if (i < hi && u[e] >= L) {
+      const uint32_t pos = atomicAdd(&s_gt, 1u);
+      if (pos < TOPK_CAP) keys[pos] = pack_key(u[e], i);
+    }
+  }
+  __syncthreads();
+  if (s_gt <= TOPK_CAP) {
+    rank_select_desc(keys, (int)s_gt, K, out);
+    return;
+  }
+  __syncthreads();
+
+  for (int attempt = 0; attempt < 2; ++attempt) {
+    if (tid == 0) s_gt = 0;
+    __syncthreads();
+#pragma unroll
+    for (int e = 0; e < TOPK_RE; ++e) {
+      const int i = lo + tid + e * TOPK_RT;
+      if (i < hi && u[e] > L) {
+        const uint32_t pos = atomicAdd(&s_gt, 1u);
+        if (pos < TOPK_CAP) keys[pos] = pack_key(u[e], i);
+      }
+    }
+    __syncthreads();
+    if (s_gt <= TOPK_CAP) break;
+    L = topk_radix_select<TOPK_RT>(hist, s_sel, K, [&](auto count) {
+#pragma unroll
+      for (int e = 0; e < TOPK_RE; ++e)
+        if (lo + tid + e * TOPK_RT < hi) count(u[e]);
+    });
+  }
+  const int g = (int)s_gt;
+  int total = g;
+  if (g < K) {
+    const int r = K - g;
+    int found = 0;
+#pragma unroll 1
+    for (int e = 0; e < TOPK_RE && found < r; ++e) {
+      const int i = lo + tid + e * TOPK_RT;
+      uint32_t ue = 0;
+#pragma unroll
+      for (int q = 0; q < TOPK_RE; ++q) ue = q == e ? u[q] : ue;
+      const bool eq = i < hi && ue == L;
+      int all;
+      const int rank = found + topk_tie_round<TOPK_RT>(eq, wave_cnt, all);
+      if (eq && rank < r) keys[g + rank] = pack_key(L, i);
+      found += all;
+      __syncthreads();
+    }
+    total = K;
+  }
+  __syncthreads();
+  rank_select_desc(keys, total, K, out);
+}
+
 __global__ __launch_bounds__(TOPK_RT) void topk_slice_reg_kernel(const float* __restrict__ heat, int C, int H, int W, int K,
                                                                  uint64_t* __restrict__ out_keys) {
-  __shared__ uint64_t keys[TOPK_CAP];
-  __shared__ __attribute__((aligned(16))) uint32_t gmax[256];
-  __shared__ uint32_t hist[256];
-  __shared__ uint32_t wave_cnt[TOPK_RT / 64];
-  __shared__ uint32_t s_gt, s_sel[2];
+  __shared__ TopkRegLds s;
   const int tid = threadIdx.x;
   const int N = C * H * W;
   const int img_i = blockIdx.x / TOPK_SLICES, slice = blockIdx.x % TOPK_SLICES;
@@ -159,106 +265,72 @@
   uint64_t* out = out_keys + (size_t)blockIdx.x * K;
   const int n = hi - lo;
   if (n <= K) {
-    topk_tiny_slice<TOPK_RT>(keys, lo, n, K, out, [&](int i) { return f2u(img[i]); });
+    topk_tiny_slice<TOPK_RT>(s.keys, lo, n, K, out, [&](int i) { return f2u(img[i]); });
     return;
   }
   uint32_t u[TOPK_RE];
-  uint32_t lmax = 0;
 #pragma unroll
   for (int e = 0; e < TOPK_RE; ++e) {
     const int i = lo + tid + e * TOPK_RT;
     u[e] = i < hi ? f2u(img[i]) : 0u;
   }
-#pragma unroll
-  for (int e = 0; e < TOPK_RE; ++e) lmax = max(lmax, u[e]);
-  const int P = K <= 128 ? 8 : 4, G = TOPK_RT / P;
-  {
-    uint32_t m = lmax;
-    m = max(m, (uint32_t)__shfl_xor((int)m, 1));
-    m = max(m, (uint32_t)__shfl_xor((int)m, 2));
-    if (P == 8) m = max(m, (uint32_t)__shfl_xor((int)m, 4));
-    if ((tid & (P - 1)) == 0) gmax[tid / P] = m;
-  }
-  if (tid == 0) s_sel[0] = 0u;
-  __syncthreads();
-  {
-    const int c = tid / P, part = tid & (P - 1), per = G / P;
-    const uint32_t mine = gmax[c];
-    const u32x4p* g4 = reinterpret_cast<const u32x4p*>(gmax + part * per);
-    int rank = 0;
-#pragma unroll 4
-    for (int j4 = 0; j4 < per / 4; ++j4) {
-      const u32x4p o = g4[j4];
-#pragma unroll
-      for (int e = 0; e < 4; ++e) rank += (o[e] > mine || (o[e] == mine && part * per + 4 * j4 + e < c)) ? 1 : 0;
-    }
-    rank += __shfl_xor(rank, 1);
-    rank += __shfl_xor(rank, 2);
-    if (P == 8) rank += __shfl_xor(rank, 4);
-    if (part == 0 && rank == K - 1) s_sel[0] = mine;
-  }
-  __syncthreads();
-  uint32_t L = s_sel[0];
-  __syncthreads();
-
-  if (tid == 0) s_gt = 0;
-  __syncthreads();
-#pragma unroll
-  for (int e = 0; e < TOPK_RE; ++e) {
-    const int i = lo + tid + e * TOPK_RT;
-    if (i < hi && u[e] >= L) {
-      const uint32_t pos = atomicAdd(&s_gt, 1u);
-      if (pos < TOPK_CAP) keys[pos] = pack_key(u[e], i);
-    }
-  }
-  __syncthreads();
-  if (s_gt <= TOPK_CAP) {
-    rank_select_desc(keys, (int)s_gt, K, out);
+  topk_reg_select(s, u, lo, hi, K, out);
+}
+
+constexpr int TOPK_NB = 4;
+template <bool RAW>
+__global__ __launch_bounds__(TOPK_RT) void topk_slice_reg_nms_kernel(const float* __restrict__ heat, int C, int H, int W, int K,
+                                                                     uint64_t* __restrict__ out_keys, size_t set_stride) {
+  __shared__ TopkRegLds s;
+  const int tid = threadIdx.x;
+  const int HW = H * W, N = C * HW;
+  const int img_i = blockIdx.x / TOPK_SLICES, slice = blockIdx.x % TOPK_SLICES;
+  const float* img = heat + (size_t)img_i * N;
+  const int len = (N + TOPK_SLICES - 1) / TOPK_SLICES;
+  const int lo = min(slice * len, N), hi = min(lo + len, N);
+  uint64_t* out_raw = out_keys + (size_t)blockIdx.x * K;
+  uint64_t* out_nms = out_raw + set_stride;
+  const int n = hi - lo;
+  if (n <= K) {
+    if (RAW) {
+      topk_tiny_slice<TOPK_RT>(s.keys, lo, n, K, out_raw, [&](int i) { return f2u(img[i]); });
+      __syncthreads();
+    }
+    topk_tiny_slice<TOPK_RT>(s.keys, lo, n, K, out_nms, [&](int i) { return f2u(peak_value<true>(img, i, H, W)); });
     return;
   }
-  __syncthreads();
-
-  for (int attempt = 0; attempt < 2; ++attempt) {
-    if (tid == 0) s_gt = 0;
-    __syncthreads();
-#pragma unroll
-    for (int e = 0; e < TOPK_RE; ++e) {
-      const int i = lo + tid + e * TOPK_RT;
-      if (i < hi && u[e] > L) {
-        const uint32_t pos = atomicAdd(&s_gt, 1u);
-        if (pos < TOPK_CAP) keys[pos] = pack_key(u[e], i);
-      }
-    }
-    __syncthreads();
-    if (s_gt <= TOPK_CAP) break;
-    L = topk_radix_select<TOPK_RT>(hist, s_sel, K, [&](auto count) {
-#pragma unroll
-      for (int e = 0; e < TOPK_RE; ++e)
-        if (lo + tid + e * TOPK_RT < hi) count(u[e]);
-    });
-  }
-  const int g = (int)s_gt;
-  int total = g;
-  if (g < K) {
-    const int r = K - g;
-    int found = 0;
-#pragma unroll 1
-    for (int e = 0; e < TOPK_RE && found < r; ++e) {
-      const int i = lo + tid + e * TOPK_RT;
-      uint32_t ue = 0;
-#pragma unroll
-      for (int q = 0; q < TOPK_RE; ++q) ue = q == e ? u[q] : ue;
-      const bool eq = i < hi && ue == L;
-      int all;
-      const int rank = found + topk_tie_round<TOPK_RT>(eq, wave_cnt, all);
-      if (eq && rank < r) keys[g + rank] = pack_key(L, i);
-      found += all;
-      __syncthreads();
-    }
-    total = K;
-  }
-  __syncthreads();
-  rank_select_desc(keys, total, K, out);
+  uint32_t ur[TOPK_RE], un[TOPK_RE];
+#pragma unroll
+  for (int eb = 0; eb < TOPK_RE; eb += TOPK_NB) {
+    float w[TOPK_NB][9];
+#pragma unroll
+    for (int q = 0; q < TOPK_NB; ++q) {
+      const int i = min(lo + tid + (eb + q) * TOPK_RT, hi - 1);
+      const int c = i / HW, pix = i - c * HW;
+      const int y = pix / W, x = pix - y * W;
+      const float* pl = img + (size_t)c * HW;
+      const int r0 = (y > 0 ? y - 1 : y) * W, r1 = y * W, r2 = (y < H - 1 ? y + 1 : y) * W;
+      const int x0 = x > 0 ? x - 1 : x, x2 = x < W - 1 ? x + 1 : x;
+      w[q][0] = pl[r0 + x0]; w[q][1] = pl[r0 + x]; w[q][2] = pl[r0 + x2];
+      w[q][3] = pl[r1 + x0]; w[q][4] = pl[r1 + x]; w[q][5] = pl[r1 + x2];
+      w[q][6] = pl[r2 + x0]; w[q][7] = pl[r2 + x]; w[q][8] = pl[r2 + x2];
+    }
+#pragma unroll
+    for (int q = 0; q < TOPK_NB; ++q) {
+      const bool in = lo + tid + (eb + q) * TOPK_RT < hi;
+      const float v = w[q][4];
+      float m = v;
+#pragma unroll
+      for (int k = 0; k < 9; ++k) m = fmaxf(m, w[q][k]);
+      un[eb + q] = in ? f2u((m == v) ? v : v * 0.0f) : 0u;
+      ur[eb + q] = in ? f2u(v) : 0u;
+    }
+  }
+  if constexpr (RAW) {
+    topk_reg_select(s, ur, lo, hi, K, out_raw);
+    __syncthreads();
+  }
+  topk_reg_select(s, un, lo, hi, K, out_nms);
 }
 
 template <int THREADS>
@@ -284,6 +356,49 @@
   for (int i = tid; i < total; i += TOPK_MERGE_THREADS) keys[i] = src[i];
   __syncthreads();
   emit_peaks<TOPK_MERGE_THREADS>(merge_sorted_lists(keys, keys + total, K), K, HW, blockIdx.x, scores, inds, classes);
+}
+
+struct TopkPeakOut {
+  float* scores;
+  int32_t* inds;
+  int32_t* classes;
+};
+__global__ __launch_bounds__(TOPK_MERGE_THREADS) void topk_merge_fused_kernel(const uint64_t* __restrict__ in_keys, size_t set_stride,
+                                                                              int B, int K, int HW, TopkPeakOut raw, TopkPeakOut nms,
+                                                                              int32_t* __restrict__ tab_ab, int32_t* __restrict__ tab_b) {
+  extern __shared__ __attribute__((aligned(16))) uint64_t keys[];
+  const int tid = threadIdx.x, total = TOPK_SLICES * K;
+  const bool has_raw = raw.scores != nullptr;
+  const int b = blockIdx.x % B, set = has_raw ? blockIdx.x / B : 1;
+  const uint64_t* src = in_keys + (size_t)set * set_stride + (size_t)b * total;
+  for (int i = tid; i < total; i += TOPK_MERGE_THREADS) keys[i] = src[i];
+  __syncthreads();
+  const uint64_t* best = merge_sorted_lists(keys, keys + total, K);
+  const TopkPeakOut o = set ? nms : raw;
+  constexpr int slots = CF_HEAD_AT_SLOTS;
+  const int per_p = (2 * K + slots - 1) / slots * slots, per_s = (K + slots - 1) / slots * slots;
+  int32_t* const tp = tab_ab ? tab_ab + (size_t)b * per_p : nullptr;
+  int32_t* const ts = tab_b ? tab_b + (size_t)b * per_s : nullptr;
+  for (int j = tid; j < K; j += TOPK_MERGE_THREADS) {
+    float score;
+    int pix, cls;
+    unpack_key(best[j], HW, score, pix, cls);
+    o.scores[(size_t)b * K + j] = score;
+    o.inds[(size_t)b * K + j] = pix;
+    o.classes[(size_t)b * K + j] = cls;
+    const int v = (unsigned)pix < (unsigned)HW ? b * HW + pix : -1;
+    if (tp) tp[set * K + j] = v;
+    if (ts && set) ts[j] = v;
+  }
+  if (set) {
+    if (tp) {
+      for (int j = 2 * K + tid; j < per_p; j += TOPK_MERGE_THREADS) tp[j] = -1;
+      if (!has_raw)
+        for (int j = tid; j < K; j += TOPK_MERGE_THREADS) tp[j] = -1;
+    }
+    if (ts)
+      for (int j = K + tid; j < per_s; j += TOPK_MERGE_THREADS) ts[j] = -1;
+  }
 }
 }
 
@@ -335,6 +450,46 @@
   return cf_check_launch("cf_topk_peaks");
 }
 
+static bool topk_fused_reg(int C, int H, int W) {
+  return ((long)C * H * W + TOPK_SLICES - 1) / TOPK_SLICES <= (long)TOPK_RT * TOPK_RE;
+}
+
+extern "C" size_t cf_topk_peaks_fused_workspace_bytes(int B, int C, int H, int W, int K) {
+  const bool reg = C > 0 && H > 0 && W > 0 && topk_fused_reg(C, H, W);
+  return cf_topk_workspace_bytes(B, K) + (reg ? cf_topk_workspace_bytes(B, K) : cf_topk_workspace_bytes_nms(B, C, H, W, K));
+}
+
+extern "C" int cf_topk_peaks_fused(const float* heat, int B, int C, int H, int W, int K, float* raw_scores, int32_t* raw_inds,
+                                   int32_t* raw_classes, float* scores, int32_t* inds, int32_t* classes, int32_t* table_ab,
+                                   int32_t* table_b, void* workspace, void* stream) {
+  const char* who = "cf_topk_peaks_fused";
+  CF_REQUIRE(heat && scores && inds && classes && workspace, "%s: null buffer", who);
+  const bool raw = raw_scores != nullptr;
+  CF_REQUIRE(raw == (raw_inds != nullptr) && raw == (raw_classes != nullptr), "%s: the raw peaks are all three or none", who);
+  if (const int e = topk_check_geometry(who, B, C, H, W, K)) return e;
+  if (table_ab || table_b) {
+    CF_REQUIRE((long)B * H * W < (1L << 31), "%s: B * HW must stay below 2^31 (flat pixels are int32)", who);
+    CF_REQUIRE((long)B * (2L * K + CF_HEAD_AT_SLOTS) < (1L << 31), "%s: B * K too large", who);
+  }
+  hipStream_t st = (hipStream_t)stream;
+  const size_t set_stride = (size_t)B * TOPK_SLICES * K;
+  uint64_t* keys = static_cast<uint64_t*>(workspace);
+  if (topk_fused_reg(C, H, W)) {
+    const auto kernel = raw ? topk_slice_reg_nms_kernel<true> : topk_slice_reg_nms_kernel<false>;
+    hipLaunchKernelGGL(kernel, dim3(B * TOPK_SLICES), dim3(TOPK_RT), 0, st, heat, C, H, W, K, keys, set_stride);
+  } else {
+    if (raw)
+      if (const int e = topk_launch_slices(who, heat, B, C, H, W, K, 0, keys, st)) return e;
+    if (const int e = topk_launch_slices(who, heat, B, C, H, W, K, 2, keys + set_stride, st)) return e;
+  }
+  static CfLdsLimit merge_limit;
+  merge_limit.ensure(topk_merge_fused_kernel, topk_merge_lds_bytes(K), 65536);
+  hipLaunchKernelGGL(topk_merge_fused_kernel, dim3(B * (raw ? 2 : 1)), dim3(TOPK_MERGE_THREADS), topk_merge_lds_bytes(K), st,
+                     static_cast<const uint64_t*>(keys), set_stride, B, K, H * W, TopkPeakOut{raw_scores, raw_inds, raw_classes},
+                     TopkPeakOut{scores, inds, classes}, table_ab, table_b);
+  return cf_check_launch(who);
+}
+
 namespace {
 __global__ __launch_bounds__(TOPK_THREADS) void topk_fallback_kernel(const float* __restrict__ heat, int C, int H, int W, int K,
                                                                      uint64_t* __restrict__ keys_ws, float* __restrict__ scores,
diff --git a/centerfusiondetect3d_amd/ops.py b/centerfusiondetect3d_amd/ops.py
--- a/centerfusiondetect3d_amd/ops.py
+++ b/centerfusiondetect3d_amd/ops.py
@@ -911,6 +911,24 @@
     return scores, inds, classes
 
 
+def topk_peaks_fused(heat, K=100, want_raw=True, want_tables=True):
+    _need_cuda(heat)
+    if not heat.is_contiguous():
+        heat = heat.contiguous()
+    B, Cc, H, W = heat.shape
+    dev = heat.device
+    new = lambda: (torch.empty((B, K), device=dev, dtype=torch.float32), torch.empty((B, K), device=dev, dtype=torch.int32),
+                   torch.empty((B, K), device=dev, dtype=torch.int32))
+    raw, nms = (new() if want_raw else (None, None, None)), new()
+    t_ab = torch.empty((B, -(-2 * K // 18), 18), device=dev, dtype=torch.int32) if want_tables else None
+    t_b = torch.empty((B, -(-K // 18), 18), device=dev, dtype=torch.int32) if want_tables else None
+    lib = _lib.load()
+    ws = torch.empty(max(1, lib.cf_topk_peaks_fused_workspace_bytes(B, Cc, H, W, K)), device=dev, dtype=torch.uint8)
+    _lib.check(lib.cf_topk_peaks_fused(heat.data_ptr(), B, Cc, H, W, K, *(_lib.ptr(t) for t in raw), *(t.data_ptr() for t in nms),
+                                       _lib.ptr(t_ab), _lib.ptr(t_b), ws.data_ptr(), _lib.stream_ptr()), "cf_topk_peaks_fused")
+    return (raw if want_raw else None), nms, t_ab, t_b
+
+
 def frustum_assoc(inds, depth, wh, dim, rot, calib, pc_dep, max_pc_dist=60.0, want_nhwc4=False,
                   pc_hm=None, pc_hm_nhwc4=None, pc_hm_split8=None):
     _need_cuda(inds, depth, wh, dim, rot, calib, pc_dep)
diff --git a/centerfusiondetect3d_amd/plan.py b/centerfusiondetect3d_amd/plan.py
--- a/centerfusiondetect3d_amd/plan.py
+++ b/centerfusiondetect3d_amd/plan.py
@@ -358,7 +358,9 @@
         tiles_b, tiles_ab = -(-K // AT_SLOTS), -(-2 * K // AT_SLOTS)
         self.at = dict(f_hm=f_hm, flops_hm=B * self.h4 * self.w4 * px_hm, f_rest=f_rest, px_rest=px_rest,
                        tab_b=self._buf(B * tiles_b * AT_SLOTS, dtype=torch.int32), n_b=B * tiles_b,
-                       tab_ab=self._buf(B * tiles_ab * AT_SLOTS, dtype=torch.int32) if self.frustum else None, n_ab=B * tiles_ab)
+                       tab_ab=self._buf(B * tiles_ab * AT_SLOTS, dtype=torch.int32) if self.frustum else None, n_ab=B * tiles_ab,
+                       ws=self._buf(max(1, self.lib.cf_topk_peaks_fused_workspace_bytes(B, self._m.config.heads["heatmap"], self.h4,
+                                                                                        self.w4, K)), dtype=torch.uint8))
 
     def _peaks_lane(self):
         ev_a = self.new_event()
@@ -602,8 +604,10 @@
         if at is None:
             self._launch(st)
         else:
-            topk = (lib.cf_topk_peaks, hm.data_ptr(), B, heads["heatmap"], h4, w4, K, 0, *tk) if self.frustum else None
-            self._launch(st, self._at_seq(at, peaks, topk, pk_i))
+            raw = tk[:3] if self.frustum else (None, None, None)
+            fused = (hm.data_ptr(), B, heads["heatmap"], h4, w4, K, *raw, pk_s.data_ptr(), pk_i.data_ptr(), pk_c.data_ptr(),
+                     at["tab_ab"].data_ptr() if self.frustum else None, at["tab_b"].data_ptr(), at["ws"].data_ptr())
+            self._launch(st, self._at_seq(at, (_peaks_fused_and_checksum, lib, fused, peaks[3])))
             y = self._pending(y, model, written)
         if self.peaks_step is not None and peaks_on:
             hm._cf_peaks = (K, hm.data_ptr(), pk_s, pk_i, pk_c, pk_sum)
@@ -612,15 +616,13 @@
                     t.record_stream(self._side)
         return [y]
 
-    def _at_seq(self, at, peaks, topk, pk_i):
+    def _at_seq(self, at, peaks):
         lib, idx = self.lib, self.step_index
         tab_b, n_b = at["tab_b"].data_ptr(), at["n_b"]
         tab_p, n_p = (at["tab_ab"].data_ptr(), at["n_ab"]) if self.frustum else (tab_b, n_b)
-        HP_PX = 128
-        extra = ([("at.topk", topk, 0)] if topk is not None else []) + [("at.peaks", peaks, 0)]
-        extra += [
-                  ("at.tables", (lib.cf_head_slot_tables, self.tk_inds.data_ptr() if self.frustum else None, pk_i.data_ptr(),
-                                 self.B, self.K, self.h4 * self.w4, at["tab_ab"].data_ptr() if self.frustum else None, tab_b), 0),
+        HP_PX = 48
+        extra = ([("at.topk", (_no_launch,), 0)] if self.frustum else []) + [
+                  ("at.peaks", peaks, 0), ("at.tables", (_no_launch,), 0),
                   ("at.primary", (lib.cf_head_fused_at, C.byref(at["f_rest"]), tab_p, n_p), 0)]
         repl = {idx["tails.primary"]: (lib.cf_head_fused, C.byref(at["f_hm"]))}
         self.step_flops["tails.primary"] = at["flops_hm"]
@@ -692,6 +694,11 @@
     return 0
 
 
+def _peaks_fused_and_checksum(lib, fused_args, sum_args, stream):
+    rc = lib.cf_topk_peaks_fused(*fused_args, stream)
+    return rc if rc != 0 else lib.cf_checksum64(*sum_args, stream)
+
+
 def _peaks_and_checksum(lib, topk_args, sum_args, stream):
     rc = lib.cf_topk_peaks(*topk_args, stream)
     return rc if rc != 0 else lib.cf_checksum64(*sum_args, stream)
diff --git a/include/cf_hip.h b/include/cf_hip.h
--- a/include/cf_hip.h
+++ b/include/cf_hip.h
@@ -162,6 +162,7 @@
 int cf_head_fused(const cf_head_fused_args* a, void* stream);
 int cf_head_fused_with(const cf_head_fused_args* a, int tile, int pc_skip, void* stream);
 
+#define CF_HEAD_AT_SLOTS 18
 int cf_head_fused_at(const cf_head_fused_args* a, const int32_t* slot_pixels, int n_tiles, void* stream);
 int cf_head_slot_tables(const int32_t* list_a, const int32_t* list_b, int B, int K, int HW, int32_t* table_ab,
                         int32_t* table_b, void* stream);
@@ -251,6 +252,10 @@
                              int32_t* classes, void* workspace, const unsigned long long* sums, void* stream);
 int cf_topk_peaks(const float* heat, int B, int C, int H, int W, int K, int nms, float* scores,
                   int32_t* inds, int32_t* classes, void* workspace, void* stream);
+size_t cf_topk_peaks_fused_workspace_bytes(int B, int C, int H, int W, int K);
+int cf_topk_peaks_fused(const float* heat, int B, int C, int H, int W, int K, float* raw_scores, int32_t* raw_inds,
+                        int32_t* raw_classes, float* scores, int32_t* inds, int32_t* classes, int32_t* table_ab,
+                        int32_t* table_b, void* workspace, void* stream);
 
 int cf_frustum_assoc(const int32_t* inds, int K, const float* depth, const float* wh,
                      const float* dim, const float* rot, const float* calib, const float* pc_dep,
```

Measured after the change: 3088 frames/s, median of 6. +2.3%, better.
